# aous72/OpenJPH

Hardware: AMD Instinct MI355X
Metric: Msamples/s encode+decode, 8K 12-bit 4:4:4; achieved HBM GB/s vs roofline (higher is better)
Workload: dtype f32; 1 GPU; c3_8k_444_12b_irv97; width=7680, height=4320, components=3, bit_depth=12, wavelet=9/7 irreversible, decomps=5, hip_streams=1, sample_container_bits=16, roundtrip_max_abs_err=8

## Files before the change

### openjph_amd/csrc/ht_tables.h

```cpp
#ifndef OJPH_HT_TABLES_H
#define OJPH_HT_TABLES_H
#include <stdint.h>

namespace ojphgpu {

struct HtTables {
  uint16_t enc_vlc[2][2048];
  uint16_t dec_vlc[2][1024];
  uint32_t dec_vlc32[2][1024];
  uint16_t dec_uvlc0[320];
  uint16_t dec_uvlc1[256];
};

void build_ht_tables(HtTables& t);
int ensure_tables();
int upload_enc_tables(const HtTables& t);
int upload_dec_tables(const HtTables& t);

}

struct ojphgpu_cb_desc; struct ojphgpu_cb_result;
namespace ojphgpu {
int ht_encode_launch(void* stream, const ojphgpu_cb_desc* d_blocks, uint32_t n, const void* d_coef, uint8_t* d_scratch,
                     uint8_t* d_out, uint32_t out_cap, ojphgpu_cb_result* d_results, uint32_t* d_cursor, uint32_t* d_status,
                     int widths, const uint32_t* d_regions, uint32_t nreg);
bool dec_fuses();
uint64_t ht_decode_fused_state_words(uint32_t n);
uint32_t device_cus(int device);
bool ht_decode_fused_pays(uint32_t n, uint32_t max_h, uint32_t cus);
uint32_t ht_decode_fused_grid(uint32_t n, uint32_t cus);
int ht_decode_fused_launch(void* stream, const ojphgpu_cb_desc* d_blocks, uint32_t n, const uint8_t* d_data, uint32_t* d_quad_scratch,
                           void* d_coef, uint8_t* d_block_status, uint32_t* d_state, uint32_t epoch, uint32_t max_h, int kinds,
                           uint32_t cus, uint32_t* d_host_retry);
uint32_t ht_decode64_extra_aux_words(uint32_t len1);
int ht_decode64_launch(void* stream, const ojphgpu_cb_desc* d_blocks, uint32_t n, const uint8_t* d_data, uint32_t* d_aux,
                       uint32_t* d_quad_scratch, void* d_coef, uint8_t* d_block_status, int refine);
int ht_decode_step2_launch(void* stream, const ojphgpu_cb_desc* d_blocks, uint32_t n, const uint8_t* d_data,
                           const uint32_t* d_quad_scratch, void* d_coef, uint8_t* d_block_status, int kinds);
inline int ht_decode_block_kinds(uint32_t w, uint32_t reversible, uint32_t num_passes, uint32_t len2)
{
  const int refine = (num_passes > 1u && len2 > 0u) ? 16 : 0;
  if (reversible & 4u) return refine | 32;
  return refine | (w > 64u ? 2 : 1) | ((reversible & 1u) ? 4 : 8) | (w > 32u ? 64 : 0) | (w > 16u ? 128 : 0) | 256;
}

}
#endif
```

### openjph_amd/csrc/kernels_ht_enc.hip

```cpp
#include <hip/hip_runtime.h>
#include <stdint.h>
#include <cstdlib>
#include <type_traits>
#include "../../include/ojphgpu.h"
#include "ht_quant.h"
#include "ht_tables.h"

namespace ojphgpu {
__device__ __attribute__((aligned(16))) uint16_t g_enc_vlc[2][2048];
}

namespace {

using ojphgpu::to_sign_mag;

constexpr int MS_WORDS = 512;
constexpr int VLC_WORDS = 64;
constexpr int MEL_CAP = 192;
constexpr int VLC_CAP = 3072 - MEL_CAP;
constexpr int WAVES = 4;
constexpr uint32_t NARROW_MAX_W = 64;

constexpr int MS_WORDS64 = 1040;
constexpr int VLC_WORDS64 = 96;
template <int MSW, int VLW>
struct WaveLdsT {
  uint32_t ms[MSW];
  uint32_t vlc[VLW];
  uint32_t ev[8];
  uint8_t  mel[MEL_CAP];
};

__device__ __forceinline__ void wave_sync()
{
  __builtin_amdgcn_fence(__ATOMIC_SEQ_CST, "wavefront");
  __builtin_amdgcn_wave_barrier();
}

__device__ __forceinline__ uint32_t wave_incl_scan(uint32_t v, int)
{
  int x = (int)v;
  x += __builtin_amdgcn_update_dpp(0, x, 0x111, 0xF, 0xF, false);
  x += __builtin_amdgcn_update_dpp(0, x, 0x112, 0xF, 0xF, false);
  x += __builtin_amdgcn_update_dpp(0, x, 0x114, 0xF, 0xF, false);
  x += __builtin_amdgcn_update_dpp(0, x, 0x118, 0xF, 0xF, false);
  x += __builtin_amdgcn_update_dpp(0, x, 0x142, 0xA, 0xF, false);
  x += __builtin_amdgcn_update_dpp(0, x, 0x143, 0xC, 0xF, false);
  return (uint32_t)x;
}

__device__ __forceinline__ uint32_t get_bits(const uint32_t* buf, uint32_t pos, uint32_t n)
{
  const uint32_t w = pos >> 5, sh = pos & 31;
  const uint32_t lo = buf[w], hi = buf[w + 1];
  const uint32_t v = __funnelshift_r(lo, hi, sh);
  return v & ((1u << n) - 1u);
}

__device__ __forceinline__ void or_bits(uint32_t* buf, uint32_t pos, uint32_t v, uint32_t n)
{
  if (n == 0) return;
  const uint32_t w = pos >> 5, sh = pos & 31;
  atomicOr(&buf[w], v << sh);
  if (sh + n > 32) atomicOr(&buf[w + 1], v >> (32 - sh));
}

__device__ __forceinline__ uint32_t rdlane(uint32_t v, int l) { return (uint32_t)__builtin_amdgcn_readlane((int)v, l); }
__device__ __forceinline__ uint32_t rdfirst(uint32_t v) { return (uint32_t)__builtin_amdgcn_readfirstlane((int)v); }

__device__ __forceinline__ uint32_t expo(uint32_t val) { return val ? 32u - (uint32_t)__clz((int)(val - 1)) : 0u; }
__device__ __forceinline__ uint32_t expo(uint64_t val) { return val ? 64u - (uint32_t)__clzll((long long)(val - 1)) : 0u; }

__device__ __forceinline__ uint32_t mel_exp(uint32_t k)
{
  const uint64_t tbl = 0ull | (1ull << 9) | (1ull << 12) | (1ull << 15) | (2ull << 18) | (2ull << 21) | (2ull << 24) |
                       (3ull << 27) | (3ull << 30) | (4ull << 33) | (5ull << 36);
  return (uint32_t)(tbl >> (3 * k)) & 7u;
}

struct MelState {
  uint32_t k, run, acc, nb, pos, lastff, err;
};

__device__ __forceinline__ void mel_put(MelState& m, uint8_t* buf, uint32_t code, uint32_t n, int lane)
{
  m.acc = (m.acc << n) | code; m.nb += n;
  for (;;) {
    const uint32_t need = m.lastff ? 7u : 8u;
    if (m.nb < need) break;
    const uint32_t byte = (m.acc >> (m.nb - need)) & ((1u << need) - 1u);
    m.nb -= need; m.acc &= (1u << m.nb) - 1u;
    if (m.pos >= (uint32_t)MEL_CAP) { m.err = 1; break; }
    if (lane == 0) buf[m.pos] = (uint8_t)byte;
    m.pos++; m.lastff = (byte == 0xFF);
  }
}

__device__ __forceinline__ void mel_zero_run(MelState& m, uint8_t* buf, uint32_t n, int lane)
{
  while (n > 0) {
    const uint32_t thr = 1u << mel_exp(m.k);
    const uint32_t need = thr - m.run;
    if (n >= need) { mel_put(m, buf, 1, 1, lane); n -= need; m.run = 0; m.k = m.k < 12 ? m.k + 1 : 12; }
    else { m.run += n; n = 0; }
  }
}

__device__ __forceinline__ void mel_one(MelState& m, uint8_t* buf, int lane)
{
  const uint32_t e = mel_exp(m.k);
  mel_put(m, buf, m.run, e + 1, lane);
  m.run = 0; m.k = m.k > 0 ? m.k - 1 : 0;
}

struct Claim { uint32_t raw, base, cap; };
__device__ __forceinline__ Claim claim_request(uint32_t* cursor, const uint32_t* regions, uint32_t nreg, uint32_t bi,
                                               uint32_t bytes, uint32_t out_cap, int lane)
{
  Claim c = { 0, 0, out_cap };
  uint32_t* cur = cursor;
  if (nreg) {
    const uint32_t r = bi & (nreg - 1u);
    c.base = regions[2u * r]; c.cap = regions[2u * r + 1u];
    cur = cursor + 32u * r;
  }
  if (lane == 0) {
    uint32_t z = 0;
    asm volatile("" : "+v"(z));
    c.raw = atomicAdd(cur + z, bytes);
  }
  return c;
}
__device__ __forceinline__ uint32_t claim_offset(const Claim& c, uint32_t bytes)
{
  const uint32_t off = rdfirst(c.raw);
  return (off > c.cap || bytes > c.cap - off) ? 0xFFFFFFFFu : c.base + off;
}
__device__ __forceinline__ uint32_t claim_output(uint32_t* cursor, const uint32_t* regions, uint32_t nreg, uint32_t bi,
                                                 uint32_t bytes, uint32_t out_cap, int lane)
{
  return claim_offset(claim_request(cursor, regions, nreg, bi, bytes, out_cap, lane), bytes);
}

template <bool S64>
__global__ __launch_bounds__(64 * WAVES) void ht_encode_wide_kernel(
    const ojphgpu_cb_desc* __restrict__ blocks, uint32_t n, const uint32_t* __restrict__ coef,
    uint8_t* __restrict__ scratch, uint8_t* __restrict__ out, uint32_t out_cap,
    ojphgpu_cb_result* __restrict__ results, uint32_t* __restrict__ cursor, uint32_t* __restrict__ status,
    const uint32_t* __restrict__ regions, uint32_t nreg)
{
  using V = typename std::conditional<S64, uint64_t, uint32_t>::type;
  constexpr uint32_t VBITS = S64 ? 64u : 32u;
  constexpr int MSW = S64 ? MS_WORDS64 : MS_WORDS, VLW = S64 ? VLC_WORDS64 : VLC_WORDS;
  __shared__ __attribute__((aligned(16))) uint16_t s_vlc[2][2048];
  __shared__ WaveLdsT<MSW, VLW> s_wave[WAVES];
  const int lane = threadIdx.x & 63;
  const int wave = __builtin_amdgcn_readfirstlane((int)(threadIdx.x >> 6));
  const uint32_t bi = blockIdx.x * WAVES + wave;
  const bool mine = bi < n && (S64 ? (blocks[bi].reversible & 4u) != 0 : (blocks[bi].w > NARROW_MAX_W && (blocks[bi].reversible & 4u) == 0));
  if (!__syncthreads_or(mine ? 1 : 0)) return;
  for (int i = threadIdx.x; i < 2 * 2048 / 8; i += blockDim.x)
    reinterpret_cast<uint4*>(&s_vlc[0][0])[i] = reinterpret_cast<const uint4*>(&ojphgpu::g_enc_vlc[0][0])[i];
  __syncthreads();
  if (!mine) return;
  const ojphgpu_cb_desc d = blocks[bi];
  WaveLdsT<MSW, VLW>& L = s_wave[wave];
  const uint32_t W = d.w, H = d.h;
  if (W == 0 || H == 0) { if (lane == 0) { results[bi].offset = 0; results[bi].length = 0; } return; }
  const uint32_t K = d.K_max, p = VBITS - 1u - K;
  const bool rev = (d.reversible & 1u) != 0;
  const float delta_inv = rev ? 0.0f : __fdiv_rn(1.0f, d.delta);
  const uint32_t* src = coef + d.coef_off;
  const uint32_t pitch = d.pitch;
  uint8_t* ms_out = scratch + d.data_off;
  const uint32_t ms_cap = d.scratch_cap > (uint32_t)VLC_CAP ? d.scratch_cap - VLC_CAP : 0;
  uint8_t* vlc_last = scratch + d.data_off + d.scratch_cap - 1;

  const uint32_t QW = (W + 1) >> 1, QH = (H + 1) >> 1, PW = (QW + 1) >> 1, NP = PW * QH;

  for (int i = lane; i < MSW; i += 64) L.ms[i] = 0;
  for (int i = lane; i < VLW; i += 64) L.vlc[i] = 0;
  if (lane < 8) L.ev[lane] = 0;
  wave_sync();
  if (lane == 0) L.vlc[0] = 0xF;
  wave_sync();

  uint32_t ms_carry = 0, ms_k = 0, ms_ff = 0;
  uint32_t v_carry = 4, v_pos = 1, v_prev = 0xFF;
  MelState mel = { 0, 0, 0, 0, 0, 0, 0 };
  uint32_t err = 0, any_sig = 0;
  uint32_t carry_rho = 0;

  uint32_t over = 0;
  auto sample = [&](int x, int y) -> V {
    if (x < 0 || y < 0 || x >= (int)W || y >= (int)H) return (V)0;
    if constexpr (S64) {
      const long long v = reinterpret_cast<const long long*>(src)[(size_t)y * pitch + x];
      const uint64_t m = (v >= 0 ? (uint64_t)v : 0ull - (uint64_t)v) << p;
      over |= (uint32_t)(m >> 63);
      return (v >= 0 ? 0ull : 0x8000000000000000ull) | m;
    } else
      return to_sign_mag(src[(size_t)y * pitch + x], rev, p, delta_inv, over);
  };

  for (uint32_t base = 0; base < NP; base += 64) {
    const uint32_t P = base + lane;
    const bool active = P < NP;
    const uint32_t qy = active ? P / PW : 0, px = active ? P - qy * PW : 0;
    const int x0 = (int)(4 * px), y0 = (int)(2 * qy);
    const bool has_q1 = active && (x0 + 2 < (int)W);
    const bool first_row = qy == 0;

    V val[8]; uint32_t sgn[8];
#pragma unroll
    for (int i = 0; i < 8; ++i) {
      const int q = i >> 2, nn = i & 3;
      V t = active ? sample(x0 + 2 * q + (nn >> 1), y0 + (nn & 1)) : (V)0;
      val[i] = ((V)(t + t) >> p) & ~(V)1;
      sgn[i] = (uint32_t)(t >> (VBITS - 1u));
    }
    uint32_t Eab[6], Sab[6];
#pragma unroll
    for (int i = 0; i < 6; ++i) {
      V t = (active && !first_row) ? sample(x0 - 1 + i, y0 - 1) : (V)0;
      V v = ((V)(t + t) >> p) & ~(V)1;
      Eab[i] = expo(v); Sab[i] = v != 0;
    }

    uint32_t rho[2], cq[2], uq[2], Uq[2], tup[2];
    V msv[8]; uint32_t msl[8];
    uint32_t rho_q[2] = { 0, 0 }, emax[2] = { 0, 0 }, e[8];
#pragma unroll
    for (int i = 0; i < 8; ++i) {
      e[i] = expo(val[i]);
      if (val[i]) rho_q[i >> 2] |= 1u << (i & 3);
      emax[i >> 2] = max(emax[i >> 2], e[i]);
    }
    if (!has_q1) { rho_q[1] = 0; emax[1] = 0; }
    uint32_t rho_prev = __shfl_up(rho_q[1], 1);
    if (lane == 0) rho_prev = carry_rho;
    if (px == 0) rho_prev = 0;
    carry_rho = rdlane(rho_q[1], 63);
#pragma unroll
    for (int q = 0; q < 2; ++q) {
      const uint32_t rl = q == 0 ? rho_prev : rho_q[0];
      uint32_t kappa = 1, c;
      if (first_row) c = (rl >> 1) | (rl & 1);
      else {
        const uint32_t* E = Eab + 2 * q; const uint32_t* S = Sab + 2 * q;
        uint32_t me = max(max(E[0], E[1]), max(E[2], E[3]));
        int max_e = (int)me - 1;
        if (rho_q[q] & (rho_q[q] - 1)) kappa = (uint32_t)max(1, max_e);
        c = (S[0] | S[1]) | ((S[2] | S[3]) << 2) | ((rl & 4) >> 1) | ((rl & 8) >> 2);
      }
      const uint32_t U = max(emax[q], kappa), u = U - kappa;
      uint32_t eps = 0;
      if (u > 0) {
#pragma unroll
        for (int nn = 0; nn < 4; ++nn) eps |= (uint32_t)(e[q * 4 + nn] == emax[q]) << nn;
      }
      const uint32_t tuple = s_vlc[first_row ? 0 : 1][(c << 8) + (rho_q[q] << 4) + eps];
      rho[q] = rho_q[q]; cq[q] = c; uq[q] = u; Uq[q] = U; tup[q] = tuple;
#pragma unroll
      for (int nn = 0; nn < 4; ++nn) {
        const int i = q * 4 + nn;
        const uint32_t m = ((rho_q[q] >> nn) & 1u) ? U - ((tuple >> nn) & 1u) : 0u;
        const V s = val[i] ? val[i] - 2u + sgn[i] : (V)0;
        msl[i] = m;
        msv[i] = m ? (s & ((m >= VBITS ? (V)0 : ((V)1 << m)) - (V)1)) : (V)0;
      }
    }
    const bool q0on = active, q1on = has_q1;
    if (!q1on) { uq[1] = 0; for (int nn = 4; nn < 8; ++nn) { msl[nn] = 0; msv[nn] = 0; } }
    if (!q0on) { uq[0] = 0; for (int nn = 0; nn < 4; ++nn) { msl[nn] = 0; msv[nn] = 0; } }
    any_sig |= (__ballot(((rho[0] | rho[1]) != 0 && active) || over != 0u) != 0ull) ? 1u : 0u;

    uint64_t vb = 0; uint32_t vl = 0;
    auto vadd = [&](uint32_t c, uint32_t len) { vb |= (uint64_t)c << vl; vl += len; };
    uint32_t x0e = 0, xl0 = 0, x1e = 0, xl1 = 0;
    auto uvlc = [](uint32_t u, uint32_t& pre, uint32_t& pl, uint32_t& suf, uint32_t& sl, uint32_t& ext, uint32_t& el) {
      ext = 0; el = 0;
      if (u == 0) { pre = 0; pl = 0; suf = 0; sl = 0; }
      else if (u == 1) { pre = 1; pl = 1; suf = 0; sl = 0; }
      else if (u == 2) { pre = 2; pl = 2; suf = 0; sl = 0; }
      else if (u <= 4) { pre = 4; pl = 3; suf = u - 3; sl = 1; }
      else if (u <= 32 || !S64) { pre = 0; pl = 3; suf = u - 5; sl = 5; }
      else { pre = 0; pl = 3; suf = 28u + ((u - 33u) & 3u); sl = 5; ext = (u - 33u) >> 2; el = 4; }
    };
    bool ev2_valid = false; uint32_t ev2_bit = 0;
    if (q0on) {
      vadd(tup[0] >> 8, (tup[0] >> 4) & 7);
      if (q1on) vadd(tup[1] >> 8, (tup[1] >> 4) & 7);
      const uint32_t u0 = uq[0], u1 = uq[1];
      uint32_t p0, l0, s0, sl0, p1, l1, s1, sl1;
      if (first_row && u0 > 0 && u1 > 0) { ev2_valid = true; ev2_bit = min(u0, u1) > 2; }
      if (first_row && u0 > 2 && u1 > 2) {
        uvlc(u0 - 2, p0, l0, s0, sl0, x0e, xl0); uvlc(u1 - 2, p1, l1, s1, sl1, x1e, xl1);
        vadd(p0, l0); vadd(p1, l1); vadd(s0, sl0); vadd(s1, sl1); vadd(x0e, xl0); vadd(x1e, xl1);
      } else if (first_row && u0 > 2 && u1 > 0) {
        uvlc(u0, p0, l0, s0, sl0, x0e, xl0);
        vadd(p0, l0); vadd(u1 - 1, 1); vadd(s0, sl0); vadd(x0e, xl0);
      } else {
        uvlc(u0, p0, l0, s0, sl0, x0e, xl0); uvlc(u1, p1, l1, s1, sl1, x1e, xl1);
        vadd(p0, l0); vadd(p1, l1); vadd(s0, sl0); vadd(s1, sl1); vadd(x0e, xl0); vadd(x1e, xl1);
      }
    }

    const bool ev0_valid = q0on && cq[0] == 0, ev1_valid = q1on && cq[1] == 0;
    const uint32_t ev0_bit = rho[0] != 0, ev1_bit = rho[1] != 0;
    {
      const uint32_t cnt = (uint32_t)ev0_valid + (uint32_t)ev1_valid + (uint32_t)ev2_valid;
      const uint32_t incl = wave_incl_scan(cnt, lane);
      const uint32_t nev = rdlane(incl, 63);
      uint32_t at = incl - cnt;
      if (ev0_valid) { if (ev0_bit) atomicOr(&L.ev[at >> 5], 1u << (at & 31)); at++; }
      if (ev1_valid) { if (ev1_bit) atomicOr(&L.ev[at >> 5], 1u << (at & 31)); at++; }
      if (ev2_valid) { if (ev2_bit) atomicOr(&L.ev[at >> 5], 1u << (at & 31)); at++; }
      wave_sync();
      uint32_t done = 0;
      while (done < nev) {
        const uint32_t w = done >> 5, sh = done & 31;
        uint32_t word = rdfirst(L.ev[w]) >> sh;
        const uint32_t avail = min(32u - sh, nev - done);
        if (word == 0) { mel_zero_run(mel, L.mel, avail, lane); done += avail; continue; }
        const uint32_t z = (uint32_t)__builtin_ctz(word);
        if (z >= avail) { mel_zero_run(mel, L.mel, avail, lane); done += avail; continue; }
        mel_zero_run(mel, L.mel, z, lane);
        mel_one(mel, L.mel, lane);
        done += z + 1;
      }
      wave_sync();
      if (lane < 8) L.ev[lane] = 0;
    }

    {
      uint32_t tot = 0;
#pragma unroll
      for (int i = 0; i < 8; ++i) tot += msl[i];
      const uint32_t incl = wave_incl_scan(tot, lane);
      const uint32_t T = ms_carry + rdlane(incl, 63);
      uint32_t at = ms_carry + incl - tot;
#pragma unroll
      for (int i = 0; i < 8; ++i) {
        if constexpr (S64) {
          const uint32_t lo = msl[i] < 32u ? msl[i] : 32u;
          or_bits(L.ms, at, (uint32_t)msv[i], lo);
          if (msl[i] > 32u) or_bits(L.ms, at + 32u, (uint32_t)(msv[i] >> 32), msl[i] - 32u);
        } else or_bits(L.ms, at, (uint32_t)msv[i], msl[i]);
        at += msl[i];
      }
      wave_sync();
      uint32_t pos = 0;
      for (;;) {
        const uint32_t first_n = ms_ff ? 7u : 8u;
        const uint32_t start = pos + (lane == 0 ? 0u : first_n + 8u * (uint32_t)(lane - 1));
        const uint32_t nb = lane == 0 ? first_n : 8u;
        const bool ok = start + nb <= T;
        const uint32_t v = ok ? get_bits(L.ms, start, nb) : 0u;
        const uint64_t m_ok = __ballot(ok), m_ff = __ballot(ok && v == 0xFF);
        const uint32_t n_ok = m_ok == ~0ull ? 64u : (uint32_t)__builtin_ctzll(~m_ok);
        const uint32_t f_ff = m_ff ? (uint32_t)__builtin_ctzll(m_ff) : 64u;
        const uint32_t nc = min(n_ok, f_ff + 1u);
        if (nc == 0) break;
        if (ms_k + nc > ms_cap) { err = 1; break; }
        if ((uint32_t)lane < nc) ms_out[ms_k + lane] = (uint8_t)v;
        ms_k += nc;
        pos += first_n + 8u * (nc - 1u);
        ms_ff = f_ff < n_ok ? 1u : 0u;
      }
      const uint32_t rem = T - pos;
      const uint32_t cv = rem ? get_bits(L.ms, pos, rem) : 0u;
      wave_sync();
      const uint32_t used = (T >> 5) + 2;
      for (uint32_t i = lane; i < used && i < (uint32_t)MSW; i += 64) L.ms[i] = 0;
      wave_sync();
      if (lane == 0) L.ms[0] = cv;
      ms_carry = rem;
      wave_sync();
    }

    {
      const uint32_t incl = wave_incl_scan(vl, lane);
      const uint32_t T = v_carry + rdlane(incl, 63);
      {
        const uint32_t at = v_carry + incl - vl, lo = vl < 32u ? vl : 32u;
        or_bits(L.vlc, at, (uint32_t)vb, lo);
        if (vl > 32u) or_bits(L.vlc, at + 32u, (uint32_t)(vb >> 32), vl - 32u);
      }
      wave_sync();
      uint32_t pos = 0;
      for (;;) {
        const uint32_t start = pos + 8u * (uint32_t)lane;
        const bool have7 = start + 7 <= T, have8 = start + 8 <= T;
        const uint32_t v8 = have7 ? get_bits(L.vlc, start, 8) : 0u;
        uint32_t pv = __shfl_up(v8, 1);
        if (lane == 0) pv = v_prev;
        const bool special = have7 && pv > 0x8F && (v8 & 0x7F) == 0x7F;
        const bool stop = !have8 && !special;
        const uint64_t m_sp = __ballot(special), m_st = __ballot(stop);
        const uint32_t fs = m_sp ? (uint32_t)__builtin_ctzll(m_sp) : 64u;
        const uint32_t ft = m_st ? (uint32_t)__builtin_ctzll(m_st) : 64u;
        const uint32_t n8 = min(fs, ft);
        const bool sp = fs < ft;
        if (n8 == 0 && !sp) break;
        if (v_pos + n8 + 1 >= (uint32_t)VLC_CAP) { err = 1; break; }
        if ((uint32_t)lane < n8) *(vlc_last - (v_pos + lane)) = (uint8_t)v8;
        if (sp && (uint32_t)lane == fs) *(vlc_last - (v_pos + lane)) = 0x7F;
        const uint32_t last8 = n8 ? rdlane(v8, (int)(n8 - 1)) : v_prev;
        v_pos += n8 + (sp ? 1u : 0u);
        pos += 8u * n8 + (sp ? 7u : 0u);
        v_prev = sp ? 0x7Fu : last8;
      }
      const uint32_t rem = T - pos;
      const uint32_t cv = rem ? get_bits(L.vlc, pos, rem) : 0u;
      wave_sync();
      for (int i = lane; i < VLW; i += 64) L.vlc[i] = 0;
      wave_sync();
      if (lane == 0) L.vlc[0] = cv;
      v_carry = rem;
      wave_sync();
    }
    if (err) break;
  }

  err |= mel.err;
  uint32_t total = 0, ms_len = ms_k;
  if (!err && any_sig) {
    const uint32_t ms_tmp0 = rdfirst(L.ms[0]);
    if (ms_carry) {
      const uint32_t maxb = ms_ff ? 7u : 8u, t = maxb - ms_carry;
      const uint32_t tmp = ms_tmp0 | ((0xFFu & ((1u << t) - 1u)) << ms_carry);
      if (tmp != 0xFF) {
        if (ms_len >= ms_cap) err = 1;
        else { if (lane == 0) ms_out[ms_len] = (uint8_t)tmp; ms_len++; }
      }
    } else if (ms_ff) ms_len--;
    if (mel.run > 0) mel_put(mel, L.mel, 1, 1, lane);
    const uint32_t need = mel.lastff ? 7u : 8u, remaining = need - mel.nb;
    const uint32_t mel_tmp = (mel.acc << remaining) & 0xFFu;
    const uint32_t mel_mask = (0xFFu << remaining) & 0xFFu;
    const uint32_t vlc_tmp = rdfirst(L.vlc[0]) & 0xFFu;
    const uint32_t vlc_mask = v_carry ? (0xFFu >> (8 - v_carry)) : 0u;
    if ((mel_mask | vlc_mask) != 0) {
      if (mel.pos >= (uint32_t)MEL_CAP) err = 1;
      else {
        const uint32_t fuse = mel_tmp | vlc_tmp;
        if (((((fuse ^ mel_tmp) & mel_mask) | ((fuse ^ vlc_tmp) & vlc_mask)) == 0) && fuse != 0xFF && v_pos > 1) {
          if (lane == 0) L.mel[mel.pos] = (uint8_t)fuse;
          mel.pos++;
        } else {
          if (v_pos >= (uint32_t)VLC_CAP) err = 1;
          else {
            if (lane == 0) { L.mel[mel.pos] = (uint8_t)mel_tmp; *(vlc_last - v_pos) = (uint8_t)vlc_tmp; }
            mel.pos++; v_pos++;
          }
        }
      }
    }
    err |= mel.err;
    total = ms_len + mel.pos + v_pos;
  }
  wave_sync();
  __threadfence_block();

  uint32_t off = 0;
  if (err) total = 0;
  if (total) {
    off = claim_output(cursor, regions, nreg, bi, (total + 3u) & ~3u, out_cap, lane);
    if (off == 0xFFFFFFFFu) { err = 1; total = 0; off = 0; }
  }
  if (total) {
    const uint32_t scup = mel.pos + v_pos;
    uint8_t* dst = out + off;
    const uint8_t* vsrc = vlc_last - v_pos + 1;
    for (uint32_t i = lane; i < total; i += 64) {
      uint32_t b;
      if (i < ms_len) b = ms_out[i];
      else if (i < ms_len + mel.pos) b = L.mel[i - ms_len];
      else b = vsrc[i - ms_len - mel.pos];
      if (i == total - 1) b = scup >> 4;
      else if (i == total - 2) b = (b & 0xF0u) | (scup & 0xFu);
      dst[i] = (uint8_t)b;
    }
  }
  if (lane == 0) {
    results[bi].offset = off; results[bi].length = total;
    if (err) atomicOr(status, 1u);
  }
}

#ifndef ABL
#define ABL 0
#endif
#ifndef NWAVES
#define NWAVES 4
#endif
#ifndef NOUT_CAP
#define NOUT_CAP 5120
#endif
#ifndef NWAVES_PER_EU
#define NWAVES_PER_EU 4
#endif
constexpr uint32_t OUT_CAP = NOUT_CAP;
constexpr int PMS_WORDS = 576;
constexpr int PVLC_WORDS = 112;

struct NarrowLds {
  uint32_t out[OUT_CAP / 4];
  uint32_t ms[PMS_WORDS];
  uint32_t vlc[PVLC_WORDS];
  uint8_t  mel[MEL_CAP + 8];
};
static_assert(MEL_CAP + 8 >= 4 * (MEL_CAP / 4 + 2), "raw MEL words");
#ifndef NWG_PER_CU
#define NWG_PER_CU 4
#endif
static_assert(NWG_PER_CU * (2 * 2048 * 2 + 64 * 4 + NWAVES * sizeof(NarrowLds)) <= 160 * 1024, "the narrow kernel's workgroups do not fit the LDS as planned");

#ifndef ENC_ROWS_W4V
#define ENC_ROWS_W4V 1
#endif
#ifndef ENC_ROWS_AHEAD
#define ENC_ROWS_AHEAD 1
#endif
static_assert(ENC_ROWS_AHEAD == 1 || ENC_ROWS_AHEAD == 2, "one or two steps of rows in flight");

struct __attribute__((aligned(4))) U4 { uint32_t x, y, z, w; };
typedef uint32_t U4V __attribute__((ext_vector_type(4), aligned(4)));

template <int KIND> struct RawRows {
  uint32_t t[4], b[4];
  __device__ __forceinline__ void arrived() { asm volatile("" : "+v"(t[0]), "+v"(t[1]), "+v"(t[2]), "+v"(t[3]), "+v"(b[0]), "+v"(b[1]), "+v"(b[2]), "+v"(b[3])); }
  __device__ __forceinline__ uint32_t top(int k) const { return t[k]; }
  __device__ __forceinline__ uint32_t bot(int k) const { return b[k]; }
};
template <> struct RawRows<1> {
  U4V t, b;
  __device__ __forceinline__ void arrived() { asm volatile("" : "+v"(t), "+v"(b)); }
  __device__ __forceinline__ uint32_t top(int k) const { return t[k]; }
  __device__ __forceinline__ uint32_t bot(int k) const { return b[k]; }
};

__device__ __forceinline__ uint32_t dpp_prev(uint32_t v) { return (uint32_t)__builtin_amdgcn_update_dpp(0, (int)v, 0x138, 0xF, 0xF, false); }
__device__ __forceinline__ uint32_t dpp_next(uint32_t v) { return (uint32_t)__builtin_amdgcn_update_dpp(0, (int)v, 0x130, 0xF, 0xF, false); }

__device__ __forceinline__ uint32_t uvlc_word(uint32_t u)
{
  const uint32_t lo = u < 3u ? 1u : 0u, mid = (u >= 3u && u < 5u) ? 1u : 0u;
  const uint32_t pre = lo ? u : (mid ? 4u : 0u);
  const uint32_t pl = u < 3u ? u : 3u;
  const uint32_t suf = lo ? 0u : (mid ? u - 3u : u - 5u);
  const uint32_t sl = lo ? 0u : (mid ? 1u : 5u);
  return pre | (pl << 8) | (suf << 16) | (sl << 24);
}

constexpr uint64_t MEL_PM = (1ull << 0) | (1ull << 1) | (1ull << 2) | (1ull << 3) | (1ull << 5) | (1ull << 7) | (1ull << 9) | (1ull << 13) |
                            (1ull << 17) | (1ull << 21) | (1ull << 29) | (1ull << 37) | (1ull << 53);
constexpr uint32_t MEL_RAW_BITS = 8u * MEL_CAP;
constexpr uint32_t MEL_RAW_WORDS = MEL_CAP / 4 + 2;

__device__ __forceinline__ void mel_at(uint32_t k, uint32_t c, uint32_t& K, uint32_t& run, uint32_t& ones, uint32_t& pKm1)
{
  const uint32_t full = c >= 85u ? (c - 53u) >> 5 : 0u;
  const uint32_t cc = c - 32u * full;
  if (cc >= 53u) { K = 12u; run = cc - 53u; pKm1 = 37u; }
  else {
    const uint64_t m = MEL_PM << (63u - cc);
    const uint32_t lz = (uint32_t)__builtin_clzll(m);
    K = (uint32_t)__popcll(m) - 1u; run = lz;
    const uint64_t m2 = m & ~(0x8000000000000000ull >> lz);
    pKm1 = m2 ? cc - (uint32_t)__builtin_clzll(m2) : 0u;
  }
  ones = K - k + full;
}

__device__ __forceinline__ void mel_stuff(const uint32_t* raw, uint32_t total_bits, uint8_t* out, MelState& st, int lane)
{
  uint32_t pos = 0, bytes = 0, lastff = 0, err = 0;
  for (;;) {
    const uint32_t first = lastff ? 7u : 8u;
    const uint32_t start = pos + (lane == 0 ? 0u : first + 8u * ((uint32_t)lane - 1u));
    const uint32_t len = lane == 0 ? first : 8u;
    const bool have = start + len <= total_bits;
    const uint32_t w = start >> 5, sh = start & 31u;
    const uint32_t x = have ? __funnelshift_l(raw[w + 1], raw[w], sh) >> (32u - len) : 0u;
    const uint64_t m_have = __ballot(have), m_ff = __ballot(have && x == 0xFFu);
    const uint32_t n_ok = m_have == ~0ull ? 64u : (uint32_t)__builtin_ctzll(~m_have);
    const uint32_t f_ff = m_ff ? (uint32_t)__builtin_ctzll(m_ff) : 64u;
    const uint32_t nc = min(n_ok, f_ff + 1u);
    if (nc == 0) break;
    if (bytes + nc > (uint32_t)MEL_CAP) { err = 1; break; }
    if ((uint32_t)lane < nc) out[bytes + lane] = (uint8_t)x;
    bytes += nc;
    pos += first + 8u * (nc - 1u);
    lastff = f_ff < n_ok ? 1u : 0u;
  }
  const uint32_t left = total_bits - pos;
  const uint32_t w = pos >> 5, sh = pos & 31u;
  const uint32_t x = left ? rdfirst(__funnelshift_l(raw[w + 1], raw[w], sh)) >> (32u - left) : 0u;
  st.k = 0; st.run = 0; st.acc = x; st.nb = left; st.pos = bytes; st.lastff = lastff; st.err = err;
}

template <bool REV, int LOGP>
__global__ __launch_bounds__(64 * NWAVES) __attribute__((amdgpu_waves_per_eu(NWAVES_PER_EU, 8))) void ht_encode_kernel(
    const ojphgpu_cb_desc* __restrict__ blocks, uint32_t n, const uint32_t* __restrict__ coef,
    uint8_t* __restrict__ scratch, uint8_t* __restrict__ out, uint32_t out_cap,
    ojphgpu_cb_result* __restrict__ results, uint32_t* __restrict__ cursor, uint32_t* __restrict__ status,
    const uint32_t* __restrict__ regions, uint32_t nreg)
{
  __shared__ __attribute__((aligned(16))) uint16_t s_vlc[2][2048];
  __shared__ uint32_t s_uvlc[64];
  __shared__ NarrowLds s_wave[NWAVES];
  const int lane = threadIdx.x & 63;
  const int wave = __builtin_amdgcn_readfirstlane((int)(threadIdx.x >> 6));
  const uint32_t bi = blockIdx.x * NWAVES + wave;
  struct DescWords { uint32_t v[sizeof(ojphgpu_cb_desc) / 4]; } dw;
  __builtin_memcpy(&dw, blocks + min(bi, n - 1u), sizeof dw);
  ojphgpu_cb_desc d;
  __builtin_memcpy(&d, &dw, sizeof d);
  static_assert(offsetof(ojphgpu_cb_desc, K_max) == 16 && offsetof(ojphgpu_cb_desc, reversible) == 17, "K_max, reversible: bytes 0, 1 of dword 4");
  uint32_t kr = dw.v[4];
  asm volatile("" : "+s"(kr));
  const uint32_t d_K_max = kr & 0xFFu, d_reversible = (kr >> 8) & 0xFFu;
  const uint32_t W = d.w, H = d.h;
  constexpr uint32_t PPR = 1u << LOGP, RPS = 64u >> LOGP;
  const bool my_width = LOGP == 5 ? (W > NARROW_MAX_W && W <= 4u * PPR) : (W <= NARROW_MAX_W && W <= 4u * PPR);
  const bool my_kind = bi < n && my_width && ((d_reversible & 1u) != 0) == REV && (d_reversible & 4u) == 0;
  const bool mine = my_kind && W != 0 && H != 0;
  NarrowLds& L = s_wave[wave];
  uint8_t* outb = reinterpret_cast<uint8_t*>(L.out);
  const uint32_t K = d_K_max, p = 31u - K;
  constexpr bool rev = REV;
  const float delta_inv = rev ? 0.0f : __fdiv_rn(1.0f, d.delta);
  const uint32_t* src = coef + d.coef_off;
  const uint32_t pitch = d.pitch;
  uint8_t* ms_spill = scratch + d.data_off;
  const uint32_t ms_cap = d.scratch_cap > (uint32_t)VLC_CAP ? d.scratch_cap - VLC_CAP : 0;
  const uint32_t QW = (W + 1) >> 1, QH = (H + 1) >> 1, PW = (QW + 1) >> 1;
  const uint32_t nsteps = (QH + RPS - 1u) / RPS;

  const uint32_t r = (uint32_t)lane >> LOGP, px = (uint32_t)lane & (PPR - 1u);
  const bool pxok = px < PW;
  const uint32_t x0 = 4u * px;
  const bool has_q1 = pxok && x0 + 2 < W;

  auto prologue = [&](bool clear) __attribute__((always_inline)) {
    for (int i = threadIdx.x; i < 2 * 2048 / 8; i += blockDim.x)
      reinterpret_cast<uint4*>(&s_vlc[0][0])[i] = reinterpret_cast<const uint4*>(&ojphgpu::g_enc_vlc[0][0])[i];
    if (threadIdx.x < 64) s_uvlc[threadIdx.x] = uvlc_word(threadIdx.x);
    if (clear) {
      for (int i = lane; i < PMS_WORDS; i += 64) L.ms[i] = 0;
      for (int i = lane; i < PVLC_WORDS; i += 64) L.vlc[i] = 0;
      if (lane < (int)MEL_RAW_WORDS) reinterpret_cast<uint32_t*>(L.mel)[lane] = 0;
      wave_sync();
      if (lane == 0) { L.vlc[0] = 0xF; outb[OUT_CAP - 1] = 0xFF; }
      wave_sync();
    }
    __syncthreads();
  };
  if (!mine) {
    prologue(false);
    if (my_kind && lane == 0) { results[bi].offset = 0; results[bi].length = 0; }
    return;
  }
  const bool w4 = (W & 3u) == 0;

  uint32_t ms_pend = 0, ms_base = 0, ms_k = 0, ms_ff = 0;
  uint32_t v_pend = 4, v_base = 0, v_pos = 1, v_prev = 0xFF;
  uint32_t mel_k = 0, mel_c = 0, mel_bits = 0, mel_err = 0;
  uint32_t* const mel_raw = reinterpret_cast<uint32_t*>(L.mel);
  auto mel_or = [&](uint32_t code, uint32_t len, uint32_t pos) __attribute__((always_inline)) {
    if (len) {
      const uint32_t sh = pos & 31u, w = pos >> 5;
      const uint64_t v = (uint64_t)code << (64u - sh - len);
      atomicOr(&mel_raw[w], (uint32_t)(v >> 32));
      if (sh + len > 32u) atomicOr(&mel_raw[w + 1u], (uint32_t)v);
    }
  };
  auto mel_ones = [&](uint32_t n) __attribute__((always_inline)) {
    if (n == 0u) return;
    if (mel_bits + n > MEL_RAW_BITS) mel_err = 1;
    else if (lane == 0) mel_or((1u << n) - 1u, n, mel_bits);
    mel_bits += n;
  };
  auto mel_zeros = [&](uint32_t n) __attribute__((always_inline)) {
    mel_c += n;
    if (mel_c >= 85u) {
      const uint32_t full = (mel_c - 53u) >> 5;
      mel_ones(12u - mel_k + full);
      mel_k = 12u; mel_c -= 32u * full;
    }
  };
  uint32_t err = 0, any_sig = 0;
  bool prev_sig = false;

  uint32_t ms_out = 0;
  auto flush_stage = [&]() __attribute__((always_inline)) -> bool {
    const uint32_t have = ms_k - ms_out, nwd = have >> 2;
    if (ms_out + 4u * nwd > ms_cap) return false;
    uint32_t* g = reinterpret_cast<uint32_t*>(ms_spill + ms_out);
    for (uint32_t i = lane; i < nwd; i += 64) g[i] = L.out[i];
    const uint32_t keep = L.out[nwd];
    wave_sync();
    if (lane == 0) L.out[0] = keep;
    wave_sync();
    ms_out += 4u * nwd;
    return true;
  };

  uint32_t last_S = 0;

  auto ms_windows = [&](uint32_t base, uint32_t T, bool flush) __attribute__((always_inline)) -> uint32_t {
    uint32_t pos = base;
    for (;;) {
      const uint32_t first_n = ms_ff ? 7u : 8u;
      if (!flush && pos + first_n + 8u * 255u > T) break;
      const uint32_t start = pos + (lane == 0 ? 0u : first_n + 8u * (4u * (uint32_t)lane - 1u));
      const uint32_t lead = lane == 0 ? first_n : 8u;
      uint32_t v = 0, cnt = 0;
      if (start + lead <= T) {
        const uint32_t w = start >> 5, sh = start & 31u;
        v = __funnelshift_r(L.ms[w], L.ms[w + 1], sh);
        cnt = min(4u, 1u + ((T - start - lead) >> 3));
      }
      const uint32_t bytes = (lane == 0 && first_n == 7u) ? ((v & 0x7Fu) | ((v >> 7) << 8)) : v;
      const uint32_t have = cnt == 4u ? 0xFFFFFFFFu : (1u << (8u * cnt)) - 1u;
      const uint32_t ffm = (((bytes & 0x7F7F7F7Fu) + 0x01010101u) & bytes & 0x80808080u) & have;
      const uint64_t m_full = __ballot(cnt == 4u), m_ff = __ballot(ffm != 0u);
      const uint32_t nfull = m_full == ~0ull ? 64u : (uint32_t)__builtin_ctzll(~m_full);
      const uint32_t n_ok = nfull == 64u ? 256u : 4u * nfull + rdlane(cnt, (int)nfull);
      uint32_t f_ff = 256u;
      if (m_ff) { const uint32_t lf = (uint32_t)__builtin_ctzll(m_ff); f_ff = 4u * lf + ((uint32_t)__builtin_ctz(rdlane(ffm, (int)lf)) >> 3); }
      const uint32_t nc = min(n_ok, f_ff + 1u);
      if (nc == 0) break;
      if (ms_k - ms_out + nc + v_pos + 72u > OUT_CAP && !flush_stage()) { err = 1; break; }
      uint8_t* dstb = outb + (ms_k - ms_out) + 4u * (uint32_t)lane;
      const uint32_t mine = nc > 4u * (uint32_t)lane ? min(4u, nc - 4u * (uint32_t)lane) : 0u;
      if (mine > 0) dstb[0] = (uint8_t)bytes;
      if (mine > 1) dstb[1] = (uint8_t)(bytes >> 8);
      if (mine > 2) dstb[2] = (uint8_t)(bytes >> 16);
      if (mine > 3) dstb[3] = (uint8_t)(bytes >> 24);
      ms_k += nc;
      pos += first_n + 8u * (nc - 1u);
      ms_ff = f_ff < n_ok ? 1u : 0u;
    }
    return pos;
  };
  auto ms_windows_full = [&](uint32_t base, uint32_t T) __attribute__((always_inline)) -> uint32_t {
    uint32_t pos = base;
    for (;;) {
      const uint32_t first_n = ms_ff ? 7u : 8u;
      if (pos + first_n + 8u * 255u > T) break;
      const uint32_t start = lane == 0 ? pos : pos + first_n - 8u + 32u * (uint32_t)lane;
      const uint32_t w = start >> 5, sh = start & 31u;
      uint32_t bytes = __funnelshift_r(L.ms[w], L.ms[w + 1], sh);
      if (ms_ff) bytes = lane == 0 ? ((bytes & 0x7Fu) | ((bytes >> 7) << 8)) : bytes;
      const uint32_t ffm = ((bytes & 0x7F7F7F7Fu) + 0x01010101u) & bytes & 0x80808080u;
      const uint64_t m_ff = __ballot(ffm != 0u);
      uint32_t nc = 256u, ff = 0u;
      if (m_ff) { const uint32_t lf = (uint32_t)__builtin_ctzll(m_ff); nc = 4u * lf + ((uint32_t)__builtin_ctz(rdlane(ffm, (int)lf)) >> 3) + 1u; ff = 1u; }
      if (ms_k - ms_out + nc + v_pos + 72u > OUT_CAP && !flush_stage()) { err = 1; break; }
      if (4u * (uint32_t)lane < nc) __builtin_memcpy(outb + (ms_k - ms_out) + 4u * (uint32_t)lane, &bytes, 4);
      ms_k += nc;
      pos += first_n + 8u * (nc - 1u);
      ms_ff = ff;
    }
    return pos;
  };
  auto vlc_windows_full = [&](uint32_t base, uint32_t T) __attribute__((always_inline)) -> uint32_t {
    uint32_t pos = base;
    for (;;) {
      if (pos + 8u * 64u > T) break;
      const uint32_t v8 = get_bits(L.vlc, pos + 8u * (uint32_t)lane, 8);
      uint32_t pv = dpp_prev(v8);
      if (lane == 0) pv = v_prev;
      const uint64_t m_sp = __ballot(pv > 0x8Fu && (v8 & 0x7Fu) == 0x7Fu);
      uint32_t n8 = 64u, sp = 0u;
      if (m_sp) { n8 = (uint32_t)__builtin_ctzll(m_sp); sp = 1u; }
      if (v_pos + n8 + 1 >= (uint32_t)VLC_CAP) { err = 1; break; }
      if (ms_k - ms_out + v_pos + n8 + 72u > OUT_CAP && !flush_stage()) { err = 1; break; }
      if ((uint32_t)lane < n8 + sp) outb[OUT_CAP - 1 - (v_pos + lane)] = (uint8_t)((uint32_t)lane == n8 ? 0x7Fu : v8);
      const uint32_t last8 = n8 ? rdlane(v8, (int)(n8 - 1)) : v_prev;
      v_pos += n8 + sp;
      pos += 8u * n8 + 7u * sp;
      v_prev = sp ? 0x7Fu : last8;
    }
    return pos;
  };
  auto vlc_windows = [&](uint32_t base, uint32_t T, bool flush) __attribute__((always_inline)) -> uint32_t {
    uint32_t pos = base;
    for (;;) {
      if (!flush && pos + 8u * 64u > T) break;
      const uint32_t start = pos + 8u * (uint32_t)lane;
      const bool have7 = start + 7 <= T, have8 = start + 8 <= T;
      const uint32_t v8 = have7 ? get_bits(L.vlc, start, 8) : 0u;
      uint32_t pv = dpp_prev(v8);
      if (lane == 0) pv = v_prev;
      const bool special = have7 && pv > 0x8F && (v8 & 0x7F) == 0x7F;
      const bool stop = !have8 && !special;
      const uint64_t m_sp = __ballot(special), m_st = __ballot(stop);
      const uint32_t fs = m_sp ? (uint32_t)__builtin_ctzll(m_sp) : 64u;
      const uint32_t ft = m_st ? (uint32_t)__builtin_ctzll(m_st) : 64u;
      const uint32_t n8 = min(fs, ft);
      const bool sp = fs < ft;
      if (n8 == 0 && !sp) break;
      if (v_pos + n8 + 1 >= (uint32_t)VLC_CAP) { err = 1; break; }
      if (ms_k - ms_out + v_pos + n8 + 72u > OUT_CAP && !flush_stage()) { err = 1; break; }
      if ((uint32_t)lane < n8) outb[OUT_CAP - 1 - (v_pos + lane)] = (uint8_t)v8;
      if (sp && (uint32_t)lane == fs) outb[OUT_CAP - 1 - (v_pos + lane)] = 0x7F;
      const uint32_t last8 = n8 ? rdlane(v8, (int)(n8 - 1)) : v_prev;
      v_pos += n8 + (sp ? 1u : 0u);
      pos += 8u * n8 + (sp ? 7u : 0u);
      v_prev = sp ? 0x7Fu : last8;
    }
    return pos;
  };
  auto compact = [&](uint32_t* buf, uint32_t pos, uint32_t T, uint32_t nwords) __attribute__((always_inline)) -> uint32_t {
    const uint32_t rem = T - pos, nw = (rem + 31u) >> 5;
    const uint32_t w0 = pos >> 5, sh = pos & 31u;
    uint32_t keep = 0;
    if ((uint32_t)lane < nw) {
      keep = __funnelshift_r(buf[w0 + lane], buf[w0 + lane + 1], sh);
      if (lane == (int)nw - 1 && (rem & 31u)) keep &= (1u << (rem & 31u)) - 1u;
    }
    wave_sync();
    const uint32_t used = min((T >> 5) + 2u, nwords);
    for (uint32_t i = lane; i < used; i += 64) buf[i] = 0;
    wave_sync();
    if ((uint32_t)lane < nw) buf[lane] = keep;
    wave_sync();
    return rem;
  };

  auto or32 = [&](uint32_t* buf, uint32_t pos, uint32_t v) __attribute__((always_inline)) {
    const uint32_t sh = pos & 31u;
    uint32_t* wp = buf + (pos >> 5);
    atomicOr(wp, v << sh);
    atomicOr(wp + 1, (v >> 1) >> (sh ^ 31u));
  };
  auto nz_flags = [](uint32_t x) __attribute__((always_inline)) -> uint32_t { return (x + 0x7F7F7F7Fu) & 0x80808080u; };
  auto gather4 = [](uint32_t f) __attribute__((always_inline)) -> uint32_t { return ((f >> 7) * 0x10204080u) >> 28; };
  typedef unsigned short us2 __attribute__((ext_vector_type(2)));
  auto pk_max = [](uint32_t a, uint32_t b2) __attribute__((always_inline)) -> uint32_t {
    return __builtin_bit_cast(uint32_t, __builtin_elementwise_max(__builtin_bit_cast(us2, a), __builtin_bit_cast(us2, b2)));
  };
  auto left_of = [&](uint32_t v) __attribute__((always_inline)) -> uint32_t {
    if (LOGP == 4) return (uint32_t)__builtin_amdgcn_update_dpp(0, (int)v, 0x111, 0xF, 0xF, false);
    const uint32_t t = dpp_prev(v); return px == 0 ? 0u : t;
  };
  auto right_of = [&](uint32_t v) __attribute__((always_inline)) -> uint32_t {
    if (LOGP == 4) return (uint32_t)__builtin_amdgcn_update_dpp(0, (int)v, 0x101, 0xF, 0xF, false);
    const uint32_t t = dpp_next(v); return px == PPR - 1u ? 0u : t;
  };

  auto code_steps = [&](auto kind_c) __attribute__((always_inline)) {
    constexpr int KIND = decltype(kind_c)::value;
    using Rows = RawRows<KIND>;
    auto load_rows = [&](uint32_t qy, Rows& R) __attribute__((always_inline)) {
      const uint32_t qyc = min(qy, QH - 1u);
      const uint32_t y0 = 2u * qyc, y1 = min(y0 + 1u, H - 1u);
      const uint32_t* r0 = src + (size_t)y0 * pitch;
      const uint32_t* r1 = src + (size_t)y1 * pitch;
      if (ABL & 32) { r0 = coef + (size_t)bi * 4096u + y0 * 64u; r1 = coef + (size_t)bi * 4096u + y1 * 64u; }
      if constexpr (KIND == 1) {
        const uint32_t xc = min(x0, W - 4u);
        R.t = *reinterpret_cast<const U4V*>(r0 + xc);
        R.b = *reinterpret_cast<const U4V*>(r1 + xc);
      } else if (KIND == 0 && w4) {
        const uint32_t xc = min(x0, W - 4u);
        const U4 a = *reinterpret_cast<const U4*>(r0 + xc);
        const U4 c = *reinterpret_cast<const U4*>(r1 + xc);
        R.t[0] = a.x; R.t[1] = a.y; R.t[2] = a.z; R.t[3] = a.w;
        R.b[0] = c.x; R.b[1] = c.y; R.b[2] = c.z; R.b[3] = c.w;
      } else {
#pragma unroll
        for (int k = 0; k < 4; ++k) { const uint32_t xk = min(x0 + (uint32_t)k, W - 1u); R.t[k] = r0[xk]; R.b[k] = r1[xk]; }
      }
    };
    Rows A;
    [[maybe_unused]] Rows B;
    load_rows(r, A);
    if constexpr (ENC_ROWS_AHEAD == 2) load_rows(r + RPS, B);
    prologue(true);

    float colf[4]; uint32_t colm[4];
#pragma unroll
    for (int k = 0; k < 4; ++k) {
      const bool in = pxok && x0 + (uint32_t)k < W;
      colf[k] = in ? ldexpf(delta_inv, -(int)p) : 0.0f;
      colm[k] = in ? (1u << (31u - p)) - 1u : 0u;
    }
    const bool ragged = (QH & (RPS - 1u)) != 0 || (H & 1u) != 0;

    auto one_step = [&](const uint32_t step, Rows& R) __attribute__((always_inline)) {
      const uint32_t qy = RPS * step + r;
      const bool active = pxok && qy < QH;
      R.arrived();
      uint32_t rt[4], rb[4];
#pragma unroll
      for (int k = 0; k < 4; ++k) { rt[k] = R.top(k); rb[k] = R.bot(k); }
      if (ragged && step + 1 == nsteps) {
        const bool bot = active && 2u * qy + 1u < H;
#pragma unroll
        for (int k = 0; k < 4; ++k) { rt[k] = active ? rt[k] : 0u; rb[k] = bot ? rb[k] : 0u; }
      }
      uint32_t mu[8], sx[8];
      uint32_t nz = 0;
#pragma unroll
      for (int k = 0; k < 4; ++k) {
#pragma unroll
        for (int j = 0; j < 2; ++j) {
// ... 22 lines not shown
      if (rev) nz &= (1u << K) - 1u;
      if (ENC_ROWS_AHEAD == 2 || step + 1 < nsteps) load_rows(qy + ENC_ROWS_AHEAD * RPS, R);
      if (ENC_ROWS_AHEAD == 2 && err) return;
      if (ABL & 16) { any_sig |= (uint32_t)(__ballot((mu[0] ^ mu[1] ^ mu[2] ^ mu[3] ^ mu[4] ^ mu[5] ^ mu[6] ^ mu[7]) == 0x12345u) != 0ull); return; }
      {
        const bool step_sig = __ballot(nz != 0u) != 0ull;
        const bool skip = !step_sig && !prev_sig;
        prev_sig = step_sig;
        if (skip) {
          const uint32_t nq = (uint32_t)__popcll(__ballot(active)) + (uint32_t)__popcll(__ballot(has_q1 && active));
          mel_zeros(nq);
          last_S = 0;
          return;
        }
        any_sig |= step_sig ? 1u : 0u;
      }
      uint32_t e[8], sv[8];
#pragma unroll
      for (int i = 0; i < 8; ++i) {
        const uint32_t m1 = mu[i] - 1u, w = m1 + mu[i];
        e[i] = (0u - (uint32_t)__builtin_clz(w)) & 31u;
        sv[i] = __builtin_amdgcn_alignbit(m1, sx[i], 31);
      }
      const uint32_t ep0 = e[0] | (e[1] << 8) | (e[2] << 16) | (e[3] << 24);
      const uint32_t ep1 = e[4] | (e[5] << 8) | (e[6] << 16) | (e[7] << 24);
      const uint32_t sf0 = nz_flags(ep0), sf1 = nz_flags(ep1);
      const uint32_t rho0 = gather4(sf0), rho1 = gather4(sf1);
      const uint32_t emax0 = max(max(e[0], e[1]), max(e[2], e[3])), emax1 = max(max(e[4], e[5]), max(e[6], e[7]));

      uint32_t S;
      {
        const uint32_t b0 = e[1], b1 = e[3], b2 = e[5], b3 = e[7];
        const uint32_t m12 = max(b1, b2);
        const uint32_t own = max(b0, m12) | (max(m12, b3) << 16);
        const uint32_t X = b3 | (b0 << 16), Y = b0 | (b3 << 16);
        const uint32_t nb = (left_of(X) & 0xFFFFu) | (right_of(X) & 0xFFFF0000u);
        const uint32_t mx = pk_max(own, nb);
        const uint32_t F = (pk_max(nb, Y) + 0x007F001Fu) & 0x00800020u;
        const uint32_t f12 = ((m12 + 31u) & 32u) * 0x10004u;
        S = mx | F | f12;
      }
      const uint32_t give = (uint32_t)lane >= 64u - PPR ? last_S : S;
      const uint32_t above = (uint32_t)__builtin_amdgcn_ds_bpermute((int)(((lane - (int)PPR) & 63) << 2), (int)give);
      last_S = S;

      const uint32_t rho_left = left_of(rho1);
      uint32_t uq[2], tup[2], Uq[2], chi[2];
#pragma unroll
      for (int q = 0; q < 2; ++q) {
        const uint32_t rl = q == 0 ? rho_left : rho0, rho = q ? rho1 : rho0, emax = q ? emax1 : emax0, ep = q ? ep1 : ep0;
        const uint32_t aq = q ? above >> 16 : above;
        uint32_t c5 = (aq & 0xA0u) | ((4u * rl + 48u) & 64u);
        uint32_t tsel = 2048u;
        if (step == 0) {
          const bool fr = qy == 0;
          c5 = fr ? ((rl >> 1) | (rl & 1u)) << 5 : c5;
          tsel = fr ? 0u : 2048u;
        }
        const uint32_t multi = 0u - ((0xFEE8u >> rho) & 1u);
        const uint32_t me = aq & 31u;
        const uint32_t kappa = 1u + ((me > 2u ? me - 2u : 0u) & multi);
        const uint32_t U = max(emax, kappa), u = U - kappa;
        const uint32_t xe = ep ^ (emax * 0x01010101u);
        uint32_t eps = gather4((nz_flags(xe) ^ 0x80808080u));
        eps = u ? eps : 0u;
        tup[q] = (&s_vlc[0][0])[tsel + (c5 << 3) + (rho << 4) + eps];
        uq[q] = u; Uq[q] = U; chi[q] = c5;
      }

      uint32_t vb = 0, vl = 0;
      bool ev2_valid = false; uint32_t ev2_bit = 0;
      {
        const uint32_t u0 = uq[0], u1 = has_q1 ? uq[1] : 0u;
        vb = tup[0] >> 8; vl = (tup[0] >> 4) & 7u;
        if (has_q1) { vb |= (tup[1] >> 8) << vl; vl += (tup[1] >> 4) & 7u; }
        const bool first_row = qy == 0;
        const bool both_big = first_row && u0 > 2 && u1 > 2;
        const bool one_big = first_row && !both_big && u0 > 2 && u1 > 0;
        ev2_valid = first_row && u0 > 0 && u1 > 0; ev2_bit = min(u0, u1) > 2;
        const uint32_t w0 = s_uvlc[both_big ? u0 - 2u : u0];
        uint32_t w1 = s_uvlc[both_big ? u1 - 2u : u1];
        if (one_big) w1 = (u1 - 1u) | (1u << 8);
        vb |= (w0 & 0xFFu) << vl; vl += (w0 >> 8) & 0xFFu;
        vb |= (w1 & 0xFFu) << vl; vl += (w1 >> 8) & 0xFFu;
        vb |= ((w0 >> 16) & 0xFFu) << vl; vl += w0 >> 24;
        vb |= ((w1 >> 16) & 0xFFu) << vl; vl += w1 >> 24;
        if (!active) { vb = 0; vl = 0; ev2_valid = false; }
      }

      uint32_t mp[2];
#pragma unroll
      for (int q = 0; q < 2; ++q) {
        const uint32_t sf = q ? sf1 : sf0;
        const uint32_t sig = (sf - (sf >> 7)) | sf;
        const uint32_t ek = ((tup[q] & 15u) * 0x204081u) & 0x01010101u;
        mp[q] = (Uq[q] * 0x01010101u - ek) & sig;
      }
      const uint32_t tot0 = __builtin_amdgcn_sad_u8(mp[0], 0u, 0u), tot = __builtin_amdgcn_sad_u8(mp[1], 0u, tot0);

      const uint32_t incl = wave_incl_scan(tot | (vl << 16), lane);
      const uint32_t sums = rdlane(incl, 63);
      const uint32_t step_bits = sums & 0xFFFFu, step_vbits = sums >> 16;
      if (ms_base + ms_pend + step_bits + 64u > 32u * (uint32_t)PMS_WORDS) {
        ms_pend = compact(L.ms, ms_base, ms_base + ms_pend, PMS_WORDS);
        ms_base = 0;
      }
      if (v_base + v_pend + step_vbits + 64u > 32u * (uint32_t)PVLC_WORDS) {
        v_pend = compact(L.vlc, v_base, v_base + v_pend, PVLC_WORDS);
        v_base = 0;
      }

      if (ABL & 8) { any_sig |= (uint32_t)(__ballot((vb ^ mp[0] ^ mp[1] ^ sv[0] ^ sv[7] ^ chi[1] ^ incl) == 0x12345u) != 0ull); return; }
      if (!(ABL & 1)) {
        const uint32_t fl = ((active && chi[0] == 0u) ? (rho0 != 0u ? 0x11u : 0x01u) : 0u) |
                            ((active && has_q1 && chi[1] == 0u) ? (rho1 != 0u ? 0x22u : 0x02u) : 0u) |
                            ((step == 0 && ev2_valid) ? (ev2_bit != 0u ? 0x44u : 0x04u) : 0u);
        if (__ballot((fl & 7u) != 0u) != 0ull) {
          const uint32_t nwords = step == 0 ? 3u : 2u;
          for (uint32_t wd = 0; wd < nwords; ++wd) {
            const uint32_t e = 64u * wd + (uint32_t)lane;
            uint32_t from, slot;
            if (step == 0) {
              const uint32_t e2 = e - 3u * PPR;
              const bool fr = e < 3u * PPR;
              from = fr ? e / 3u : PPR + (e2 >> 1);
              slot = fr ? e - 3u * (e / 3u) : e2 & 1u;
            } else { from = e >> 1; slot = e & 1u; }
            const uint32_t g = (uint32_t)__builtin_amdgcn_ds_bpermute((int)((from & 63u) << 2), (int)fl) >> slot;
            const bool valid = from < 64u && (g & 1u) != 0u, one = valid && (g & 16u) != 0u;
            const uint64_t Vw = __ballot(valid), Bw = __ballot(one);
            if (Vw == 0ull) continue;
            const uint32_t nvalid = (uint32_t)__popcll(Vw);
            if (Bw == 0ull) { mel_c += nvalid; continue; }
            const uint32_t before = __builtin_amdgcn_mbcnt_hi((uint32_t)(Vw >> 32), __builtin_amdgcn_mbcnt_lo((uint32_t)Vw, 0u));
            uint32_t info = 0;
            uint32_t consumed = 0;
            {
              uint64_t ones = Bw;
              while (ones) {
                const uint32_t l = (uint32_t)__builtin_ctzll(ones);
                asm("s_bitset0_b64 %0, %1" : "+s"(ones) : "s"(l));
                const uint32_t bf = rdlane(before, (int)l);
                mel_c += bf - consumed; consumed = bf + 1u;
                info = (uint32_t)lane == l ? (mel_k | (mel_c << 4)) : info;
                uint32_t K, pKm1;
                if (mel_c >= 85u) mel_c -= (mel_c - 53u) & ~31u;
                if (mel_c >= 53u) { K = 12u; pKm1 = 37u; }
                else {
                  const uint64_t m = MEL_PM << (63u - mel_c);
                  K = (uint32_t)__popcll(m) - 1u;
                  const uint64_t m2 = m & ~(0x8000000000000000ull >> (uint32_t)__builtin_clzll(m));
                  pKm1 = m2 ? mel_c - (uint32_t)__builtin_clzll(m2) : 0u;
                }
                int km1 = (int)K - 1;
                asm("s_max_i32 %0, %1, 0" : "=s"(km1) : "s"(km1) : "scc");
                mel_k = (uint32_t)km1; mel_c = pKm1;
              }
            }
            uint32_t code = 0, len = 0;
            if (one) {
              uint32_t K, run, nones, pKm1;
              mel_at(info & 15u, info >> 4, K, run, nones, pKm1);
              const uint32_t eb = mel_exp(K);
              code = (((1u << nones) - 1u) << (eb + 1u)) | run;
              len = nones + eb + 1u;
            }
            const uint32_t at_incl = wave_incl_scan(len, lane);
            const uint32_t wbits = rdlane(at_incl, 63);
            if (mel_bits + wbits > MEL_RAW_BITS) mel_err = 1;
            else mel_or(code, len, mel_bits + at_incl - len);
            mel_bits += wbits;
            mel_c += nvalid - consumed;
          }
          mel_zeros(0u);
        }
      }

      if (ABL & 2) { any_sig |= (uint32_t)(__ballot((vb ^ mp[0] ^ mp[1] ^ sv[0] ^ sv[3] ^ sv[5] ^ sv[7] ^ incl) == 0x12345u) != 0ull); }
      else {
        const uint32_t at = ms_base + ms_pend + (incl & 0xFFFFu) - tot;
        const bool wide_bits = __ballot(max(Uq[0], Uq[1]) > 16u) != 0ull;
        if (!wide_bits) {
          uint32_t pr[4], ln[2];
#pragma unroll
          for (int q = 0; q < 2; ++q) {
            const uint32_t m = mp[q];
            const uint32_t m0 = m & 0xFFu, m2 = (m >> 16) & 0xFFu;
            const uint32_t v0 = __builtin_amdgcn_ubfe(sv[4 * q + 0], 0u, m0), v1 = __builtin_amdgcn_ubfe(sv[4 * q + 1], 0u, (m >> 8) & 0xFFu);
            const uint32_t v2 = __builtin_amdgcn_ubfe(sv[4 * q + 2], 0u, m2), v3 = __builtin_amdgcn_ubfe(sv[4 * q + 3], 0u, m >> 24);
            pr[2 * q] = v0 | (v1 << m0); pr[2 * q + 1] = v2 | (v3 << m2);
            ln[q] = (m + (m >> 8)) & 0xFFu;
          }
          if (tot != 0u) {
            or32(L.ms, at, pr[0]);
            or32(L.ms, at + ln[0], pr[1]);
            or32(L.ms, at + tot0, pr[2]);
            or32(L.ms, at + tot0 + ln[1], pr[3]);
          }
        } else {
          uint32_t pos = at;
#pragma unroll
          for (int i = 0; i < 8; ++i) {
            const uint32_t m = (mp[i >> 2] >> (8 * (i & 3))) & 0xFFu;
            or_bits(L.ms, pos, __builtin_amdgcn_ubfe(sv[i], 0u, m), m);
            pos += m;
          }
        }
        if (vl != 0u) or32(L.vlc, v_base + v_pend + (incl >> 16) - vl, vb);
      }
      wave_sync();
      if (ABL & 4) { ms_base = 0; ms_pend = step_bits & 7u; v_base = 0; v_pend = step_vbits & 7u; return; }
      {
        const uint32_t T = ms_base + ms_pend + step_bits;
        const uint32_t pos = ms_windows_full(ms_base, T);
        ms_base = pos; ms_pend = T - pos;
      }
      {
        const uint32_t T = v_base + v_pend + step_vbits;
        const uint32_t pos = vlc_windows_full(v_base, T);
        v_base = pos; v_pend = T - pos;
      }
    };
    if constexpr (ENC_ROWS_AHEAD == 2) {
      uint32_t step = 0;
      for (; step + 1u < nsteps && !err; step += 2) {
        one_step(step, A);
        one_step(step + 1u, B);
      }
      if (step < nsteps && !err) one_step(step, A);
    } else {
      for (uint32_t step = 0; step < nsteps && !err; ++step) one_step(step, A);
    }
  };
  if (!ENC_ROWS_W4V) code_steps(std::integral_constant<int, 0>());
  else if (w4) code_steps(std::integral_constant<int, 1>());
  else code_steps(std::integral_constant<int, 2>());

  uint32_t ms_carry = 0, v_carry = 0;
  if (!err) {
    uint32_t pos = ms_windows(ms_base, ms_base + ms_pend, true);
    ms_carry = compact(L.ms, pos, ms_base + ms_pend, PMS_WORDS);
    pos = vlc_windows(v_base, v_base + v_pend, true);
    v_carry = compact(L.vlc, pos, v_base + v_pend, PVLC_WORDS);
  }

  err |= mel_err;
  uint32_t total = 0, ms_len = ms_k;
  MelState mel = { 0, 0, 0, 0, 0, 0, 0 };
  if (!err && any_sig) {
    const uint32_t ms_tmp0 = rdfirst(L.ms[0]);
    if (ms_carry) {
      const uint32_t maxb = ms_ff ? 7u : 8u, tt = maxb - ms_carry;
      const uint32_t tmp = ms_tmp0 | ((0xFFu & ((1u << tt) - 1u)) << ms_carry);
      if (tmp != 0xFF) {
        if (lane == 0) outb[ms_len - ms_out] = (uint8_t)tmp;
        ms_len++;
      }
    } else if (ms_ff) ms_len--;
    {
      uint32_t K, run, nones, pKm1;
      mel_at(mel_k, mel_c, K, run, nones, pKm1);
      mel_ones(nones + (run > 0u ? 1u : 0u));
    }
    err |= mel_err;
    {
      uint32_t* rawc = L.ms + 128;
      const uint32_t total_bits = mel_bits;
      wave_sync();
      if ((uint32_t)lane < MEL_RAW_WORDS) rawc[lane] = (uint32_t)lane < MEL_RAW_WORDS - 1u ? mel_raw[lane] : 0u;
      wave_sync();
      mel_stuff(rawc, err ? 0u : total_bits, L.mel, mel, lane);
      wave_sync();
    }
    const uint32_t need = mel.lastff ? 7u : 8u, remaining = need - mel.nb;
    const uint32_t mel_tmp = (mel.acc << remaining) & 0xFFu;
    const uint32_t mel_mask = (0xFFu << remaining) & 0xFFu;
    const uint32_t vlc_tmp = rdfirst(L.vlc[0]) & 0xFFu;
    const uint32_t vlc_mask = v_carry ? (0xFFu >> (8 - v_carry)) : 0u;
    if ((mel_mask | vlc_mask) != 0) {
      if (mel.pos >= (uint32_t)MEL_CAP) err = 1;
      else {
        const uint32_t fuse = mel_tmp | vlc_tmp;
        if (((((fuse ^ mel_tmp) & mel_mask) | ((fuse ^ vlc_tmp) & vlc_mask)) == 0) && fuse != 0xFF && v_pos > 1) {
          if (lane == 0) L.mel[mel.pos] = (uint8_t)fuse;
          mel.pos++;
        } else {
          if (v_pos >= (uint32_t)VLC_CAP) err = 1;
          else {
            if (lane == 0) { L.mel[mel.pos] = (uint8_t)mel_tmp; outb[OUT_CAP - 1 - v_pos] = (uint8_t)vlc_tmp; }
            mel.pos++; v_pos++;
          }
        }
      }
    }
    err |= mel.err;
    total = ms_len + mel.pos + v_pos;
  }
  wave_sync();
  __threadfence_block();

  if (err) total = 0;
  const uint32_t slot = (total + 3u) & ~3u;
  Claim claim = { 0, 0, 0 };
  if (total) claim = claim_request(cursor, regions, nreg, bi, slot, out_cap, lane);
  const uint32_t scup = mel.pos + v_pos;
  const uint32_t tail = mel.pos + v_pos;
  const uint32_t gpart = min(ms_out, ms_len), local = ms_len - gpart;
  const bool packed = (gpart & 3u) == 0 && local + tail <= OUT_CAP;
  if (total && packed) {
    for (uint32_t base = 0; base < tail; base += 64) {
      const uint32_t i = base + lane;
      uint32_t b = 0;
      if (i < mel.pos) b = L.mel[i];
      else if (i < tail) b = outb[OUT_CAP - v_pos + (i - mel.pos)];
      wave_sync();
      if (i < tail) {
        if (i == tail - 1) b = scup >> 4;
        else if (i == tail - 2) b = (b & 0xF0u) | (scup & 0xFu);
        outb[local + i] = (uint8_t)b;
      }
      wave_sync();
    }
  }
  uint32_t off = 0;
  if (total) {
    off = claim_offset(claim, slot);
    if (off == 0xFFFFFFFFu) { err = 1; total = 0; off = 0; }
  }
  if (total) {
    uint8_t* dst = out + off;
    if (gpart) {
      const uint32_t nwd = gpart >> 2;
      const uint32_t* s32 = reinterpret_cast<const uint32_t*>(ms_spill);
      uint32_t* d32 = reinterpret_cast<uint32_t*>(dst);
      for (uint32_t i = lane; i < nwd; i += 64) d32[i] = s32[i];
      if ((uint32_t)lane < (gpart & 3u)) dst[4u * nwd + lane] = ms_spill[4u * nwd + lane];
    }
    if (packed) {
      uint32_t* d32 = reinterpret_cast<uint32_t*>(dst + gpart);
      const uint32_t nw = (local + tail + 3u) >> 2;
      for (uint32_t i = lane; i < nw; i += 64) d32[i] = L.out[i];
    } else {
      for (uint32_t i = gpart + lane; i < total; i += 64) {
        uint32_t b;
        if (i < ms_len) b = outb[i - ms_out];
        else if (i < ms_len + mel.pos) b = L.mel[i - ms_len];
        else b = outb[OUT_CAP - v_pos + (i - ms_len - mel.pos)];
        if (i == total - 1) b = scup >> 4;
        else if (i == total - 2) b = (b & 0xF0u) | (scup & 0xFu);
        dst[i] = (uint8_t)b;
      }
    }
  }
  if (lane == 0) {
    results[bi].offset = off; results[bi].length = total;
    if (err) atomicOr(status, 1u);
  }
}

}

namespace ojphgpu {
int ht_encode_launch(void* stream, const ojphgpu_cb_desc* d_blocks, uint32_t n, const void* d_coef, uint8_t* d_scratch,
                     uint8_t* d_out, uint32_t out_cap, ojphgpu_cb_result* d_results, uint32_t* d_cursor, uint32_t* d_status,
                     int widths, const uint32_t* d_regions, uint32_t nreg)
{
  if (n == 0) return OJPHGPU_OK;
  if (ensure_tables() != 0) return OJPHGPU_E_HIP;
  if (!d_blocks || !d_coef || !d_scratch || !d_out || !d_results || !d_cursor || !d_status) return OJPHGPU_E_INVALID;
  if (nreg && (!d_regions || (nreg & (nreg - 1u)))) return OJPHGPU_E_INVALID;
  dim3 grid((n + WAVES - 1) / WAVES);
  if ((widths & 12) == 0) widths |= 12;
  static const unsigned ballast = [] { const char* e = getenv("OJPHGPU_ENC_LDS_BALLAST"); const long v = e ? atol(e) : 0; return v > 0 && v < 100000 ? (unsigned)v : 0u; }();
  const dim3 ngrid((n + NWAVES - 1) / NWAVES);
  if ((widths & 1) && (widths & 4) && (widths & 16))
    hipLaunchKernelGGL((ht_encode_kernel<true, 3>), ngrid, dim3(64 * NWAVES), ballast, (hipStream_t)stream, d_blocks, n,
                       (const uint32_t*)d_coef, d_scratch, d_out, out_cap, d_results, d_cursor, d_status, d_regions, nreg);
  else if ((widths & 1) && (widths & 4))
    hipLaunchKernelGGL((ht_encode_kernel<true, 4>), ngrid, dim3(64 * NWAVES), ballast, (hipStream_t)stream, d_blocks, n,
                       (const uint32_t*)d_coef, d_scratch, d_out, out_cap, d_results, d_cursor, d_status, d_regions, nreg);
  if ((widths & 1) && (widths & 8) && (widths & 16))
    hipLaunchKernelGGL((ht_encode_kernel<false, 3>), ngrid, dim3(64 * NWAVES), ballast, (hipStream_t)stream, d_blocks, n,
                       (const uint32_t*)d_coef, d_scratch, d_out, out_cap, d_results, d_cursor, d_status, d_regions, nreg);
  else if ((widths & 1) && (widths & 8))
    hipLaunchKernelGGL((ht_encode_kernel<false, 4>), ngrid, dim3(64 * NWAVES), ballast, (hipStream_t)stream, d_blocks, n,
                       (const uint32_t*)d_coef, d_scratch, d_out, out_cap, d_results, d_cursor, d_status, d_regions, nreg);
  if ((widths & 2) && (widths & 64)) {
    if (widths & 4)
      hipLaunchKernelGGL((ht_encode_kernel<true, 5>), ngrid, dim3(64 * NWAVES), ballast, (hipStream_t)stream, d_blocks, n,
                         (const uint32_t*)d_coef, d_scratch, d_out, out_cap, d_results, d_cursor, d_status, d_regions, nreg);
    if (widths & 8)
      hipLaunchKernelGGL((ht_encode_kernel<false, 5>), ngrid, dim3(64 * NWAVES), ballast, (hipStream_t)stream, d_blocks, n,
                         (const uint32_t*)d_coef, d_scratch, d_out, out_cap, d_results, d_cursor, d_status, d_regions, nreg);
  } else if (widths & 2)
    hipLaunchKernelGGL(ht_encode_wide_kernel<false>, grid, dim3(64 * WAVES), 0, (hipStream_t)stream, d_blocks, n,
                       (const uint32_t*)d_coef, d_scratch, d_out, out_cap, d_results, d_cursor, d_status, d_regions, nreg);
  if (widths & 32)
    hipLaunchKernelGGL(ht_encode_wide_kernel<true>, grid, dim3(64 * WAVES), 0, (hipStream_t)stream, d_blocks, n,
                       (const uint32_t*)d_coef, d_scratch, d_out, out_cap, d_results, d_cursor, d_status, d_regions, nreg);
  return hipGetLastError() == hipSuccess ? OJPHGPU_OK : OJPHGPU_E_HIP;
}
}

extern "C" int ojphgpu_ht_encode(void* stream, const ojphgpu_cb_desc* d_blocks, uint32_t n,
                                  const void* d_coef, uint8_t* d_scratch, uint8_t* d_out, uint32_t out_cap,
                                  ojphgpu_cb_result* d_results, uint32_t* d_cursor, uint32_t* d_status)
{
  return ojphgpu::ht_encode_launch(stream, d_blocks, n, d_coef, d_scratch, d_out, out_cap, d_results, d_cursor, d_status, 3 | 32, nullptr, 0);
}

namespace ojphgpu {
int upload_enc_tables(const HtTables& t)
{
  return hipMemcpyToSymbol(HIP_SYMBOL(g_enc_vlc), t.enc_vlc, sizeof(t.enc_vlc)) == hipSuccess ? 0 : -1;
}
}
```

### openjph_amd/csrc/ojphgpu_codec.cpp

```cpp
#include <hip/hip_runtime.h>

#include <algorithm>
#include <chrono>
#include <cstdio>
#include <cstdlib>
#include <cstring>
#include <memory>
#include <mutex>
#include <new>
#include <vector>

#include "ht_tables.h"
#include "ojph_plan.h"
#include "ojph_pool.h"

using namespace ojphgpu;

namespace ojphgpu {

int ensure_tables()
{
  static std::mutex mu;
  static bool done[64] = { false };
  int dev = 0;
  if (hipGetDevice(&dev) != hipSuccess || dev < 0 || dev >= 64) return -1;
  std::lock_guard<std::mutex> lock(mu);
  if (done[dev]) return 0;
  static HtTables tables;
  static bool built = false;
  if (!built) { build_ht_tables(tables); built = true; }
  if (upload_enc_tables(tables) != 0 || upload_dec_tables(tables) != 0) return -1;
  done[dev] = true;
  return 0;
}

}

#include "ojphgpu_objects.h"

extern "C" void ojphgpu_encoder_destroy(ojphgpu_encoder* e)
{
  if (!e) return;
  (void)hipSetDevice(e->device);
  if (e->side) (void)hipStreamSynchronize(e->side);
  if (e->low) (void)hipStreamSynchronize(e->low);
  e->pending = false;
  for (DeviceBuf* b : { &e->arena, &e->image, &e->dwt_descs, &e->img_descs, &e->cb_descs, &e->conv_descs, &e->scratch, &e->out,
                        &e->results, &e->counters, &e->regions }) b->release();
  e->h_out.release(); e->h_res.release();
  if (e->side) (void)hipStreamDestroy(e->side);
  if (e->low) (void)hipStreamDestroy(e->low);
  if (e->ev_fork) (void)hipEventDestroy(e->ev_fork);
  if (e->ev_join) (void)hipEventDestroy(e->ev_join);
  if (e->ev_low) (void)hipEventDestroy(e->ev_low);
  e->timer.destroy();
  delete e->quality;
  delete e->rate;
  delete e;
}

extern "C" int ojphgpu_encoder_create(const ojphgpu_plan* plan, int device, void* stream, ojphgpu_encoder** out)
{
  if (!plan) return OJPHGPU_E_INVALID;
  return ojphgpu_encoder_create_tiles(plan, device, stream, 0, (uint32_t)plan->plan.tiles.size(), out);
}

static int encoder_create(const ojphgpu_plan* plan, int device, void* stream, uint32_t tile_first, uint32_t tile_count,
                          uint32_t nframes, ojphgpu_encoder** out, bool blocks_only = false, bool joined_only = false);

extern "C" int ojphgpu_encoder_create_tiles(const ojphgpu_plan* plan, int device, void* stream, uint32_t tile_first,
                                             uint32_t tile_count, ojphgpu_encoder** out)
{
  return no_throw([&] { return encoder_create(plan, device, stream, tile_first, tile_count, 1, out); });
}

int ojphgpu_encoder_create_joined(const ojphgpu_plan* plan, int device, void* stream, ojphgpu_encoder** out)
{
  if (!plan) return OJPHGPU_E_INVALID;
  return no_throw([&] { return encoder_create(plan, device, stream, 0, (uint32_t)plan->plan.tiles.size(), 1, out, false, true); });
}

extern "C" int ojphgpu_encoder_create_batch(const ojphgpu_plan* plan, int device, void* stream, uint32_t num_frames,
                                             ojphgpu_encoder** out)
{
  if (!plan) return OJPHGPU_E_INVALID;
  return no_throw([&] { return encoder_create(plan, device, stream, 0, (uint32_t)plan->plan.tiles.size(), num_frames, out); });
}

static void encoder_block_layout(ojphgpu_encoder* e, const uint32_t* band_kmax, std::vector<ojphgpu_cb_desc>& bd, uint64_t& scratch_total,
                                 bool* clamped = nullptr)
{
  if (clamped) *clamped = false;
  const Plan& P = *e->P;
  const uint32_t nframes = e->nframes;
  bd.assign(e->block_ids.size(), ojphgpu_cb_desc());
  uint64_t scratch_bytes = 0, samples = 0;
  bool over32_top = false, over32_rest = false, over128_top = false, over128_rest = false;
  for (size_t i = 0; i < bd.size(); ++i) {
    const Block& k = P.blocks[e->block_ids[i]]; const Band& B = P.bands[k.band];
    samples += (uint64_t)k.r.w * k.r.h;
    ojphgpu_cb_desc& d = bd[i]; memset(&d, 0, sizeof(d));
    const bool wide = is_wide(P, B.comp);
    d.coef_off = B.plane_off + ((uint64_t)k.r.y0 * B.pitch + k.r.x0) * (wide ? 2u : 1u); d.pitch = B.pitch;
    d.w = (uint16_t)k.r.w; d.h = (uint16_t)k.r.h; d.K_max = (uint8_t)B.K_max; d.reversible = (uint8_t)((P.style(B.comp).rev ? 1 : 0) | (wide ? 4 : 0));
    d.missing_msbs = (uint8_t)(B.K_max - 1); d.num_passes = 1; d.delta = B.delta;
    d.data_off = scratch_bytes; d.scratch_cap = block_scratch_bytes(k.r.w, k.r.h, band_kmax ? std::max(B.K_max, band_kmax[k.band]) : B.K_max);
    scratch_bytes += d.scratch_cap;
    (i < e->n_top ? e->widths_top : e->widths_rest) |= wide ? 32 : ((k.r.w > 64 ? 2 : 1) | ((d.reversible & 1) ? 4 : 8));
    if (!wide && k.r.w > 32 && k.r.w <= 64) (i < e->n_top ? over32_top : over32_rest) = true;
    if (!wide && k.r.w > 128) (i < e->n_top ? over128_top : over128_rest) = true;
  }
  if (!over32_top) e->widths_top |= 16;
  if (!over32_rest) e->widths_rest |= 16;
  if (!over128_top) e->widths_top |= 64;
  if (!over128_rest) e->widths_rest |= 64;
  if (nframes > 1) {
    const size_t nb = bd.size();
    bd.resize(nb * nframes);
    for (uint32_t f = 1; f < nframes; ++f)
      for (size_t i = 0; i < nb; ++i) {
        ojphgpu_cb_desc d = bd[i];
        d.coef_off += (uint64_t)f * P.arena_elems; d.data_off += (uint64_t)f * scratch_bytes;
        bd[f * nb + i] = d;
      }
    scratch_bytes *= nframes; samples *= nframes;
  }
  uint32_t kmax_all = 0;
  for (size_t b = 0; b < P.bands.size(); ++b) kmax_all = std::max(kmax_all, band_kmax ? std::max(P.bands[b].K_max, band_kmax[b]) : P.bands[b].K_max);
  uint64_t cap = kmax_all > 20 ? scratch_bytes : std::min<uint64_t>(scratch_bytes, samples * 3 + (1u << 20));
  if (clamped && cap > 0xFFFFFF00ull) *clamped = true;
  cap = std::min<uint64_t>(cap, 0xFFFFFF00ull);
  {
    const char* ev = getenv("OJPHGPU_ENC_REGIONS"); const long v = ev ? atol(ev) : 16;
    uint32_t R = (v >= 0 && v <= 64 && (v & (v - 1)) == 0) ? (uint32_t)v : 16u;
    if (bd.size() < 4 * (size_t)R) R = 0;
    std::vector<uint64_t> rc(R ? R : 1, 0);
    if (R) for (size_t i = 0; i < bd.size(); ++i) {
      const uint64_t own = kmax_all > 20 ? bd[i].scratch_cap : std::min<uint64_t>(bd[i].scratch_cap, (uint64_t)bd[i].w * bd[i].h * 3 + 64);
      rc[(i < e->n_top ? i : i - e->n_top) & (R - 1)] += own;
    }
    uint64_t total = 0;
    e->h_regions.assign(2 * (size_t)R, 0);
    for (uint32_t r = 0; r < R; ++r) {
      const uint64_t c = (rc[r] + (1u << 16) + 255) & ~(uint64_t)255;
      if (total + c > 0xFFFFFF00ull) {
        if (clamped) *clamped = true;
        R = 0; break;
      }
      e->h_regions[2 * r] = (uint32_t)total; e->h_regions[2 * r + 1] = (uint32_t)c;
      total += c;
    }
    e->nreg = R;
    if (R) cap = total; else e->h_regions.clear();
    e->counters_bytes = R ? (size_t)R * 128 : 16;
  }
  e->out_cap = (uint32_t)cap;
  scratch_total = scratch_bytes;
}

static int encoder_create(const ojphgpu_plan* plan, int device, void* stream, uint32_t tile_first, uint32_t tile_count,
                          uint32_t nframes, ojphgpu_encoder** out, bool blocks_only, bool joined_only)
{
  if (!plan || !out || nframes == 0) return OJPHGPU_E_INVALID;
  *out = nullptr;
  if ((uint64_t)tile_first + tile_count > plan->plan.tiles.size()) return OJPHGPU_E_INVALID;
  if (plan->plan.skip_read || plan->plan.skip_recon) return OJPHGPU_E_INVALID;
  HIPCHK(hipSetDevice(device));
  if (ensure_tables() != 0) return OJPHGPU_E_HIP;
  ojphgpu_encoder* e = new (std::nothrow) ojphgpu_encoder();
  if (!e) return OJPHGPU_E_NOMEM;
  struct Owner { ojphgpu_encoder* p; ~Owner() { if (p) ojphgpu_encoder_destroy(p); } } owner{ e };
  const Plan& P = plan->plan;
  e->handle = plan; e->P = &P; e->device = device; e->stream = (hipStream_t)stream;
  auto bail = [&](int rc) { return rc; };

  e->tiles = TileRange{ tile_first, tile_count };
  e->nframes = nframes;
  const TileRange tr = e->tiles;
  const uint64_t frame_elems = P.frame_elems;
  std::vector<ojphgpu_dwt_desc> dd, idd;
  std::vector<ojphgpu_convert_desc> cd;
  if (!blocks_only) {
    build_level_batches(P, tr, dd, e->batches);
    build_image_level_descs(P, tr, dd, e->batches, idd);
    replicate_levels(dd, idd, e->batches, nframes, P.arena_elems, frame_elems);
    e->need_convert = build_convert_descs(P, tr, cd, e->conv_max_w, e->conv_max_h);
    replicate_converts(cd, nframes, P.arena_elems, P.frame_elems);
  }
  e->block_ids = blocks_of_tiles(P, tr);
  if (nframes == 1 && max_recon_decomps(P) >= 2 && getenv("OJPHGPU_NO_OVERLAP") == nullptr) {
    auto top = [&](uint32_t id) { const Band& B = P.bands[P.blocks[id].band]; return B.res == P.style(B.comp).L; };
    auto mid = std::stable_partition(e->block_ids.begin(), e->block_ids.end(), top);
    e->n_top = (uint32_t)(mid - e->block_ids.begin());
    {
      static const int share_env = [] { const char* v = getenv("OJPHGPU_ENC_TOP_SHARE"); const int x = v ? atoi(v) : 0; return x < 10 ? 0 : x > 100 ? 100 : x; }();
      double s_top = 0, s_low = 0;
      for (size_t i = 0; i < e->block_ids.size(); ++i) {
        const Block& k = P.blocks[e->block_ids[i]];
        (i < e->n_top ? s_top : s_low) += (double)k.r.w * k.r.h * 1e-6;
      }
      double dwt_us = 0, level_bytes = 8.0 * (s_top + s_low) * 1e6 / 4.0;
      for (uint32_t l = 2; l <= max_recon_decomps(P); ++l, level_bytes /= 4.0) dwt_us += std::max(12.0, level_bytes / 3.0e6);
      const double us_per_ms = 3.8, margin_us = 30.0;
      const double move = (s_top + margin_us / us_per_ms - 1.6 * s_low - dwt_us / us_per_ms) / 2.0;
      int share = share_env;
      if (!share) { share = s_top > 0 && move > 0 ? (int)(100.0 * (1.0 - move / s_top)) : 100; share = share < 50 ? 50 : share > 100 ? 100 : share; }
      e->n_top = (uint32_t)((uint64_t)e->n_top * (uint32_t)share / 100u);
    }
    if (e->n_top == 0 || e->n_top == e->block_ids.size()) e->n_top = 0;
    else {
      int prio_lo = 0, prio_hi = 0;
      (void)hipDeviceGetStreamPriorityRange(&prio_lo, &prio_hi);
      const char* pe = getenv("OJPHGPU_ENC_SIDE_PRIO");
      const int prio = pe && pe[0] == 'l' ? prio_lo : pe && pe[0] == 'h' ? prio_hi : (prio_lo + prio_hi) / 2;
      const char* rel = getenv("OJPHGPU_ENC_RELEASE");
      e->can_release = !blocks_only && !joined_only && !(rel && rel[0] == '0');
      const int own_prio = pe ? prio : e->can_release ? prio_lo : 0;
      if (hipStreamCreateWithPriority(&e->side, hipStreamNonBlocking, own_prio) != hipSuccess ||
          hipEventCreateWithFlags(&e->ev_fork, hipEventDisableTiming) != hipSuccess ||
          hipEventCreateWithFlags(&e->ev_join, hipEventDisableTiming) != hipSuccess) return bail(OJPHGPU_E_HIP);
      if (e->can_release &&
          (hipStreamCreateWithPriority(&e->low, hipStreamNonBlocking, own_prio) != hipSuccess ||
           hipEventCreateWithFlags(&e->ev_low, hipEventDisableTiming) != hipSuccess)) return bail(OJPHGPU_E_HIP);
    }
  }
  std::vector<ojphgpu_cb_desc> bd;
  uint64_t scratch_bytes = 0;
  encoder_block_layout(e, nullptr, bd, scratch_bytes);
  const uint64_t cap = e->out_cap;

  if ((!blocks_only && (e->arena.alloc(P.arena_elems * 4 * nframes) || e->dwt_descs.alloc(dd.size() * sizeof(dd[0])) ||
                        e->img_descs.alloc(idd.size() * sizeof(dd[0])) || e->conv_descs.alloc(cd.size() * sizeof(cd[0])))) ||
      e->cb_descs.alloc(bd.size() * sizeof(bd[0])) ||
      e->scratch.alloc(scratch_bytes) || e->out.alloc(cap) ||
      e->results.alloc(bd.size() * sizeof(ojphgpu_cb_result)) || e->counters.alloc(e->counters_bytes) ||
      (e->nreg && e->regions.alloc(e->h_regions.size() * 4)))
    return bail(OJPHGPU_E_NOMEM);
  if (e->nreg && hipMemcpy(e->regions.p, e->h_regions.data(), e->h_regions.size() * 4, hipMemcpyHostToDevice) != hipSuccess) return bail(OJPHGPU_E_HIP);
  if (!blocks_only && hipMemset(e->arena.p, 0, P.arena_elems * 4 * nframes) != hipSuccess) return bail(OJPHGPU_E_HIP);
  if (!dd.empty() && hipMemcpy(e->dwt_descs.p, dd.data(), dd.size() * sizeof(dd[0]), hipMemcpyHostToDevice) != hipSuccess) return bail(OJPHGPU_E_HIP);
  if (!idd.empty() && hipMemcpy(e->img_descs.p, idd.data(), idd.size() * sizeof(idd[0]), hipMemcpyHostToDevice) != hipSuccess) return bail(OJPHGPU_E_HIP);
  if (!bd.empty() && hipMemcpy(e->cb_descs.p, bd.data(), bd.size() * sizeof(bd[0]), hipMemcpyHostToDevice) != hipSuccess) return bail(OJPHGPU_E_HIP);
  if (!cd.empty() && hipMemcpy(e->conv_descs.p, cd.data(), cd.size() * sizeof(cd[0]), hipMemcpyHostToDevice) != hipSuccess) return bail(OJPHGPU_E_HIP);
  e->h_results.resize(bd.size());
  if (e->timer.init() != 0) return bail(OJPHGPU_E_HIP);
  owner.p = nullptr;
  *out = e;
  return OJPHGPU_OK;
}

int ojphgpu_encoder_run_container(ojphgpu_encoder* e, const void* d_image, int container);

extern "C" int ojphgpu_encoder_run_device(ojphgpu_encoder* e, const int32_t* d_image) { return ojphgpu_encoder_run_container(e, d_image, 32); }
extern "C" int ojphgpu_encoder_run_device16(ojphgpu_encoder* e, const uint16_t* d_image) { return ojphgpu_encoder_run_container(e, d_image, 16); }
extern "C" int ojphgpu_encoder_run_device8(ojphgpu_encoder* e, const uint8_t* d_image) { return ojphgpu_encoder_run_container(e, d_image, 8); }

namespace {
struct BlockCoderRun {
  ojphgpu_encoder* e; uint8_t* out; ojphgpu_cb_result* res; uint32_t* cnt; uint32_t nblocks; Spans* T;
  bool forked = false;
  int launch(hipStream_t st, uint32_t first, uint32_t n, int widths) {
    const int sh = T ? T->begin(SP_HT_ENC, st) : -1;
    int rc = ojphgpu::ht_encode_launch(st, (const ojphgpu_cb_desc*)e->cb_descs.p + first, n, e->arena.p, (uint8_t*)e->scratch.p, out,
                                       e->out_cap, res + first, cnt, cnt + 1, widths, (const uint32_t*)e->regions.p, e->nreg);
    if (rc) return rc;
    if (T) T->end(sh, st);
    return OJPHGPU_OK;
  }
  int clear() { int rc = encoder_settle(e); if (rc) return rc; HIPCHK(hipMemsetAsync(cnt, 0, e->counters_bytes, e->stream)); return OJPHGPU_OK; }
  int fork_top(bool release = false) {
    forked = true;
    HIPCHK(hipEventRecord(e->ev_fork, e->stream));
    HIPCHK(hipStreamWaitEvent(e->side, e->ev_fork, 0));
    int rc = launch(e->side, 0, e->n_top, e->widths_top);
    if (rc) return rc;
    HIPCHK(hipEventRecord(e->ev_join, e->side));
    if (release) { e->pending = true; HIPCHK(hipStreamWaitEvent(e->low, e->ev_fork, 0)); }
    return OJPHGPU_OK;
  }
  int rest_released() { return launch(e->low, e->n_top, nblocks - e->n_top, e->widths_rest); }
  int rest_and_join() {
    int rc = e->n_top && !forked ? fork_top() : OJPHGPU_OK;
    if (rc) return rc;
    rc = launch(e->stream, e->n_top, nblocks - e->n_top, e->widths_rest);
    if (rc) return rc;
    if (e->n_top) HIPCHK(hipStreamWaitEvent(e->stream, e->ev_join, 0));
    return OJPHGPU_OK;
  }
};
struct ReleasedBranch {
  ojphgpu_encoder* e; bool armed = false;
  ~ReleasedBranch() { if (armed) (void)hipEventRecord(e->ev_low, e->low); }
};
}

int ojphgpu_encoder_run_container(ojphgpu_encoder* e, const void* d_image, int container)
{
  if (!e || !d_image) return OJPHGPU_E_INVALID;
  const Plan& P = *e->P;
  if (container != 32 && container != 16 && container != 8) return OJPHGPU_E_INVALID;
  if (container != 32) for (const CompGeo& g : P.comps) if (g.bit_depth > (uint32_t)container) return OJPHGPU_E_INVALID;
  hipStream_t s = e->stream;
  Spans& T = e->timer;
  BlockCoderRun coder{ e, (uint8_t*)(e->o_out ? e->o_out : e->out.p),
                       (ojphgpu_cb_result*)(e->o_results ? e->o_results : e->results.p),
                       (uint32_t*)(e->o_counters ? e->o_counters : e->counters.p), (uint32_t)e->block_ids.size() * e->nframes, &T };
  int rc = coder.clear();
  if (rc) return rc;
  const bool release = encoder_releases(e);
  ReleasedBranch branch{ e };
  T.start(s);
  if (e->need_convert) {
    const int sp = T.begin(SP_CONVERT, s);
    rc = ojphgpu_convert_forward_ex(s, &P.p, (const ojphgpu_convert_desc*)e->conv_descs.p, e->tiles.count * e->nframes,
                                    e->conv_max_w, e->conv_max_h, d_image, e->arena.p, container);
    T.end(sp, s);
  }
  if (rc) return rc;
  const bool budget = e->searches();
  for (size_t i = 0; i < e->batches.size(); ++i) {
    const LevelBatch& b = e->batches[i];
    const int sp = T.begin(SP_DWT, s);
    if (b.img_first >= 0) {
      ojphgpu_params pp = P.p; pp.reversible = b.rev ? 1 : 0; pp.bit_depth = b.img_depth; pp.is_signed = b.img_signed;
      const ojphgpu_dwt_desc* idesc = (const ojphgpu_dwt_desc*)e->img_descs.p + b.img_first;
      rc = b.general ? ojphgpu_dwt_forward_general_image(s, &b.k, &pp, idesc, b.count, b.max_w, b.max_h, d_image, e->arena.p, container)
                     : ojphgpu_dwt_forward_image_ex(s, &pp, idesc, b.count, b.max_w, b.max_h, d_image, e->arena.p, container, b.nc == 3);
    } else if (b.general)
      rc = ojphgpu_dwt_forward_general(s, &b.k, (const ojphgpu_dwt_desc*)e->dwt_descs.p + b.first, b.count, b.max_w, b.max_h, e->arena.p);
    else
      rc = ojphgpu_dwt_forward(s, b.rev ? 1 : 0, (const ojphgpu_dwt_desc*)e->dwt_descs.p + b.first, b.count,
                               b.max_w, b.max_h, e->arena.p);
    if (rc) return rc;
    T.end(sp, s);
    const bool top_done = b.depth == 0 && (i + 1 == e->batches.size() || e->batches[i + 1].depth != 0);
    if (!budget && e->n_top && top_done) {
      if ((rc = coder.fork_top(release)) != 0) return rc;
      if (release) { s = e->low; branch.armed = true; }
    }
  }
  if (e->quality_on) {
    T.finish(s);
    e->quality->frame = d_image; e->quality->container = container;
    e->rate->searched = false;
    e->ran = true; e->fetched = false;
    return OJPHGPU_OK;
  }
  if (budget) {
    EncoderRate& R = *e->rate;
    HIPCHK(hipMemsetAsync(R.hist.p, 0, R.hist.n, s));
    const int sp = T.begin(SP_STATS, s);
    rc = ojphgpu_band_stats(s, (const ojphgpu_stats_desc*)R.stats_descs.p, R.n_stats, R.stats_max_w, R.stats_max_h, e->arena.p, (uint32_t*)R.hist.p);
    if (rc) return rc;
    T.end(sp, s);
    T.finish(s);
    R.searched = false;
    e->ran = true; e->fetched = false;
    return OJPHGPU_OK;
  }
  if (release && coder.forked) {
    if ((rc = coder.rest_released()) != 0) return rc;
    T.finish_two(s, e->side);
  } else {
    if ((rc = coder.rest_and_join()) != 0) return rc;
    T.finish(s);
  }
  e->ran = true; e->fetched = false;
  return OJPHGPU_OK;
}

extern "C" int ojphgpu_encoder_set_timing(ojphgpu_encoder* e, int per_launch)
{
  if (!e) return OJPHGPU_E_INVALID;
  e->timer.detail = per_launch != 0;
  return OJPHGPU_OK;
}

extern "C" int ojphgpu_encoder_is_pending(const ojphgpu_encoder* e, int* pending)
{
  if (!e || !pending) return OJPHGPU_E_INVALID;
  *pending = e->pending ? 1 : 0;
  return OJPHGPU_OK;
}

extern "C" int ojphgpu_encoder_coded_bytes(ojphgpu_encoder* e, uint64_t* bytes)
{
  if (!e || !bytes || !e->ran) return OJPHGPU_E_INVALID;
  int rc = encoder_settle(e);
  if (rc) return rc;
  e->h_cursors.assign(e->counters_bytes / 4, 0);
  HIPCHK(hipMemcpyAsync(e->h_cursors.data(), e->counters.p, e->counters_bytes, hipMemcpyDeviceToHost, e->stream));
  HIPCHK(hipStreamSynchronize(e->stream));
  uint64_t total = e->h_cursors[0];
  for (uint32_t r = 1; r < e->nreg; ++r) total += e->h_cursors[32 * (size_t)r];
  *bytes = total;
  return e->h_cursors[1] ? OJPHGPU_E_OVERFLOW : OJPHGPU_OK;
}

static int encoder_fetch(ojphgpu_encoder* e, uint32_t frame, std::vector<ojphgpu_coded_block>& cb)
{
  if (frame >= e->nframes) return OJPHGPU_E_INVALID;
  const Plan& P = e->searches() ? e->rate->frame_plan[frame]->plan : *e->P;
  if (!e->fetched) {
    int rc = ojphgpu_encoder_coded_bytes(e, &e->nbytes);
    if (rc) return rc;
    const size_t rbytes = e->h_results.size() * sizeof(ojphgpu_cb_result);
    if (e->h_out.reserve(std::max<size_t>((size_t)e->nbytes + 16, (size_t)e->out_cap / 4)) || e->h_res.reserve(rbytes + 16))
      return OJPHGPU_E_NOMEM;
    if (rbytes) HIPCHK(hipMemcpyAsync(e->h_res.p, e->results.p, rbytes, hipMemcpyDeviceToHost, e->stream));
    std::vector<uint64_t> hpos(e->nreg ? e->nreg : 1, 0);
    if (e->nreg) {
      uint64_t at = 0;
      for (uint32_t r = 0; r < e->nreg; ++r) {
        const uint32_t used = e->h_cursors[32 * (size_t)r];
        hpos[r] = at;
        if (used) HIPCHK(hipMemcpyAsync(e->h_out.p + at, (const uint8_t*)e->out.p + e->h_regions[2 * r], used, hipMemcpyDeviceToHost, e->stream));
        at += used;
      }
    } else if (e->nbytes) HIPCHK(hipMemcpyAsync(e->h_out.p, e->out.p, (size_t)e->nbytes, hipMemcpyDeviceToHost, e->stream));
    HIPCHK(hipStreamSynchronize(e->stream));
    if (rbytes) memcpy(e->h_results.data(), e->h_res.p, rbytes);
    if (e->nreg)
      for (size_t i = 0; i < e->h_results.size(); ++i) {
        const uint32_t r = (uint32_t)(i < e->n_top ? i : i - e->n_top) & (e->nreg - 1);
        if (e->h_results[i].length) e->h_results[i].offset = (uint32_t)(e->h_results[i].offset - e->h_regions[2 * r] + hpos[r]);
      }
    e->fetched = true;
  }
  ojphgpu_coded_blocks(P, e->block_ids, e->h_results.data() + (size_t)frame * e->block_ids.size(), cb);
  return OJPHGPU_OK;
}

static int encoder_rate_search(ojphgpu_encoder* e);
static int encoder_quality_search(ojphgpu_encoder* e);
static int encoder_capped_search(ojphgpu_encoder* e);

extern "C" int ojphgpu_encoder_finish(ojphgpu_encoder* e, uint8_t* h_out, size_t cap, size_t* out_len)
{
  if (!e || !out_len || !e->ran) return OJPHGPU_E_INVALID;
  return ojphgpu_encoder_finish_frame(e, 0, h_out, cap, out_len);
}

extern "C" int ojphgpu_encoder_finish_frame(ojphgpu_encoder* e, uint32_t frame, uint8_t* h_out, size_t cap, size_t* out_len)
{
  if (!e || !out_len || !e->ran) return OJPHGPU_E_INVALID;
  if (e->tiles.first != 0 || e->tiles.count != e->P->tiles.size()) return OJPHGPU_E_INVALID;
  if (frame >= e->nframes) return OJPHGPU_E_INVALID;
  return no_throw([&]() -> int {
  std::vector<ojphgpu_coded_block> cb;
  const bool tm = getenv("OJPHGPU_TIMING") != nullptr;
  auto now = [] { return std::chrono::steady_clock::now(); };
  auto t0 = now();
  const bool budgets = !e->budgets.empty();
  int rc = e->quality_on ? (e->cap_bytes ? encoder_capped_search(e) : encoder_quality_search(e)) : budgets ? encoder_rate_search(e) : OJPHGPU_OK;
  if (rc) return rc;
  ojphgpu_rate_info info;
  if (budgets && (rc = ojphgpu_rate_rounds_frame(e->rate->rounds, frame, &info)) != 0) return rc;
  if (e->searches()) t0 = now();
  rc = encoder_fetch(e, frame, cb);
  if (rc) return rc;
  auto t1 = now();
  rc = ojphgpu_t2_write(e->searches() ? e->rate->frame_plan[frame] : e->handle, e->h_out.p, cb.data(), h_out, cap, out_len);
  if (budgets) e->rate->final_ms = std::chrono::duration<double, std::milli>(now() - t0).count();
  if (e->quality_on) e->quality->final_ms += std::chrono::duration<double, std::milli>(now() - t0).count();
  if (tm) fprintf(stderr, "ojphgpu: finish frame %u: D2H %.2f ms, Tier-2 %.2f ms\n", frame,
                  std::chrono::duration<double, std::milli>(t1 - t0).count(),
                  std::chrono::duration<double, std::milli>(now() - t1).count());
  return rc;
  });
}

extern "C" int ojphgpu_encoder_finish_tiles(ojphgpu_encoder* e, uint8_t* h_out, size_t cap, size_t* out_len,
                                             uint32_t* tile_part_len)
{
  if (!e || !out_len || !e->ran || e->searches()) return OJPHGPU_E_INVALID;
  return no_throw([&]() -> int {
    std::vector<ojphgpu_coded_block> cb;
    int rc = encoder_fetch(e, 0, cb);
    if (rc) return rc;
    return ojphgpu_t2_write_tiles(e->handle, e->h_out.p, cb.data(), e->tiles.first, e->tiles.count, h_out, cap,
                                  out_len, tile_part_len);
  });
}

namespace ojphgpu {
int assemble_launch(void* stream, const T2Job* d_jobs, uint32_t njobs, const uint8_t* d_blob, const uint8_t* d_data, uint8_t* d_out);
int publish_words_launch(void* stream, uint32_t* d_dst, const uint32_t* src, uint32_t n);
int copy_to_host_launch(void* stream, void* d_dst, const void* src, size_t bytes);
}

extern "C" int ojphgpu_encoder_finish_tiles_device(ojphgpu_encoder* e, uint8_t* d_out, size_t cap, size_t* out_len,
                                                    uint32_t* tile_part_len)
{
  if (!e || !out_len || !e->ran || e->searches()) return OJPHGPU_E_INVALID;
  return no_throw([&]() -> int {
    const Plan& P = *e->P;
    uint64_t nbytes = 0;
    int rc = ojphgpu_encoder_coded_bytes(e, &nbytes);
    if (rc) return rc;
    const size_t rbytes = e->h_results.size() * sizeof(ojphgpu_cb_result);
    if (rbytes) HIPCHK(hipMemcpyAsync(e->h_results.data(), e->results.p, rbytes, hipMemcpyDeviceToHost, e->stream));
    HIPCHK(hipStreamSynchronize(e->stream));
    e->fetched = false;
    std::vector<ojphgpu_coded_block> cb;
    ojphgpu_coded_blocks(P, e->block_ids, e->h_results.data(), cb);
    T2Layout L;
    rc = t2_layout_tiles(P, cb.data(), e->tiles.first, (size_t)e->tiles.first + e->tiles.count, L, tile_part_len);
    if (rc) return rc;
    *out_len = (size_t)L.total;
    if (!d_out || cap < L.total) return OJPHGPU_E_OVERFLOW;
    const size_t jbytes = L.jobs.size() * sizeof(T2Job), boff = (jbytes + 63) & ~(size_t)63;
    DeviceBuf lay;
    if (lay.alloc(boff + L.blob.size() + 64)) return OJPHGPU_E_NOMEM;
    struct Free { DeviceBuf& b; ~Free() { b.release(); } } fr{ lay };
    if (jbytes) HIPCHK(hipMemcpyAsync(lay.p, L.jobs.data(), jbytes, hipMemcpyHostToDevice, e->stream));
    if (!L.blob.empty()) HIPCHK(hipMemcpyAsync((uint8_t*)lay.p + boff, L.blob.data(), L.blob.size(), hipMemcpyHostToDevice, e->stream));
    rc = assemble_launch(e->stream, (const T2Job*)lay.p, (uint32_t)L.jobs.size(), (const uint8_t*)lay.p + boff,
                         (const uint8_t*)(e->o_out ? e->o_out : e->out.p), d_out);
    if (rc) return rc;
    HIPCHK(hipStreamSynchronize(e->stream));
    return OJPHGPU_OK;
  });
}

static int encoder_restore_descs(ojphgpu_encoder* e)
{
  HIPCHK(hipSetDevice(e->device));
  int rc = encoder_settle(e);
  if (rc) return rc;
  HIPCHK(hipStreamSynchronize(e->stream));
  const std::vector<ojphgpu_cb_desc>& bd = e->rate->bd;
  if (!bd.empty()) HIPCHK(hipMemcpy(e->cb_descs.p, bd.data(), bd.size() * sizeof(bd[0]), hipMemcpyHostToDevice));
  e->ran = false;
  return OJPHGPU_OK;
}

static bool encoder_may_search(const ojphgpu_encoder* e)
{
  const Plan& P = *e->P;
  return e->tiles.first == 0 && e->tiles.count == P.tiles.size() && !e->o_out && rate_plan_ok(P);
}

static int encoder_rate_setup(ojphgpu_encoder* e);

extern "C" int ojphgpu_encoder_set_budget(ojphgpu_encoder* e, uint64_t max_bytes)
{
  if (!e) return OJPHGPU_E_INVALID;
  if (max_bytes == 0) {
    if (!e->budgets.empty() && e->rate) { const int rc = encoder_restore_descs(e); if (rc) return rc; }
    e->budgets.clear();
    return OJPHGPU_OK;
  }
  if (e->nframes > 1) return OJPHGPU_E_INVALID;
  return ojphgpu_encoder_set_budgets(e, &max_bytes, 1);
}

extern "C" int ojphgpu_encoder_set_budgets(ojphgpu_encoder* e, const uint64_t* max_bytes, uint32_t n)
{
  if (!e || !max_bytes || n != e->nframes) return OJPHGPU_E_INVALID;
  uint32_t zeros = 0;
  for (uint32_t f = 0; f < n; ++f) zeros += max_bytes[f] == 0;
  if (zeros == n) return ojphgpu_encoder_set_budget(e, 0);
  if (zeros) return OJPHGPU_E_INVALID;
  if (!encoder_may_search(e) || e->quality_on) return OJPHGPU_E_INVALID;
  return no_throw([&]() -> int {
    if (!e->rate) { const int rc = encoder_rate_setup(e); if (rc) return rc; }
    e->budgets.assign(max_bytes, max_bytes + n);
    e->ran = false;
    return OJPHGPU_OK;
  });
}

static int encoder_rate_setup(ojphgpu_encoder* e)
{
  const Plan& P = *e->P;
  return no_throw([&]() -> int {
    HIPCHK(hipSetDevice(e->device));
    EncoderRate* R = new EncoderRate();
    struct Owner { EncoderRate* p; ~Owner() { delete p; } } owner{ R };
    for (const Band& B : P.bands) if ((uint64_t)B.r.w * B.r.h > 0xFFFFFFFFull) return OJPHGPU_E_INVALID;
    int rc = rate_table_build(P, R->table);
    if (rc) return rc;
    const uint32_t nframes = e->nframes;
    if ((uint64_t)P.bands.size() * nframes > 0xFFFFFFFFull) return OJPHGPU_E_INVALID;
    std::vector<ojphgpu_stats_desc> sd;
    for (uint32_t f = 0; f < nframes; ++f)
      for (size_t i = 0; i < P.bands.size(); ++i) {
        const Band& B = P.bands[i];
        if (B.empty) continue;
        sd.push_back(ojphgpu_stats_desc{ B.plane_off + (uint64_t)f * P.arena_elems, B.pitch, B.r.w, B.r.h, (uint32_t)(f * P.bands.size() + i) });
        R->stats_max_w = std::max(R->stats_max_w, B.r.w); R->stats_max_h = std::max(R->stats_max_h, B.r.h);
      }
    R->n_stats = (uint32_t)sd.size();
    std::vector<uint32_t> cls(e->block_ids.size());
    for (size_t i = 0; i < cls.size(); ++i) cls[i] = R->table.band_class[P.blocks[e->block_ids[i]].band];
    const uint32_t nc = R->table.nclasses;
    std::vector<uint32_t> kfine(P.bands.size());
    for (size_t i = 0; i < kfine.size(); ++i) kfine[i] = R->table.quant[(size_t)(OJPHGPU_RATE_GRID - 1) * nc + R->table.band_class[i]].K_max;
    std::vector<ojphgpu_cb_desc>& bd = R->bd;
    uint64_t scratch_bytes = 0;
    {
      const uint32_t out_cap = e->out_cap, nreg = e->nreg; const size_t counters_bytes = e->counters_bytes;
      const std::vector<uint32_t> regions = e->h_regions;
      bool clamped = false;
      encoder_block_layout(e, kfine.data(), bd, scratch_bytes, &clamped);
      if (clamped && nframes > 1) {
        e->out_cap = out_cap; e->nreg = nreg; e->counters_bytes = counters_bytes; e->h_regions = regions;
        return OJPHGPU_E_INVALID;
      }
    }
    { const int rc = encoder_settle(e); if (rc) return rc; }
    HIPCHK(hipStreamSynchronize(e->stream));
    if (e->side) HIPCHK(hipStreamSynchronize(e->side));
    e->scratch.release(); e->out.release(); e->regions.release(); e->counters.release();
    if (e->scratch.alloc(scratch_bytes) || e->out.alloc(e->out_cap) || e->counters.alloc(e->counters_bytes) ||
        (e->nreg && e->regions.alloc(e->h_regions.size() * 4)) ||
        R->stats_descs.alloc(sd.size() * sizeof(sd[0])) || R->hist.alloc(P.bands.size() * OJPHGPU_STATS_BINS * 4 * nframes) ||
        R->block_class.alloc(cls.size() * 4) || R->quant.alloc((size_t)nc * sizeof(BandQuant) * nframes))
      return OJPHGPU_E_NOMEM;
    if (e->nreg) HIPCHK(hipMemcpy(e->regions.p, e->h_regions.data(), e->h_regions.size() * 4, hipMemcpyHostToDevice));
    if (!bd.empty()) HIPCHK(hipMemcpy(e->cb_descs.p, bd.data(), bd.size() * sizeof(bd[0]), hipMemcpyHostToDevice));
    if (!sd.empty()) HIPCHK(hipMemcpy(R->stats_descs.p, sd.data(), sd.size() * sizeof(sd[0]), hipMemcpyHostToDevice));
    if (!cls.empty()) HIPCHK(hipMemcpy(R->block_class.p, cls.data(), cls.size() * 4, hipMemcpyHostToDevice));
    R->h_hist.assign(P.bands.size() * OJPHGPU_STATS_BINS * nframes, 0);
    R->h_quant.assign((size_t)nc * nframes, BandQuant{ 0.0f, 0 });
    e->rate = R; owner.p = nullptr;
    e->ran = false;
    return OJPHGPU_OK;
  });
}

static int encoder_code_round(ojphgpu_encoder* e, const RateTrialOut& o, const uint32_t* idx, const ojphgpu_cb_result** lengths)
{
  EncoderRate& R = *e->rate;
  hipStream_t s = e->stream;
  const uint32_t F = e->nframes, nc = R.table.nclasses, nb = (uint32_t)e->block_ids.size();
  for (uint32_t f = 0; f < F; ++f) std::copy_n(&R.table.quant[(size_t)idx[f] * nc], nc, &R.h_quant[(size_t)f * nc]);
  HIPCHK(hipMemcpyAsync(R.quant.p, R.h_quant.data(), R.h_quant.size() * sizeof(BandQuant), hipMemcpyHostToDevice, s));
  int rc = requant_frames_launch(s, (ojphgpu_cb_desc*)e->cb_descs.p, nb, F, (const uint32_t*)R.block_class.p, (const BandQuant*)R.quant.p, nc);
  if (rc) return rc;
  BlockCoderRun coder{ e, (uint8_t*)o.out, o.d_results, o.d_counters, nb * F, nullptr };
  if ((rc = coder.clear()) != 0 || (rc = coder.rest_and_join()) != 0) return rc;
  uint32_t status = 0;
  const auto w0 = std::chrono::steady_clock::now();
  if (o.h_results) {
    if ((rc = publish_words_launch(s, o.d_publish, o.d_counters, 2)) != 0) return rc;
    HIPCHK(hipEventRecord(o.done, s));
    HIPCHK(hipEventSynchronize(o.done));
    status = o.h_publish[1];
    *lengths = o.h_results;
  } else {
    const size_t rbytes = e->h_results.size() * sizeof(ojphgpu_cb_result);
    if (rbytes) HIPCHK(hipMemcpyAsync(e->h_results.data(), o.d_results, rbytes, hipMemcpyDeviceToHost, s));
    HIPCHK(hipMemcpyAsync(&status, o.d_counters + 1, 4, hipMemcpyDeviceToHost, s));
    HIPCHK(hipStreamSynchronize(s));
    *lengths = e->h_results.data();
  }
  R.wait_ms += std::chrono::duration<double, std::milli>(std::chrono::steady_clock::now() - w0).count();
  e->fetched = false;
  return status ? OJPHGPU_E_OVERFLOW : OJPHGPU_OK;
}

static int64_t rate_layout_bytes(const Plan& Q, const std::vector<uint32_t>& block_ids, const ojphgpu_cb_result* lengths)
{
  std::vector<ojphgpu_coded_block> cb;
  ojphgpu_coded_blocks(Q, block_ids, lengths, cb);
  T2Layout L;
  const int rc = t2_layout_codestream(Q, cb.data(), L);
  return rc ? (int64_t)rc : (int64_t)L.total;
}

int64_t ojphgpu_encoder_rate_trial(ojphgpu_encoder* e, Plan& Q, const RateTrialOut& o, uint32_t j)
{
  if (!rate_apply_step(Q, rate_grid_qstep(j))) return OJPHGPU_E_INVALID;
  const ojphgpu_cb_result* lengths = nullptr;
  const int rc = encoder_code_round(e, o, &j, &lengths);
  return rc ? (int64_t)rc : rate_layout_bytes(Q, e->block_ids, lengths);
}

static int encoder_plans_at(ojphgpu_encoder* e, const std::vector<uint32_t>& idx)
{
  EncoderRate& R = *e->rate;
  if (R.plans.size() > 32)
    for (auto it = R.plans.begin(); it != R.plans.end();) {
      if (std::find(idx.begin(), idx.end(), it->first) == idx.end()) { delete it->second; it = R.plans.erase(it); } else ++it;
    }
  R.frame_plan.assign(idx.size(), nullptr);
  for (size_t f = 0; f < idx.size(); ++f) {
    auto it = R.plans.find(idx[f]);
    if (it == R.plans.end()) {
      std::unique_ptr<ojphgpu_plan> q(new ojphgpu_plan{ *e->P });
      if (!rate_apply_step(q->plan, rate_grid_qstep(idx[f]))) return OJPHGPU_E_INVALID;
      it = R.plans.emplace(idx[f], q.release()).first;
    }
    R.frame_plan[f] = it->second;
  }
  return OJPHGPU_OK;
}

static int encoder_rate_search(ojphgpu_encoder* e)
{
  EncoderRate& R = *e->rate;
  if (R.searched) return R.search_rc;
  const auto t0 = std::chrono::steady_clock::now();
  R.wait_ms = 0;
  auto run = [&]() -> int {
    const uint32_t F = e->nframes, nb = (uint32_t)e->block_ids.size();
    if (e->budgets.size() != F) return OJPHGPU_E_INVALID;
    HIPCHK(hipMemcpyAsync(R.h_hist.data(), R.hist.p, R.h_hist.size() * 4, hipMemcpyDeviceToHost, e->stream));
    HIPCHK(hipStreamSynchronize(e->stream));
    R.wait_ms += std::chrono::duration<double, std::milli>(std::chrono::steady_clock::now() - t0).count();
    ojphgpu_rate_rounds_destroy(R.rounds); R.rounds = nullptr;
    int rc = rate_rounds_create(R.table, R.h_hist.data(), e->P->bands.size() * OJPHGPU_STATS_BINS, e->budgets.data(), F, -1, &R.rounds);
    if (rc) return rc;
    const RateTrialOut own{ e->out.p, (ojphgpu_cb_result*)e->results.p, (uint32_t*)e->counters.p, nullptr, nullptr, nullptr, nullptr };
    std::vector<uint32_t> idx(F, 0), list; std::vector<uint8_t> measures(F, 0); std::vector<int64_t> sizes(F, 0);
    while ((rc = ojphgpu_rate_rounds_next(R.rounds, idx.data(), measures.data())) == 1) {
      const ojphgpu_cb_result* lengths = nullptr;
      if ((rc = encoder_plans_at(e, idx)) != 0 || (rc = encoder_code_round(e, own, idx.data(), &lengths)) != 0) return rc;
      list.clear();
      for (uint32_t f = 0; f < F; ++f) if (measures[f]) list.push_back(f);
      parallel_for(list.size(), [&](size_t k) {
        const uint32_t f = list[k];
        sizes[f] = rate_layout_bytes(R.frame_plan[f]->plan, e->block_ids, lengths + (size_t)f * nb);
      });
      if ((rc = ojphgpu_rate_rounds_feed(R.rounds, sizes.data())) != 0) return rc;
    }
    return rc;
  };
  R.search_rc = no_throw(run);
  R.searched = true;
  R.search_ms = std::chrono::duration<double, std::milli>(std::chrono::steady_clock::now() - t0).count();
  return R.search_rc;
}

extern "C" int ojphgpu_encoder_rate_info_frame(ojphgpu_encoder* e, uint32_t frame, ojphgpu_rate_info* info)
{
  if (!e || !info || !e->rate || frame >= e->nframes) return OJPHGPU_E_INVALID;
  const EncoderRate& R = *e->rate;
  if (e->budgets.empty() || !R.searched || R.search_rc) return OJPHGPU_E_INVALID;
  return ojphgpu_rate_rounds_frame(R.rounds, frame, info);
}

extern "C" int ojphgpu_encoder_rate_info(ojphgpu_encoder* e, ojphgpu_rate_info* info)
{
  const int rc = ojphgpu_encoder_rate_info_frame(e, 0, info);
  return rc == OJPHGPU_E_BUDGET ? OJPHGPU_OK : rc;
}

extern "C" int ojphgpu_encoder_rate_rounds(ojphgpu_encoder* e, uint32_t* rounds)
{
  if (!e || !rounds || !e->rate || !e->rate->searched || e->budgets.empty()) return OJPHGPU_E_INVALID;
  return ojphgpu_rate_rounds_count(e->rate->rounds, rounds);
}

extern "C" int ojphgpu_encoder_rate_timing(ojphgpu_encoder* e, float out[4])
{
  if (!e || !out || !e->rate || !e->rate->searched || !e->ran) return OJPHGPU_E_INVALID;
  out[0] = (float)e->rate->search_ms; out[1] = (float)e->rate->wait_ms; out[2] = (float)e->rate->final_ms;
  if (e->timer.read(SP_STATS, &out[3])) return OJPHGPU_E_HIP;
  return OJPHGPU_OK;
}

static int decoder_create_synthesis(const ojphgpu_plan* plan, int device, void* stream, ojphgpu_decoder** out);
static int decoder_synthesis_only(ojphgpu_decoder* d, void* d_image, int container);

extern "C" int ojphgpu_encoder_clear_quality(ojphgpu_encoder* e)
{
  if (!e) return OJPHGPU_E_INVALID;
  if (e->quality_on && e->rate) { const int rc = encoder_restore_descs(e); if (rc) return rc; }
  e->quality_on = false; e->cap_bytes = 0;
  return OJPHGPU_OK;
}

extern "C" int ojphgpu_encoder_set_quality(ojphgpu_encoder* e, uint64_t max_sse)
{
  if (!e) return OJPHGPU_E_INVALID;
  if (e->nframes > 1 || !encoder_may_search(e) || !e->budgets.empty()) return OJPHGPU_E_INVALID;
  const Plan& P = *e->P;
  for (const CompGeo& g : P.comps) if (g.bit_depth > 16) return OJPHGPU_E_INVALID;
  if (e->quality) { e->max_sse = max_sse; e->cap_bytes = 0; e->quality_on = true; e->ran = false; return OJPHGPU_OK; }
  return no_throw([&]() -> int {
    HIPCHK(hipSetDevice(e->device));
    {
      RateTable T;
      const int rc = e->rate ? OJPHGPU_OK : rate_table_build(P, T);
      if (rc) return rc;
      const RateTable& U = e->rate ? e->rate->table : T;
      for (uint32_t c = 0; c < U.nclasses; ++c) if (U.quant[(size_t)(OJPHGPU_RATE_GRID - 1) * U.nclasses + c].K_max > 30) return OJPHGPU_E_INVALID;
    }
    if (!e->rate) { const int rc = encoder_rate_setup(e); if (rc) return rc; }
    EncoderQuality* Q = new EncoderQuality();
    struct Owner { EncoderQuality* p; ~Owner() { delete p; } } owner{ Q };
    int rc = decoder_create_synthesis(e->handle, e->device, e->stream, &Q->syn);
    if (rc) return rc;
    for (size_t i = 0; i < P.bands.size(); ++i) {
      const Band& B = P.bands[i];
      if (B.empty) continue;
      ojphgpu_requant_desc d; memset(&d, 0, sizeof(d));
      d.plane_off = B.plane_off; d.pitch = B.pitch; d.w = B.r.w; d.h = B.r.h;
      Q->h_descs.push_back(d); Q->desc_band.push_back((uint32_t)i);
      Q->max_w = std::max(Q->max_w, B.r.w); Q->max_h = std::max(Q->max_h, B.r.h);
    }
    std::vector<ojphgpu_error_comp> ec;
    for (const CompGeo& g : P.comps) ec.push_back(ojphgpu_error_comp{ g.frame_off, (uint64_t)g.w * g.h, g.is_signed ? 1u : 0u, 0u });
    Q->h_err.assign(ec.size(), ojphgpu_frame_err{ 0, 0, 0 }); Q->best = Q->h_err;
    if (Q->recon.alloc((size_t)P.frame_elems * 4) || Q->descs.alloc(Q->h_descs.size() * sizeof(ojphgpu_requant_desc)) ||
        Q->comps.alloc(ec.size() * sizeof(ec[0])) || Q->err.alloc(ec.size() * sizeof(ojphgpu_frame_err)))
      return OJPHGPU_E_NOMEM;
    if (!ec.empty()) HIPCHK(hipMemcpy(Q->comps.p, ec.data(), ec.size() * sizeof(ec[0]), hipMemcpyHostToDevice));
    e->quality = Q; owner.p = nullptr;
    e->max_sse = max_sse; e->cap_bytes = 0; e->quality_on = true; e->ran = false;
    return OJPHGPU_OK;
  });
}

extern "C" int ojphgpu_encoder_set_quality_capped(ojphgpu_encoder* e, uint64_t max_sse, uint64_t cap_bytes)
{
  const int rc = ojphgpu_encoder_set_quality(e, max_sse);
  if (rc == OJPHGPU_OK) e->cap_bytes = cap_bytes;
  return rc;
}

int ojphgpu_encoder_quality_trial(ojphgpu_encoder* e, const QualityTrialIo& io, uint32_t j, ojphgpu_frame_err* comps)
{
  EncoderRate& R = *e->rate; EncoderQuality& Q = *e->quality;
  hipStream_t s = e->stream;
  auto hip = [](hipError_t x) { return x == hipSuccess; };
  const uint32_t nc = R.table.nclasses;
  for (size_t i = 0; i < Q.h_descs.size(); ++i) {
    const BandQuant& q = R.table.quant[(size_t)j * nc + R.table.band_class[Q.desc_band[i]]];
    Q.h_descs[i].delta = q.delta; Q.h_descs[i].delta_inv = 1.0f / q.delta; Q.h_descs[i].K_max = q.K_max;
  }
  const size_t dbytes = Q.h_descs.size() * sizeof(ojphgpu_requant_desc), ebytes = Q.h_err.size() * sizeof(ojphgpu_frame_err);
  int rc;
  if (io.h_descs) {
    memcpy(io.h_descs, Q.h_descs.data(), dbytes);
    if ((rc = copy_to_host_launch(s, Q.descs.p, io.d_descs, dbytes)) != 0) return rc;
  } else if (dbytes && !hip(hipMemcpyAsync(Q.descs.p, Q.h_descs.data(), dbytes, hipMemcpyHostToDevice, s))) return OJPHGPU_E_HIP;
  rc = ojphgpu_band_requantise(s, (const ojphgpu_requant_desc*)Q.descs.p, (uint32_t)Q.h_descs.size(), Q.max_w, Q.max_h, e->arena.p, Q.syn->arena.p);
  if (rc) return rc;
  if ((rc = decoder_synthesis_only(Q.syn, Q.recon.p, 32)) != 0) return rc;
  if (!hip(hipMemsetAsync(Q.err.p, 0, ebytes, s))) return OJPHGPU_E_HIP;
  rc = ojphgpu_frame_error_ex(s, io.frame, io.container, Q.recon.p, 32, (const ojphgpu_error_comp*)Q.comps.p, (uint32_t)Q.h_err.size(), (ojphgpu_frame_err*)Q.err.p);
  if (rc) return rc;
  const auto w0 = std::chrono::steady_clock::now();
  if (io.h_err) {
    if ((rc = copy_to_host_launch(s, io.d_err, Q.err.p, ebytes)) != 0) return rc;
    if (!hip(hipEventRecord(io.done, s)) || !hip(hipEventSynchronize(io.done))) return OJPHGPU_E_HIP;
    memcpy(comps, io.h_err, ebytes);
  } else if (!hip(hipMemcpyAsync(comps, Q.err.p, ebytes, hipMemcpyDeviceToHost, s)) || !hip(hipStreamSynchronize(s))) return OJPHGPU_E_HIP;
  Q.wait_ms += std::chrono::duration<double, std::milli>(std::chrono::steady_clock::now() - w0).count();
  return OJPHGPU_OK;
}

static int64_t encoder_quality_trial(void* user, uint32_t j, uint64_t* sse)
{
  ojphgpu_encoder* e = (ojphgpu_encoder*)user;
  EncoderQuality& Q = *e->quality;
  const QualityTrialIo own{ Q.frame, Q.container, nullptr, nullptr, nullptr, nullptr, nullptr };
  const int rc = ojphgpu_encoder_quality_trial(e, own, j, Q.h_err.data());
  if (rc) return rc;
  uint64_t total = 0;
  for (const ojphgpu_frame_err& c : Q.h_err) total += c.sse;
  Q.by_index[j] = Q.h_err;
  *sse = total;
  return 0;
}

static int encoder_quality_search(ojphgpu_encoder* e)
{
  EncoderRate& R = *e->rate; EncoderQuality& Q = *e->quality;
  if (R.searched) return R.search_rc;
  const auto t0 = std::chrono::steady_clock::now();
  Q.wait_ms = 0; Q.final_ms = 0;
  auto run = [&]() -> int {
    if (!Q.frame) return OJPHGPU_E_INVALID;
    Q.by_index.assign(OJPHGPU_RATE_GRID, {});
    int rc = ojphgpu_quality_search(e->max_sse, encoder_quality_trial, e, &Q.info);
    Q.have_info = rc == OJPHGPU_OK || rc == OJPHGPU_E_QUALITY; Q.have_capped = false;
    Q.search_ms = std::chrono::duration<double, std::milli>(std::chrono::steady_clock::now() - t0).count();
    if (rc) return rc;
    Q.best = Q.by_index[Q.info.grid_index];
    for (const ojphgpu_frame_err& c : Q.best) Q.info.pae = std::max(Q.info.pae, c.pae);
    const auto t1 = std::chrono::steady_clock::now();
    const RateTrialOut own{ e->out.p, (ojphgpu_cb_result*)e->results.p, (uint32_t*)e->counters.p, nullptr, nullptr, nullptr, nullptr };
    const ojphgpu_cb_result* lengths = nullptr;
    if ((rc = encoder_plans_at(e, { Q.info.grid_index })) != 0 || (rc = encoder_code_round(e, own, &Q.info.grid_index, &lengths)) != 0) return rc;
    const int64_t size = rate_layout_bytes(R.frame_plan[0]->plan, e->block_ids, lengths);
    Q.final_ms = std::chrono::duration<double, std::milli>(std::chrono::steady_clock::now() - t1).count();
    if (size < 0) return size < INT32_MIN ? OJPHGPU_E_INVALID : (int)size;
    Q.info.bytes = (uint64_t)size;
    return OJPHGPU_OK;
  };
  R.search_rc = no_throw(run);
  R.searched = true;
  return R.search_rc;
}

static int64_t encoder_size_trial(void* user, uint32_t j)
{
  ojphgpu_encoder* e = (ojphgpu_encoder*)user;
  EncoderRate& R = *e->rate;
  const RateTrialOut own{ e->out.p, (ojphgpu_cb_result*)e->results.p, (uint32_t*)e->counters.p, nullptr, nullptr, nullptr, nullptr };
  const ojphgpu_cb_result* lengths = nullptr;
  int rc;
  if ((rc = encoder_plans_at(e, { j })) != 0 || (rc = encoder_code_round(e, own, &j, &lengths)) != 0) return rc;
  e->quality->coded_at = (int)j;
  return rate_layout_bytes(R.frame_plan[0]->plan, e->block_ids, lengths);
}

static const uint32_t* encoder_capped_hist(void* user)
{
  ojphgpu_encoder* e = (ojphgpu_encoder*)user;
  EncoderRate& R = *e->rate;
  int& verdict = e->quality->hist_rc;
  hipStream_t s = e->stream;
  auto hip = [](hipError_t x) { return x == hipSuccess; };
  verdict = OJPHGPU_E_HIP;
  if (!hip(hipMemsetAsync(R.hist.p, 0, R.hist.n, s))) return nullptr;
  if ((verdict = ojphgpu_band_stats(s, (const ojphgpu_stats_desc*)R.stats_descs.p, R.n_stats, R.stats_max_w, R.stats_max_h, e->arena.p, (uint32_t*)R.hist.p)) != 0) return nullptr;
  verdict = OJPHGPU_E_HIP;
  if (!hip(hipMemcpyAsync(R.h_hist.data(), R.hist.p, R.h_hist.size() * 4, hipMemcpyDeviceToHost, s)) || !hip(hipStreamSynchronize(s))) return nullptr;
  verdict = OJPHGPU_OK;
  return R.h_hist.data();
}

static int encoder_capped_search(ojphgpu_encoder* e)
{
  EncoderRate& R = *e->rate; EncoderQuality& Q = *e->quality;
  if (R.searched) return R.search_rc;
  const auto t0 = std::chrono::steady_clock::now();
  Q.wait_ms = 0; Q.final_ms = 0; R.wait_ms = 0;
  auto run = [&]() -> int {
    if (!Q.frame) return OJPHGPU_E_INVALID;
    Q.by_index.assign(OJPHGPU_RATE_GRID, {});
    Q.coded_at = -1; Q.have_info = false; Q.hist_rc = OJPHGPU_OK;
    int rc = capped_search(R.table, e->max_sse, e->cap_bytes, -1, -1, encoder_quality_trial, encoder_size_trial, encoder_capped_hist, e, &Q.capped);
    Q.have_capped = !Q.hist_rc && (rc == OJPHGPU_OK || rc == OJPHGPU_E_BUDGET);
    if (Q.hist_rc) return Q.hist_rc;
    if (rc) return rc;
    ojphgpu_capped_info& I = Q.capped;
    if (Q.coded_at != (int)I.grid_index) {
      const int64_t size = encoder_size_trial(e, I.grid_index);
      I.rate_passes++;
      if (size < 0) return size < INT32_MIN ? OJPHGPU_E_INVALID : (int)size;
      if ((uint64_t)size != I.bytes) return OJPHGPU_E_HIP;
    }
    Q.best = Q.by_index[I.grid_index];
    if (Q.best.size() != Q.h_err.size()) return OJPHGPU_E_INVALID;
    for (const ojphgpu_frame_err& c : Q.best) I.pae = std::max(I.pae, c.pae);
    return OJPHGPU_OK;
  };
  R.search_rc = no_throw(run);
  R.searched = true;
  Q.search_ms = std::chrono::duration<double, std::milli>(std::chrono::steady_clock::now() - t0).count();
  Q.wait_ms += R.wait_ms;
  return R.search_rc;
}

extern "C" int ojphgpu_encoder_capped_info(ojphgpu_encoder* e, ojphgpu_capped_info* info)
{
  if (!e || !info || !e->quality || !e->quality_on || !e->cap_bytes || !e->quality->have_capped || !e->rate->searched) return OJPHGPU_E_INVALID;
  *info = e->quality->capped;
  return OJPHGPU_OK;
}

extern "C" int ojphgpu_encoder_quality_info(ojphgpu_encoder* e, ojphgpu_quality_info* info)
{
  if (!e || !info || !e->quality || e->cap_bytes || !e->quality->have_info) return OJPHGPU_E_INVALID;
  *info = e->quality->info;
  return OJPHGPU_OK;
}

extern "C" int ojphgpu_encoder_quality_comp(ojphgpu_encoder* e, uint32_t comp, uint64_t* sse, uint32_t* pae)
{
  if (!e || !sse || !pae || !e->quality || !(e->quality->have_info || e->quality->have_capped) || !e->rate->searched || e->rate->search_rc || comp >= e->quality->best.size())
    return OJPHGPU_E_INVALID;
  *sse = e->quality->best[comp].sse; *pae = e->quality->best[comp].pae;
  return OJPHGPU_OK;
}

extern "C" int ojphgpu_encoder_quality_timing(ojphgpu_encoder* e, float out[3])
{
  if (!e || !out || !e->quality || !e->rate->searched) return OJPHGPU_E_INVALID;
  out[0] = (float)e->quality->search_ms; out[1] = (float)e->quality->wait_ms; out[2] = (float)e->quality->final_ms;
  return OJPHGPU_OK;
}

static int encode_host(ojphgpu_encoder* e, const void* h_image, int container, uint8_t* h_out, size_t cap, size_t* out_len)
{
  if (!e || !h_image) return OJPHGPU_E_INVALID;
  const Plan& P = *e->P;
  const size_t bytes = (size_t)P.frame_elems * 4 * e->nframes;
  if (!e->image.p && e->image.alloc(bytes)) return OJPHGPU_E_NOMEM;
  HIPCHK(hipMemcpyAsync(e->image.p, h_image, bytes / (32 / container), hipMemcpyHostToDevice, e->stream));
  int rc = ojphgpu_encoder_run_container(e, e->image.p, container);
  if (rc) return rc;
  return ojphgpu_encoder_finish(e, h_out, cap, out_len);
}

extern "C" int ojphgpu_encode(ojphgpu_encoder* e, const int32_t* h_image, uint8_t* h_out, size_t cap, size_t* out_len)
{
  return encode_host(e, h_image, 32, h_out, cap, out_len);
}

extern "C" int ojphgpu_encode16(ojphgpu_encoder* e, const uint16_t* h_image, uint8_t* h_out, size_t cap, size_t* out_len)
{
  return encode_host(e, h_image, 16, h_out, cap, out_len);
}

extern "C" int ojphgpu_encoder_timing(ojphgpu_encoder* e, float out[4])
{
  if (!e || !out || !e->ran) return OJPHGPU_E_INVALID;
  if (encoder_settle(e)) return OJPHGPU_E_HIP;
  if (e->timer.read(SP_CONVERT, &out[0]) || e->timer.read(SP_DWT, &out[1]) || e->timer.read(SP_HT_ENC, &out[2]) ||
      e->timer.read(-1, &out[3])) return OJPHGPU_E_HIP;
  return OJPHGPU_OK;
}

extern "C" int ojphgpu_encoder_ht_timing(ojphgpu_encoder* e, float* out, uint32_t cap, uint32_t* n, uint32_t* n_top)
{
  if (!e || !out || !n || !e->ran) return OJPHGPU_E_INVALID;
  if (encoder_settle(e)) return OJPHGPU_E_HIP;
  int k = e->timer.read_each(SP_HT_ENC, out, cap);
  if (k < 0) return OJPHGPU_E_HIP;
  *n = (uint32_t)k;
  if (n_top) *n_top = e->n_top;
  return OJPHGPU_OK;
}

extern "C" int ojphgpu_encoder_level_timing(ojphgpu_encoder* e, float* out, uint32_t cap, uint32_t* n)
{
  if (!e || !out || !n || !e->ran) return OJPHGPU_E_INVALID;
  if (encoder_settle(e)) return OJPHGPU_E_HIP;
  int k = e->timer.read_each(SP_DWT, out, cap);
  if (k < 0) return OJPHGPU_E_HIP;
  *n = (uint32_t)k;
  return OJPHGPU_OK;
}

extern "C" void ojphgpu_decoder_destroy(ojphgpu_decoder* d)
{
  if (!d) return;
  (void)hipSetDevice(d->device);
  for (DeviceBuf* b : { &d->arena, &d->image, &d->dwt_descs, &d->img_descs, &d->cb_descs, &d->conv_descs, &d->data, &d->status, &d->quads, &d->aux,
                       &d->fstate, &d->dwt_regs, &d->img_regs })
    b->release();
  if (d->h_retry) (void)hipHostFree(d->h_retry);
  if (d->h_stage) (void)hipHostFree(d->h_stage);
  if (d->ev_stage) (void)hipEventDestroy(d->ev_stage);
  if (d->side) (void)hipStreamDestroy(d->side);
  if (d->ev_fork) (void)hipEventDestroy(d->ev_fork);
  if (d->ev_join) (void)hipEventDestroy(d->ev_join);
  d->timer.destroy();
  delete d;
}

extern "C" int ojphgpu_decoder_create(const ojphgpu_plan* plan, int device, void* stream, ojphgpu_decoder** out)
{
  if (!plan) return OJPHGPU_E_INVALID;
  return ojphgpu_decoder_create_tiles(plan, device, stream, 0, (uint32_t)plan->plan.tiles.size(), out);
}

static int decoder_create(const ojphgpu_plan* const* plans, uint32_t nframes, int device, void* stream, uint32_t tile_first,
                          uint32_t tile_count, ojphgpu_decoder** out, bool blocks_only = false);

extern "C" int ojphgpu_decoder_create_tiles(const ojphgpu_plan* plan, int device, void* stream, uint32_t tile_first,
                                             uint32_t tile_count, ojphgpu_decoder** out)
{
  return no_throw([&] { return decoder_create(&plan, 1, device, stream, tile_first, tile_count, out); });
}

extern "C" int ojphgpu_decoder_create_batch(const ojphgpu_plan* const* plans, uint32_t num_frames, int device, void* stream,
                                             ojphgpu_decoder** out)
{
  if (!plans || num_frames == 0 || !plans[0]) return OJPHGPU_E_INVALID;
  return no_throw([&] { return decoder_create(plans, num_frames, device, stream, 0, (uint32_t)plans[0]->plan.tiles.size(), out); });
}

int ojphgpu_same_frame_geometry(const Plan& P, const Plan& Q, bool compare_blocks)
{
  if (Q.coded.size() != Q.blocks.size()) return OJPHGPU_E_INVALID;
  if (Q.skip_read != P.skip_read || Q.skip_recon != P.skip_recon) return OJPHGPU_E_INVALID;
// ... 1043 lines not shown
```

### openjph_amd/csrc/ojphgpu_objects.h

```cpp
#ifndef OJPHGPU_OBJECTS_H
#define OJPHGPU_OBJECTS_H
#include <hip/hip_runtime.h>

#include <algorithm>
#include <cstdint>
#include <cstdlib>
#include <cstring>
#include <map>
#include <vector>

#include "dwt_region.h"
#include "ht_tables.h"
#include "ojph_plan.h"

using namespace ojphgpu;

namespace {

#define HIPCHK(x) do { if ((x) != hipSuccess) return OJPHGPU_E_HIP; } while (0)

struct DeviceBuf {
  void* p = nullptr; size_t n = 0;
  int alloc(size_t bytes) { n = bytes; return hipMalloc(&p, bytes ? bytes : 16) == hipSuccess ? 0 : -1; }
  void release() { if (p) (void)hipFree(p); p = nullptr; }
};

struct HostBuf {
  uint8_t* p = nullptr; size_t cap = 0; bool pinned = false; unsigned uses = 0;
  int reserve(size_t bytes) {
    const bool want_pin = ++uses >= 2;
    if (bytes <= cap && (pinned || !want_pin)) return 0;
    release();
    void* q = nullptr;
    if (want_pin && hipHostMalloc(&q, bytes, hipHostMallocDefault) == hipSuccess) { p = (uint8_t*)q; pinned = true; }
    else { (void)hipGetLastError(); p = (uint8_t*)malloc(bytes); pinned = false; }
    cap = p ? bytes : 0;
    return p ? 0 : -1;
  }
  void release() { if (p) { if (pinned) (void)hipHostFree(p); else free(p); } p = nullptr; cap = 0; }
};

struct LevelBatch { uint32_t first, count, max_w, max_h, depth; bool rev; int img_first; int nc; int group; bool general; ojphgpu_lift k;
                    std::vector<uint32_t> comps;
                    ojphgpu::DwtRegionGrid rgrid;
                    uint32_t img_depth = 0, img_signed = 0; };

struct TileRange { uint32_t first, count; bool has(uint32_t t) const { return t >= first && t - first < count; } };

inline bool in_group(uint32_t comp, int group) { return group == 0 || (group == 1) == (comp < 3); }

inline bool is_wide(const Plan& P, uint32_t comp) { return comp < P.wide.size() && P.wide[comp] != 0; }
inline bool deep(const Plan& P, uint32_t comp) { return P.comps[comp].bit_depth > 26 || P.general(comp); }

inline bool general_image_fusable(const Plan& P, uint32_t c)
{
  if (!P.general(c) || is_wide(P, c) || P.comps[c].bit_depth > 26 || P.recon_decomps(c) == 0) return false;
  if (P.p.color_transform && c < 3) return false;
  const ojphgpu_lift k = P.lift_of(c, P.skip_recon + 1);
  return k.horz && k.vert && k.num_steps >= 1 && k.num_steps <= 4 && k.elem != 1;
}
inline bool general_fused(const Plan& P);

inline bool colour_fused(const Plan& P)
{
  if (!P.p.color_transform || P.any_nlt3 || P.p.num_comps < 3) return false;
  for (uint32_t c = 0; c < 3; ++c) if (P.recon_decomps(c) == 0 || deep(P, c)) return false;
  const char* off = getenv("OJPHGPU_NO_COLOUR_FUSION");
  return !(off && off[0] && off[0] != '0');
}

inline bool general_fused(const Plan& P)
{
  const char* off = getenv("OJPHGPU_NO_GENERAL_FUSION");
  if ((off && off[0] && off[0] != '0') || P.any_nlt3 || (P.p.color_transform && !colour_fused(P))) return false;
  bool any = false;
  for (uint32_t c = 0; c < P.p.num_comps; ++c) {
    if (!P.general(c) || P.recon_decomps(c) == 0) continue;
    if (!general_image_fusable(P, c)) return false;
    any = true;
  }
  return any;
}

template <typename F>
void for_levels_of(const Plan& P, TileRange tr, uint32_t depth, bool rev, int group, int gen_comp, F f)
{
  for (const ojphgpu_level_info& lv : P.levels) {
    if (!tr.has(lv.tile) || P.style(lv.comp).rev != rev || !in_group(lv.comp, group)) continue;
    if (gen_comp < 0 ? P.general(lv.comp) : (int)lv.comp != gen_comp) continue;
    const uint32_t L = P.recon_decomps(lv.comp);
    if (L > depth && lv.res == L - depth) f(lv);
  }
}

uint32_t max_recon_decomps(const Plan& P)
{
  uint32_t m = 0;
  for (uint32_t c = 0; c < P.p.num_comps; ++c) m = std::max(m, P.recon_decomps(c));
  return m;
}

inline void push_level_desc(const ojphgpu_level_info& lv, std::vector<ojphgpu_dwt_desc>& descs, LevelBatch& b)
{
  ojphgpu_dwt_desc d; memset(&d, 0, sizeof(d));
  d.src_off = lv.src_off; d.ll_off = lv.ll_off; d.hl_off = lv.hl_off; d.lh_off = lv.lh_off; d.hh_off = lv.hh_off;
  d.src_pitch = lv.src_pitch; d.ll_pitch = lv.ll_pitch; d.hl_pitch = lv.hl_pitch; d.lh_pitch = lv.lh_pitch;
  d.hh_pitch = lv.hh_pitch; d.w = lv.w; d.h = lv.h; d.x_even = lv.x_even; d.y_even = lv.y_even;
  descs.push_back(d);
  b.count++; b.max_w = std::max(b.max_w, lv.w); b.max_h = std::max(b.max_h, lv.h);
}

void build_level_batches(const Plan& P, TileRange tr, std::vector<ojphgpu_dwt_desc>& descs, std::vector<LevelBatch>& batches)
{
  descs.clear(); batches.clear();
  const uint32_t depths = max_recon_decomps(P);
  const bool fused = colour_fused(P);
  ojphgpu_lift none; memset(&none, 0, sizeof(none));
  for (uint32_t depth = 0; depth < depths; ++depth) {
    for (int rev = 0; rev < 2; ++rev)
    for (int group = (fused && depth == 0) ? 1 : 0; group <= ((fused && depth == 0) ? 2 : 0); ++group) {
      LevelBatch b{ (uint32_t)descs.size(), 0, 0, 0, depth, rev != 0, -1, group == 1 ? 3 : 1, group, false, none };
      for_levels_of(P, tr, depth, rev != 0, group, -1, [&](const ojphgpu_level_info& lv) { push_level_desc(lv, descs, b); });
      if (b.count) batches.push_back(b);
    }
    for (uint32_t c = 0; c < P.p.num_comps; ++c) {
      if (!P.general(c)) continue;
      const uint32_t L = P.recon_decomps(c);
      if (L <= depth) continue;
      LevelBatch b{ (uint32_t)descs.size(), 0, 0, 0, depth, P.style(c).rev, -1, 1, 0, true, P.lift_of(c, P.skip_recon + depth + 1) };
      for_levels_of(P, tr, depth, P.style(c).rev, 0, (int)c, [&](const ojphgpu_level_info& lv) { push_level_desc(lv, descs, b); });
      if (!b.count) continue;
      b.comps.push_back(c);
      LevelBatch* prev = batches.empty() ? nullptr : &batches.back();
      if (prev && prev->general && prev->depth == depth && prev->first + prev->count == b.first && memcmp(&prev->k, &b.k, sizeof(b.k)) == 0) {
        prev->count += b.count; prev->max_w = std::max(prev->max_w, b.max_w); prev->max_h = std::max(prev->max_h, b.max_h);
        prev->comps.push_back(c);
      } else batches.push_back(b);
    }
  }
}

void build_image_level_descs(const Plan& P, TileRange tr, const std::vector<ojphgpu_dwt_desc>& descs, std::vector<LevelBatch>& batches,
                             std::vector<ojphgpu_dwt_desc>& out)
{
  out.clear();
  if (P.any_nlt3 || (P.p.color_transform && !colour_fused(P))) return;
  const bool gfused = general_fused(P);
  auto note_format = [&](LevelBatch& b, const CompGeo& g) {
    if (g.bit_depth > b.img_depth) { b.img_depth = g.bit_depth; b.img_signed = g.is_signed ? 1 : 0; }
  };
  auto image_desc = [&](const ojphgpu_level_info& lv, ojphgpu_dwt_desc d) {
    const TileComp& tc = P.tcomps[P.tiles[lv.tile].comps[lv.comp]];
    const CompGeo& g = P.comps[lv.comp];
    const Rect& rr = P.ress[tc.res[lv.res]].r;
    d.src_off = g.frame_off + (uint64_t)(rr.y0 - g.y0) * g.w + (rr.x0 - g.x0);
    d.src_pitch = g.w;
    d.reserved = g.bit_depth | (g.is_signed ? 0x100u : 0u);
    return d;
  };
  for (LevelBatch& b : batches) {
    if (b.depth == 0 && b.count && b.general && gfused) {
      b.img_first = (int)out.size();
      size_t k = 0;
      for (uint32_t c : b.comps)
        for_levels_of(P, tr, 0, P.style(c).rev, 0, (int)c, [&](const ojphgpu_level_info& lv) {
          note_format(b, P.comps[lv.comp]);
          out.push_back(image_desc(lv, descs[b.first + k++]));
        });
      continue;
    }
    if (b.depth != 0 || b.count == 0 || b.general) continue;
    bool all_shallow = true;
    for_levels_of(P, tr, 0, b.rev, b.group, -1, [&](const ojphgpu_level_info& lv) { all_shallow = all_shallow && !deep(P, lv.comp); });
    if (!all_shallow) continue;
    b.img_first = (int)out.size();
    size_t k = 0;
    for_levels_of(P, tr, 0, b.rev, b.group, -1, [&](const ojphgpu_level_info& lv) {
      ojphgpu_dwt_desc d = descs[b.first + k++];
      const TileComp& tc = P.tcomps[P.tiles[lv.tile].comps[lv.comp]];
      const CompGeo& g = P.comps[lv.comp];
      const Rect& rr = P.ress[tc.res[lv.res]].r;
      d.src_off = g.frame_off + (uint64_t)(rr.y0 - g.y0) * g.w + (rr.x0 - g.x0);
      d.src_pitch = g.w;
      d.reserved = g.bit_depth | (g.is_signed ? 0x100u : 0u);
      note_format(b, g);
      out.push_back(d);
    });
  }
}

bool build_convert_descs(const Plan& P, TileRange tr, std::vector<ojphgpu_convert_desc>& descs, uint32_t& max_w, uint32_t& max_h)
{
  descs.clear(); max_w = max_h = 0;
  bool any = false;
  for (const Tile& t : P.tiles) {
    if (!tr.has(t.idx)) continue;
    for (uint32_t c = 0; c < P.p.num_comps; ++c) {
      const uint32_t L = P.recon_decomps(c);
      const TileComp& tc = P.tcomps[t.comps[c]];
      const Resolution& R = P.ress[tc.res[L]];
      ojphgpu_convert_desc d; memset(&d, 0, sizeof(d));
      if (L == 0) { const Band& B = P.bands[(size_t)R.band[0]]; d.plane_off = B.plane_off; d.pitch = B.pitch; }
      else { d.plane_off = R.plane_off; d.pitch = R.pitch; }
      const CompGeo& g = P.comps[c];
      d.src_x0 = R.r.x0 - g.x0; d.src_y0 = R.r.y0 - g.y0;
      d.img_pitch = g.w; d.img_off = g.frame_off;
      d.fmt = g.bit_depth | (g.is_signed ? 0x100u : 0u) | 0x200u | (P.style(c).rev ? 0x400u : 0u) | (P.nlt3[c] ? 0x800u : 0u) |
              (is_wide(P, c) ? 0x1000u : 0u);
      bool batch_deep = false;
      const int grp = colour_fused(P) ? (c < 3 ? 1 : 2) : 0;
      for (uint32_t o = 0; o < P.p.num_comps; ++o)
        batch_deep = batch_deep || (P.style(o).rev == P.style(c).rev && in_group(o, grp) && !P.general(o) && deep(P, o) && P.recon_decomps(o) > 0);
      if ((P.p.color_transform && !colour_fused(P)) || P.any_nlt3 || L == 0 || (P.general(c) && !general_fused(P)) || batch_deep) { d.w = R.r.w; d.h = R.r.h; any |= d.w && d.h; }
      descs.push_back(d);
      max_w = std::max(max_w, d.w); max_h = std::max(max_h, d.h);
    }
  }
  return any;
}

inline ojphgpu_dwt_region region_of_level(const Plan& P, const ojphgpu_level_info& lv, bool top)
{
  const TileComp& tc = P.tcomps[P.tiles[lv.tile].comps[lv.comp]];
  const uint32_t rid = tc.res[lv.res];
  const Rect& E = P.reg_exact[rid]; const Rect& R = P.ress[rid].r;
  ojphgpu_dwt_region r; memset(&r, 0, sizeof(r));
  if (E.w == 0 || E.h == 0) return r;
  r.rx0 = E.x0 - R.x0; r.ry0 = E.y0 - R.y0; r.rx1 = r.rx0 + E.w; r.ry1 = r.ry0 + E.h;
  if (top) {
    const CompGeo& g = P.comps[lv.comp];
    r.out_off = g.frame_off + (uint64_t)(E.y0 - g.y0) * g.w + (E.x0 - g.x0); r.out_pitch = g.w;
  }
  return r;
}

void restrict_levels_to_region(const Plan& P, TileRange tr, std::vector<ojphgpu_dwt_desc>& descs, std::vector<ojphgpu_dwt_desc>& img_descs,
                               std::vector<LevelBatch>& batches, std::vector<ojphgpu_dwt_region>& regs, std::vector<ojphgpu_dwt_region>& img_regs)
{
  std::vector<ojphgpu_dwt_desc> od, oi; std::vector<LevelBatch> ob;
  regs.clear(); img_regs.clear();
  for (const LevelBatch& b : batches) {
    LevelBatch n = b;
    n.first = (uint32_t)od.size(); n.count = 0; n.img_first = b.img_first >= 0 ? (int)oi.size() : -1;
    n.rgrid = ojphgpu::DwtRegionGrid();
    size_t k = 0;
    for_levels_of(P, tr, b.depth, b.rev, b.group, -1, [&](const ojphgpu_level_info& lv) {
      const size_t i = k++;
      const ojphgpu_dwt_region r = region_of_level(P, lv, b.img_first >= 0);
      if (r.rx1 <= r.rx0) return;
      od.push_back(descs[b.first + i]); regs.push_back(r);
      if (b.img_first >= 0) { oi.push_back(img_descs[(size_t)b.img_first + i]); img_regs.push_back(r); }
      ojphgpu::dwt_region_grid_add(n.rgrid, descs[b.first + i], r);
      n.count++;
    });
    if (n.count) ob.push_back(n);
  }
  descs.swap(od); img_descs.swap(oi); batches.swap(ob);
}

void replicate_regions(std::vector<ojphgpu_dwt_region>& regs, std::vector<ojphgpu_dwt_region>& img_regs, const std::vector<LevelBatch>& batches,
                       uint32_t nframes, uint64_t frame_elems)
{
  if (nframes <= 1) return;
  std::vector<ojphgpu_dwt_region> out, iout;
  for (const LevelBatch& b : batches)
    for (uint32_t f = 0; f < nframes; ++f)
      for (uint32_t i = 0; i < b.count; ++i) {
        out.push_back(regs[b.first + i]);
        if (b.img_first >= 0) { ojphgpu_dwt_region r = img_regs[(size_t)b.img_first + i]; r.out_off += (uint64_t)f * frame_elems; iout.push_back(r); }
      }
  regs.swap(out); img_regs.swap(iout);
}

uint32_t restrict_converts_to_region(const Plan& P, TileRange tr, std::vector<ojphgpu_convert_desc>& descs, uint32_t& max_w, uint32_t& max_h)
{
  std::vector<ojphgpu_convert_desc> out;
  max_w = max_h = 0;
  uint32_t kept = 0, ti = 0;
  for (const Tile& t : P.tiles) {
    if (!tr.has(t.idx)) continue;
    const size_t base = (size_t)(ti++) * P.p.num_comps;
    if (!P.reg_tiles[t.idx]) continue;
    ++kept;
    for (uint32_t c = 0; c < P.p.num_comps; ++c) {
      ojphgpu_convert_desc d = descs[base + c];
      const TileComp& tc = P.tcomps[t.comps[c]];
      const uint32_t rid = tc.res[P.recon_decomps(c)];
      const Rect& E = P.reg_exact[rid]; const Rect& R = P.ress[rid].r;
      const CompGeo& g = P.comps[c];
      if (d.w && d.h && E.w && E.h) {
        d.plane_off += (uint64_t)(E.y0 - R.y0) * d.pitch + (E.x0 - R.x0);
        d.w = E.w; d.h = E.h;
        d.src_x0 = E.x0 - g.x0; d.src_y0 = E.y0 - g.y0;
        d.img_pitch = g.w; d.img_off = g.frame_off;
      } else d.w = d.h = 0;
      max_w = std::max(max_w, d.w); max_h = std::max(max_h, d.h);
      out.push_back(d);
    }
  }
  descs.swap(out);
  return kept;
}

void replicate_levels(std::vector<ojphgpu_dwt_desc>& descs, std::vector<ojphgpu_dwt_desc>& img_descs, std::vector<LevelBatch>& batches,
                      uint32_t nframes, uint64_t arena_elems, uint64_t frame_elems)
{
  if (nframes <= 1) return;
  std::vector<ojphgpu_dwt_desc> out, iout; std::vector<LevelBatch> nb;
  for (const LevelBatch& b : batches) {
    LevelBatch n = b;
    n.first = (uint32_t)out.size(); n.count = b.count * nframes;
    if (b.img_first >= 0) n.img_first = (int)iout.size();
    for (uint32_t f = 0; f < nframes; ++f)
      for (uint32_t i = 0; i < b.count; ++i) {
        const uint64_t o = (uint64_t)f * arena_elems;
        ojphgpu_dwt_desc d = descs[b.first + i];
        d.src_off += o; d.ll_off += o; d.hl_off += o; d.lh_off += o; d.hh_off += o;
        out.push_back(d);
        if (b.img_first >= 0) {
          d = img_descs[(size_t)b.img_first + i];
          d.src_off += (uint64_t)f * frame_elems; d.ll_off += o; d.hl_off += o; d.lh_off += o; d.hh_off += o;
          iout.push_back(d);
        }
      }
    nb.push_back(n);
  }
  descs.swap(out); img_descs.swap(iout); batches.swap(nb);
}

void replicate_converts(std::vector<ojphgpu_convert_desc>& descs, uint32_t nframes, uint64_t arena_elems, uint64_t frame_elems)
{
  if (nframes <= 1 || descs.empty()) return;
  const size_t n = descs.size();
  for (uint32_t f = 1; f < nframes; ++f)
    for (size_t i = 0; i < n; ++i) {
      ojphgpu_convert_desc d = descs[i];
      d.plane_off += (uint64_t)f * arena_elems; d.img_off += (uint64_t)f * frame_elems;
      descs.push_back(d);
    }
}

std::vector<uint32_t> blocks_of_tiles(const Plan& P, TileRange tr)
{
  std::vector<uint32_t> ids;
  for (size_t i = 0; i < P.blocks.size(); ++i) {
    const Band& B = P.bands[P.blocks[i].band];
    if (P.has_region && !P.reg_blocks[i]) continue;
    if (tr.has(B.tile) && B.res <= P.top_read_res(B.comp)) ids.push_back((uint32_t)i);
  }
  return ids;
}

struct Spans {
  struct Span { hipEvent_t a, b; int kind; };
  std::vector<Span> pool;
  size_t used = 0;
  hipEvent_t t0 = nullptr, t1 = nullptr, t2 = nullptr;
  bool ok = false;
  bool detail = true;
  bool two = false;
  int init() { ok = hipEventCreate(&t0) == hipSuccess && hipEventCreate(&t1) == hipSuccess && hipEventCreate(&t2) == hipSuccess; return ok ? 0 : -1; }
  void destroy() {
    for (Span& x : pool) { (void)hipEventDestroy(x.a); (void)hipEventDestroy(x.b); }
    if (t0) (void)hipEventDestroy(t0);
    if (t1) (void)hipEventDestroy(t1);
    if (t2) (void)hipEventDestroy(t2);
    pool.clear();
  }
  void start(hipStream_t s) { used = 0; two = false; if (ok) (void)hipEventRecord(t0, s); }
  void finish(hipStream_t s) { if (ok) (void)hipEventRecord(t1, s); }
  void finish_two(hipStream_t s, hipStream_t other) { finish(s); two = ok; if (ok) (void)hipEventRecord(t2, other); }
  int begin(int kind, hipStream_t s) {
    if (!ok || !detail) return -1;
    if (used == pool.size()) {
      Span x{ nullptr, nullptr, kind };
      if (hipEventCreate(&x.a) != hipSuccess || hipEventCreate(&x.b) != hipSuccess) { ok = false; return -1; }
      pool.push_back(x);
    }
    pool[used].kind = kind;
    (void)hipEventRecord(pool[used].a, s);
    return (int)used++;
  }
  void end(int id, hipStream_t s) { if (ok && id >= 0) (void)hipEventRecord(pool[(size_t)id].b, s); }
  int read(int kind, float* out) {
    if (!ok || hipEventSynchronize(t1) != hipSuccess) return -1;
    if (kind < 0) {
      if (hipEventElapsedTime(out, t0, t1) != hipSuccess) return -1;
      float other = 0;
      if (two && (hipEventSynchronize(t2) != hipSuccess || hipEventElapsedTime(&other, t0, t2) != hipSuccess)) return -1;
      *out = std::max(*out, other);
      return 0;
    }
    float sum = 0;
    for (size_t i = 0; i < used; ++i)
      if (pool[i].kind == kind) { float ms = 0; if (hipEventElapsedTime(&ms, pool[i].a, pool[i].b) != hipSuccess) return -1; sum += ms; }
    *out = sum;
    return 0;
  }
  int read_each(int kind, float* out, uint32_t cap) {
    if (!ok || hipEventSynchronize(t1) != hipSuccess) return -1;
    int n = 0;
    for (size_t i = 0; i < used; ++i)
      if (pool[i].kind == kind && (uint32_t)n < cap) { if (hipEventElapsedTime(&out[n], pool[i].a, pool[i].b) != hipSuccess) return -1; ++n; }
    return n;
  }
};
enum { SP_CONVERT = 0, SP_DWT = 1, SP_HT_ENC = 2, SP_PREP = 3, SP_STEP1 = 4, SP_STEP2 = 5, SP_REFINE = 6, SP_STATS = 7 };

}

struct EncoderRate {
  RateTable table;
  DeviceBuf stats_descs, hist, block_class, quant;
  uint32_t n_stats = 0, stats_max_w = 0, stats_max_h = 0;
  std::vector<uint32_t> h_hist;
  std::vector<BandQuant> h_quant;
  std::vector<ojphgpu_cb_desc> bd;
  bool searched = false; int search_rc = 0;
  double search_ms = 0, wait_ms = 0, final_ms = 0;
  ojphgpu_rate_rounds* rounds = nullptr;
  std::vector<ojphgpu_plan*> frame_plan;
  std::map<uint32_t, ojphgpu_plan*> plans;
  ~EncoderRate() {
    for (DeviceBuf* b : { &stats_descs, &hist, &block_class, &quant }) b->release();
    for (auto& kv : plans) delete kv.second;
    ojphgpu_rate_rounds_destroy(rounds);
  }
};

struct ojphgpu_decoder;
struct EncoderQuality {
  ojphgpu_decoder* syn = nullptr;
  DeviceBuf recon, descs, comps, err;
  std::vector<uint32_t> desc_band;
  std::vector<ojphgpu_requant_desc> h_descs;
  uint32_t max_w = 0, max_h = 0;
  const void* frame = nullptr; int container = 0;
  std::vector<ojphgpu_frame_err> h_err, best;
  std::vector<std::vector<ojphgpu_frame_err>> by_index;
  bool have_info = false;
  ojphgpu_quality_info info;
  bool have_capped = false;
  ojphgpu_capped_info capped;
  int coded_at = -1;
  int hist_rc = 0;
  double search_ms = 0, wait_ms = 0, final_ms = 0;
  ~EncoderQuality();
};

struct ojphgpu_encoder {
  const ojphgpu_plan* handle = nullptr;
  const Plan* P = nullptr;
  int device = 0; hipStream_t stream = nullptr;
  DeviceBuf arena, image, dwt_descs, img_descs, cb_descs, conv_descs, scratch, out, results, counters;
  bool need_convert = false;
  std::vector<LevelBatch> batches;
  uint32_t conv_max_w = 0, conv_max_h = 0, out_cap = 0;
  TileRange tiles{ 0, 0 };
  uint32_t nframes = 1;
  bool fetched = false;
  uint64_t nbytes = 0;
  std::vector<uint32_t> block_ids;
  std::vector<ojphgpu_cb_result> h_results;
  HostBuf h_out, h_res;
  Spans timer;
  bool ran = false;
  uint32_t n_top = 0;
  int widths_top = 0, widths_rest = 0;
  hipStream_t side = nullptr;
  hipEvent_t ev_fork = nullptr, ev_join = nullptr;
  hipStream_t low = nullptr;
  hipEvent_t ev_low = nullptr;
  bool pending = false, can_release = false;
  void* o_out = nullptr; void* o_results = nullptr; void* o_counters = nullptr;
  uint32_t nreg = 0;
  std::vector<uint32_t> h_regions, h_cursors;
  DeviceBuf regions;
  size_t counters_bytes = 16;
  std::vector<uint64_t> budgets;
  EncoderRate* rate = nullptr;
  bool quality_on = false; uint64_t max_sse = 0;
  uint64_t cap_bytes = 0;
  EncoderQuality* quality = nullptr;
  bool searches() const { return !budgets.empty() || quality_on; }
};
inline bool encoder_releases(const ojphgpu_encoder* e)
{
  return e->can_release && e->n_top && !e->o_out && !e->o_results && !e->o_counters && !e->searches() && !e->timer.detail;
}
inline int encoder_settle(ojphgpu_encoder* e)
{
  if (!e->pending) return OJPHGPU_OK;
  HIPCHK(hipStreamWaitEvent(e->stream, e->ev_join, 0));
  HIPCHK(hipStreamWaitEvent(e->stream, e->ev_low, 0));
  e->pending = false;
  return OJPHGPU_OK;
}
struct RateTrialOut {
  void* out; ojphgpu_cb_result* d_results; uint32_t* d_counters;
  const ojphgpu_cb_result* h_results; uint32_t* d_publish; const uint32_t* h_publish; hipEvent_t done;
};
int64_t ojphgpu_encoder_rate_trial(ojphgpu_encoder* e, Plan& Q, const RateTrialOut& o, uint32_t j);
struct QualityTrialIo {
  const void* frame; int container;
  ojphgpu_requant_desc* h_descs; const void* d_descs;
  const ojphgpu_frame_err* h_err; void* d_err; hipEvent_t done;
};
int ojphgpu_encoder_quality_trial(ojphgpu_encoder* e, const QualityTrialIo& io, uint32_t j, ojphgpu_frame_err* comps);
int ojphgpu_encoder_run_container(ojphgpu_encoder* e, const void* d_image, int container);
int ojphgpu_encoder_create_joined(const ojphgpu_plan* plan, int device, void* stream, ojphgpu_encoder** out);

inline void ojphgpu_coded_blocks(const Plan& P, const std::vector<uint32_t>& block_ids, const ojphgpu_cb_result* res,
                                 std::vector<ojphgpu_coded_block>& cb)
{
  cb.assign(P.blocks.size(), ojphgpu_coded_block{ 0, 0, 0, 0, 0 });
  for (size_t i = 0; i < block_ids.size(); ++i) {
    const ojphgpu_cb_result& r = res[i];
    ojphgpu_coded_block& c = cb[block_ids[i]];
    c.offset = r.offset; c.len1 = r.length; c.len2 = 0;
    c.missing_msbs = r.length ? P.bands[P.blocks[block_ids[i]].band].K_max - 1 : 0;
    c.num_passes = r.length ? 1 : 0;
  }
}

struct PadCopy { uint64_t src, dst; uint32_t got, total; };
struct DecRun { uint64_t src, dst, n; };
struct ojphgpu_decoder {
  const Plan* P = nullptr;
  int device = 0; hipStream_t stream = nullptr;
  DeviceBuf arena, image, dwt_descs, img_descs, cb_descs, conv_descs, data, status, quads, aux;
  DeviceBuf fstate; uint32_t fused_epoch = 0, max_block_h = 0;
  uint32_t cus = 256;
  bool last_fused = false, force_separate = false;
  void* last_image = nullptr; int last_container = 0;
  uint32_t fused_retries = 0;
  uint32_t* h_retry = nullptr; uint32_t* d_h_retry = nullptr; bool uncollected = false;
  uint32_t retry_acked = 0;
  uint32_t fused_strikes = 0; bool fused_off = false;
  void fused_outcome(bool repeated) { if (!repeated) fused_strikes = 0; else if (++fused_strikes >= 8u) fused_off = true; }
  uint32_t n_low = 0;
  hipStream_t side = nullptr;
  hipEvent_t ev_fork = nullptr, ev_join = nullptr;
  bool need_convert = false;
  TileRange tiles{ 0, 0 };
  uint32_t nframes = 1;
  bool any_refine = false;
  int kinds = 0;
  std::vector<size_t> f_first, f_len, f_base;
  std::vector<std::vector<PadCopy>> f_pads;
  bool region = false;
  std::vector<std::vector<DecRun>> f_runs;
  uint8_t* h_stage = nullptr; size_t stage_cap = 0;
  hipEvent_t ev_stage = nullptr;
  DeviceBuf dwt_regs, img_regs;
  uint32_t conv_tiles = 0, tiles_touched = 0;
  uint32_t nblocks = 0;
  std::vector<LevelBatch> batches;
  uint32_t conv_max_w = 0, conv_max_h = 0, max_len1 = 0;
  size_t data_first = 0, data_len = 0;
  Spans timer;
  bool ran = false;
  std::vector<uint32_t> block_ids;
  const void* o_cb_descs = nullptr; const void* o_data = nullptr; void* o_status = nullptr;
  bool blocks_only = false;
};
struct ojphgpu_transcoder {
  ojphgpu_decoder* dec = nullptr; ojphgpu_encoder* enc = nullptr;
  const Plan* S = nullptr; const Plan* O = nullptr;
  int device = 0; hipStream_t stream = nullptr;
  std::vector<ojphgpu_cb_desc> h_descs;
  int stage = 0;
  bool resilient = false;
  uint32_t failed = 0;
  double code_ms = 0, final_ms = 0;
};
struct ojphgpu_recoder {
  ojphgpu_decoder* dec = nullptr; ojphgpu_encoder* enc = nullptr;
  const Plan* S = nullptr; const Plan* O = nullptr;
  int device = 0; hipStream_t stream = nullptr;
  DeviceBuf frame, fitted, comps;
  int container = 32; uint32_t ncomps = 0;
  std::vector<ojphgpu_cb_desc> h_descs;
  std::vector<uint8_t> h_stage;
  hipEvent_t ev_fit0 = nullptr, ev_fit1 = nullptr;
  int stage = 0;
  bool resilient = false;
  uint32_t failed = 0;
  double final_ms = 0;
  void* g() const { return container == 32 ? frame.p : fitted.p; }
};
struct DecFrameInfo;
typedef int (*ojphgpu_status_fetch)(void* user, const uint8_t** h_status);
int ojphgpu_decoder_collect(ojphgpu_decoder* d, ojphgpu_status_fetch fetch, void* user, uint32_t* count);
int ojphgpu_transcoder_check_source(const ojphgpu_transcoder* t, const Plan& Q);
int ojphgpu_transcoder_fill_descs(const ojphgpu_transcoder* t, const Plan& Q, size_t cs_len, ojphgpu_cb_desc* bd, DecFrameInfo& fi);
int ojphgpu_transcoder_decode(ojphgpu_transcoder* t, bool any_refine, int kinds, uint32_t max_len1);
int ojphgpu_transcoder_stats(ojphgpu_transcoder* t);
int ojphgpu_transcoder_verdicts(ojphgpu_transcoder* t, ojphgpu_status_fetch fetch, void* user, bool resilient, uint32_t* failed);
int ojphgpu_transcoder_code(ojphgpu_transcoder* t, void* out, ojphgpu_cb_result* d_results, uint32_t* d_counters);
struct DecFrameInfo {
  std::vector<DecRun> runs;
  uint64_t first = 0, len = 0; bool any_refine = false; uint32_t max_len1 = 0; int kinds = 0;
  std::vector<PadCopy> pads; uint64_t pad_len = 0;
  uint64_t data_bytes() const { return ((len + 63) & ~(uint64_t)63) + pad_len; }
};
int ojphgpu_decoder_upload_pads(hipStream_t s, uint8_t* d_frame_data, const uint8_t* h_codestream, size_t cs_len, const std::vector<PadCopy>& pads);
int  ojphgpu_same_frame_geometry(const Plan& P, const Plan& Q, bool compare_blocks);
void ojphgpu_decoder_fill_descs(const Plan& P, const Plan& Q, const std::vector<uint32_t>& ids, uint64_t arena_off,
                                uint64_t data_base, ojphgpu_cb_desc* bd, DecFrameInfo& fi, bool want_runs = false);
int  ojphgpu_decoder_run_container(ojphgpu_decoder* d, void* d_image, int container);
inline EncoderQuality::~EncoderQuality()
{
  for (DeviceBuf* b : { &recon, &descs, &comps, &err }) b->release();
  if (syn) ojphgpu_decoder_destroy(syn);
}
inline bool ojphgpu_fused_retry_wanted(const uint8_t* h_status, uint32_t nblocks, uint32_t epoch)
{
  uint32_t w; memcpy(&w, h_status + ((nblocks + 3u) & ~3u), 4);
  return w == epoch;
}


#endif
```

Measured before the change: 108,300 Msamples/s.

## Double-buffer encoder output sets and split released top blocks separately

Adds a second set of arena, output, results and counter buffers that alternate between consecutive released encodes, so a new frame can start before the previous frame's low-priority block-coding tail has drained. The counter clear moves onto the side stream when possible, and the released path gets its own top/rest block split (default 50% of top-resolution blocks). Output regions are now indexed by absolute block index instead of being rebased per split. In exchange it doubles buffer memory and makes the event and stream ordering more complex.

```diff
diff --git a/openjph_amd/csrc/ht_tables.h b/openjph_amd/csrc/ht_tables.h
--- a/openjph_amd/csrc/ht_tables.h
+++ b/openjph_amd/csrc/ht_tables.h
@@ -23,7 +23,7 @@
 namespace ojphgpu {
 int ht_encode_launch(void* stream, const ojphgpu_cb_desc* d_blocks, uint32_t n, const void* d_coef, uint8_t* d_scratch,
                      uint8_t* d_out, uint32_t out_cap, ojphgpu_cb_result* d_results, uint32_t* d_cursor, uint32_t* d_status,
-                     int widths, const uint32_t* d_regions, uint32_t nreg);
+                     int widths, const uint32_t* d_regions, uint32_t nreg, uint32_t first);
 bool dec_fuses();
 uint64_t ht_decode_fused_state_words(uint32_t n);
 uint32_t device_cus(int device);
diff --git a/openjph_amd/csrc/kernels_ht_enc.hip b/openjph_amd/csrc/kernels_ht_enc.hip
--- a/openjph_amd/csrc/kernels_ht_enc.hip
+++ b/openjph_amd/csrc/kernels_ht_enc.hip
@@ -147,7 +147,7 @@
     const ojphgpu_cb_desc* __restrict__ blocks, uint32_t n, const uint32_t* __restrict__ coef,
     uint8_t* __restrict__ scratch, uint8_t* __restrict__ out, uint32_t out_cap,
     ojphgpu_cb_result* __restrict__ results, uint32_t* __restrict__ cursor, uint32_t* __restrict__ status,
-    const uint32_t* __restrict__ regions, uint32_t nreg)
+    const uint32_t* __restrict__ regions, uint32_t nreg, uint32_t first)
 {
   using V = typename std::conditional<S64, uint64_t, uint32_t>::type;
   constexpr uint32_t VBITS = S64 ? 64u : 32u;
@@ -466,7 +466,7 @@
   uint32_t off = 0;
   if (err) total = 0;
   if (total) {
-    off = claim_output(cursor, regions, nreg, bi, (total + 3u) & ~3u, out_cap, lane);
+    off = claim_output(cursor, regions, nreg, first + bi, (total + 3u) & ~3u, out_cap, lane);
     if (off == 0xFFFFFFFFu) { err = 1; total = 0; off = 0; }
   }
   if (total) {
@@ -606,7 +606,7 @@
     const ojphgpu_cb_desc* __restrict__ blocks, uint32_t n, const uint32_t* __restrict__ coef,
     uint8_t* __restrict__ scratch, uint8_t* __restrict__ out, uint32_t out_cap,
     ojphgpu_cb_result* __restrict__ results, uint32_t* __restrict__ cursor, uint32_t* __restrict__ status,
-    const uint32_t* __restrict__ regions, uint32_t nreg)
+    const uint32_t* __restrict__ regions, uint32_t nreg, uint32_t first)
 {
   __shared__ __attribute__((aligned(16))) uint16_t s_vlc[2][2048];
   __shared__ uint32_t s_uvlc[64];
@@ -1235,7 +1235,7 @@
   if (err) total = 0;
   const uint32_t slot = (total + 3u) & ~3u;
   Claim claim = { 0, 0, 0 };
-  if (total) claim = claim_request(cursor, regions, nreg, bi, slot, out_cap, lane);
+  if (total) claim = claim_request(cursor, regions, nreg, first + bi, slot, out_cap, lane);
   const uint32_t scup = mel.pos + v_pos;
   const uint32_t tail = mel.pos + v_pos;
   const uint32_t gpart = min(ms_out, ms_len), local = ms_len - gpart;
@@ -1296,7 +1296,7 @@
 namespace ojphgpu {
 int ht_encode_launch(void* stream, const ojphgpu_cb_desc* d_blocks, uint32_t n, const void* d_coef, uint8_t* d_scratch,
                      uint8_t* d_out, uint32_t out_cap, ojphgpu_cb_result* d_results, uint32_t* d_cursor, uint32_t* d_status,
-                     int widths, const uint32_t* d_regions, uint32_t nreg)
+                     int widths, const uint32_t* d_regions, uint32_t nreg, uint32_t first)
 {
   if (n == 0) return OJPHGPU_OK;
   if (ensure_tables() != 0) return OJPHGPU_E_HIP;
@@ -1308,29 +1308,29 @@
   const dim3 ngrid((n + NWAVES - 1) / NWAVES);
   if ((widths & 1) && (widths & 4) && (widths & 16))
     hipLaunchKernelGGL((ht_encode_kernel<true, 3>), ngrid, dim3(64 * NWAVES), ballast, (hipStream_t)stream, d_blocks, n,
-                       (const uint32_t*)d_coef, d_scratch, d_out, out_cap, d_results, d_cursor, d_status, d_regions, nreg);
+                       (const uint32_t*)d_coef, d_scratch, d_out, out_cap, d_results, d_cursor, d_status, d_regions, nreg, first);
   else if ((widths & 1) && (widths & 4))
     hipLaunchKernelGGL((ht_encode_kernel<true, 4>), ngrid, dim3(64 * NWAVES), ballast, (hipStream_t)stream, d_blocks, n,
-                       (const uint32_t*)d_coef, d_scratch, d_out, out_cap, d_results, d_cursor, d_status, d_regions, nreg);
+                       (const uint32_t*)d_coef, d_scratch, d_out, out_cap, d_results, d_cursor, d_status, d_regions, nreg, first);
   if ((widths & 1) && (widths & 8) && (widths & 16))
     hipLaunchKernelGGL((ht_encode_kernel<false, 3>), ngrid, dim3(64 * NWAVES), ballast, (hipStream_t)stream, d_blocks, n,
-                       (const uint32_t*)d_coef, d_scratch, d_out, out_cap, d_results, d_cursor, d_status, d_regions, nreg);
+                       (const uint32_t*)d_coef, d_scratch, d_out, out_cap, d_results, d_cursor, d_status, d_regions, nreg, first);
   else if ((widths & 1) && (widths & 8))
     hipLaunchKernelGGL((ht_encode_kernel<false, 4>), ngrid, dim3(64 * NWAVES), ballast, (hipStream_t)stream, d_blocks, n,
-                       (const uint32_t*)d_coef, d_scratch, d_out, out_cap, d_results, d_cursor, d_status, d_regions, nreg);
+                       (const uint32_t*)d_coef, d_scratch, d_out, out_cap, d_results, d_cursor, d_status, d_regions, nreg, first);
   if ((widths & 2) && (widths & 64)) {
     if (widths & 4)
       hipLaunchKernelGGL((ht_encode_kernel<true, 5>), ngrid, dim3(64 * NWAVES), ballast, (hipStream_t)stream, d_blocks, n,
-                         (const uint32_t*)d_coef, d_scratch, d_out, out_cap, d_results, d_cursor, d_status, d_regions, nreg);
+                         (const uint32_t*)d_coef, d_scratch, d_out, out_cap, d_results, d_cursor, d_status, d_regions, nreg, first);
     if (widths & 8)
       hipLaunchKernelGGL((ht_encode_kernel<false, 5>), ngrid, dim3(64 * NWAVES), ballast, (hipStream_t)stream, d_blocks, n,
-                         (const uint32_t*)d_coef, d_scratch, d_out, out_cap, d_results, d_cursor, d_status, d_regions, nreg);
+                         (const uint32_t*)d_coef, d_scratch, d_out, out_cap, d_results, d_cursor, d_status, d_regions, nreg, first);
   } else if (widths & 2)
     hipLaunchKernelGGL(ht_encode_wide_kernel<false>, grid, dim3(64 * WAVES), 0, (hipStream_t)stream, d_blocks, n,
-                       (const uint32_t*)d_coef, d_scratch, d_out, out_cap, d_results, d_cursor, d_status, d_regions, nreg);
+                       (const uint32_t*)d_coef, d_scratch, d_out, out_cap, d_results, d_cursor, d_status, d_regions, nreg, first);
   if (widths & 32)
     hipLaunchKernelGGL(ht_encode_wide_kernel<true>, grid, dim3(64 * WAVES), 0, (hipStream_t)stream, d_blocks, n,
-                       (const uint32_t*)d_coef, d_scratch, d_out, out_cap, d_results, d_cursor, d_status, d_regions, nreg);
+                       (const uint32_t*)d_coef, d_scratch, d_out, out_cap, d_results, d_cursor, d_status, d_regions, nreg, first);
   return hipGetLastError() == hipSuccess ? OJPHGPU_OK : OJPHGPU_E_HIP;
 }
 }
@@ -1339,7 +1339,7 @@
                                   const void* d_coef, uint8_t* d_scratch, uint8_t* d_out, uint32_t out_cap,
                                   ojphgpu_cb_result* d_results, uint32_t* d_cursor, uint32_t* d_status)
 {
-  return ojphgpu::ht_encode_launch(stream, d_blocks, n, d_coef, d_scratch, d_out, out_cap, d_results, d_cursor, d_status, 3 | 32, nullptr, 0);
+  return ojphgpu::ht_encode_launch(stream, d_blocks, n, d_coef, d_scratch, d_out, out_cap, d_results, d_cursor, d_status, 3 | 32, nullptr, 0, 0);
 }
 
 namespace ojphgpu {
diff --git a/openjph_amd/csrc/ojphgpu_codec.cpp b/openjph_amd/csrc/ojphgpu_codec.cpp
--- a/openjph_amd/csrc/ojphgpu_codec.cpp
+++ b/openjph_amd/csrc/ojphgpu_codec.cpp
@@ -44,15 +44,19 @@
   (void)hipSetDevice(e->device);
   if (e->side) (void)hipStreamSynchronize(e->side);
   if (e->low) (void)hipStreamSynchronize(e->low);
-  e->pending = false;
+  e->pending = e->other.pending = false;
   for (DeviceBuf* b : { &e->arena, &e->image, &e->dwt_descs, &e->img_descs, &e->cb_descs, &e->conv_descs, &e->scratch, &e->out,
-                        &e->results, &e->counters, &e->regions }) b->release();
+                        &e->results, &e->counters, &e->regions, &e->other.arena, &e->other.out, &e->other.results,
+                        &e->other.counters }) b->release();
   e->h_out.release(); e->h_res.release();
   if (e->side) (void)hipStreamDestroy(e->side);
   if (e->low) (void)hipStreamDestroy(e->low);
   if (e->ev_fork) (void)hipEventDestroy(e->ev_fork);
   if (e->ev_join) (void)hipEventDestroy(e->ev_join);
   if (e->ev_low) (void)hipEventDestroy(e->ev_low);
+  if (e->other.ev_join) (void)hipEventDestroy(e->other.ev_join);
+  if (e->other.ev_low) (void)hipEventDestroy(e->other.ev_low);
+  if (e->ev_clear) (void)hipEventDestroy(e->ev_clear);
   e->timer.destroy();
   delete e->quality;
   delete e->rate;
@@ -85,6 +89,28 @@
 {
   if (!plan) return OJPHGPU_E_INVALID;
   return no_throw([&] { return encoder_create(plan, device, stream, 0, (uint32_t)plan->plan.tiles.size(), num_frames, out); });
+}
+
+#ifndef OJPHGPU_ENC_TOP_SHARE_RELEASED_DEFAULT
+#define OJPHGPU_ENC_TOP_SHARE_RELEASED_DEFAULT 50
+#endif
+static ojphgpu_encoder::EncoderCut encoder_cut(const ojphgpu_encoder* e, uint32_t n_top)
+{
+  const Plan& P = *e->P;
+  ojphgpu_encoder::EncoderCut c; c.n_top = n_top;
+  bool over32_top = false, over32_rest = false, over128_top = false, over128_rest = false;
+  for (size_t i = 0; i < e->block_ids.size(); ++i) {
+    const Block& k = P.blocks[e->block_ids[i]]; const Band& B = P.bands[k.band];
+    const bool wide = is_wide(P, B.comp), rev = P.style(B.comp).rev;
+    (i < n_top ? c.widths_top : c.widths_rest) |= wide ? 32 : ((k.r.w > 64 ? 2 : 1) | (rev ? 4 : 8));
+    if (!wide && k.r.w > 32 && k.r.w <= 64) (i < n_top ? over32_top : over32_rest) = true;
+    if (!wide && k.r.w > 128) (i < n_top ? over128_top : over128_rest) = true;
+  }
+  if (!over32_top) c.widths_top |= 16;
+  if (!over32_rest) c.widths_rest |= 16;
+  if (!over128_top) c.widths_top |= 64;
+  if (!over128_rest) c.widths_rest |= 64;
+  return c;
 }
 
 static void encoder_block_layout(ojphgpu_encoder* e, const uint32_t* band_kmax, std::vector<ojphgpu_cb_desc>& bd, uint64_t& scratch_total,
@@ -95,7 +121,6 @@
   const uint32_t nframes = e->nframes;
   bd.assign(e->block_ids.size(), ojphgpu_cb_desc());
   uint64_t scratch_bytes = 0, samples = 0;
-  bool over32_top = false, over32_rest = false, over128_top = false, over128_rest = false;
   for (size_t i = 0; i < bd.size(); ++i) {
     const Block& k = P.blocks[e->block_ids[i]]; const Band& B = P.bands[k.band];
     samples += (uint64_t)k.r.w * k.r.h;
@@ -106,14 +131,7 @@
     d.missing_msbs = (uint8_t)(B.K_max - 1); d.num_passes = 1; d.delta = B.delta;
     d.data_off = scratch_bytes; d.scratch_cap = block_scratch_bytes(k.r.w, k.r.h, band_kmax ? std::max(B.K_max, band_kmax[k.band]) : B.K_max);
     scratch_bytes += d.scratch_cap;
-    (i < e->n_top ? e->widths_top : e->widths_rest) |= wide ? 32 : ((k.r.w > 64 ? 2 : 1) | ((d.reversible & 1) ? 4 : 8));
-    if (!wide && k.r.w > 32 && k.r.w <= 64) (i < e->n_top ? over32_top : over32_rest) = true;
-    if (!wide && k.r.w > 128) (i < e->n_top ? over128_top : over128_rest) = true;
-  }
-  if (!over32_top) e->widths_top |= 16;
-  if (!over32_rest) e->widths_rest |= 16;
-  if (!over128_top) e->widths_top |= 64;
-  if (!over128_rest) e->widths_rest |= 64;
+  }
   if (nframes > 1) {
     const size_t nb = bd.size();
     bd.resize(nb * nframes);
@@ -137,7 +155,7 @@
     std::vector<uint64_t> rc(R ? R : 1, 0);
     if (R) for (size_t i = 0; i < bd.size(); ++i) {
       const uint64_t own = kmax_all > 20 ? bd[i].scratch_cap : std::min<uint64_t>(bd[i].scratch_cap, (uint64_t)bd[i].w * bd[i].h * 3 + 64);
-      rc[(i < e->n_top ? i : i - e->n_top) & (R - 1)] += own;
+      rc[i & (R - 1)] += own;
     }
     uint64_t total = 0;
     e->h_regions.assign(2 * (size_t)R, 0);
@@ -188,6 +206,7 @@
     replicate_converts(cd, nframes, P.arena_elems, P.frame_elems);
   }
   e->block_ids = blocks_of_tiles(P, tr);
+  uint32_t n_top_released = 0;
   if (nframes == 1 && max_recon_decomps(P) >= 2 && getenv("OJPHGPU_NO_OVERLAP") == nullptr) {
     auto top = [&](uint32_t id) { const Band& B = P.bands[P.blocks[id].band]; return B.res == P.style(B.comp).L; };
     auto mid = std::stable_partition(e->block_ids.begin(), e->block_ids.end(), top);
@@ -205,7 +224,12 @@
       const double move = (s_top + margin_us / us_per_ms - 1.6 * s_low - dwt_us / us_per_ms) / 2.0;
       int share = share_env;
       if (!share) { share = s_top > 0 && move > 0 ? (int)(100.0 * (1.0 - move / s_top)) : 100; share = share < 50 ? 50 : share > 100 ? 100 : share; }
-      e->n_top = (uint32_t)((uint64_t)e->n_top * (uint32_t)share / 100u);
+      const uint32_t n_res_top = e->n_top;
+      e->n_top = (uint32_t)((uint64_t)n_res_top * (uint32_t)share / 100u);
+      const char* rv = getenv("OJPHGPU_ENC_TOP_SHARE_RELEASED");
+      const int rshare = rv ? std::min(100, std::max(10, atoi(rv))) : OJPHGPU_ENC_TOP_SHARE_RELEASED_DEFAULT;
+      n_top_released = rshare ? (uint32_t)((uint64_t)n_res_top * (uint32_t)rshare / 100u) : e->n_top;
+      if (n_top_released == 0 || n_top_released == e->block_ids.size()) n_top_released = e->n_top;
     }
     if (e->n_top == 0 || e->n_top == e->block_ids.size()) e->n_top = 0;
     else {
@@ -222,8 +246,18 @@
       if (e->can_release &&
           (hipStreamCreateWithPriority(&e->low, hipStreamNonBlocking, own_prio) != hipSuccess ||
            hipEventCreateWithFlags(&e->ev_low, hipEventDisableTiming) != hipSuccess)) return bail(OJPHGPU_E_HIP);
-    }
-  }
+      const char* sets = getenv("OJPHGPU_ENC_SETS"); const char* sc = getenv("OJPHGPU_ENC_SIDE_CLEAR");
+      e->two_sets = e->can_release && !(sets && atoi(sets) == 1);
+      e->clear_on_side = e->can_release && !(sc && sc[0] == '0');
+      if (e->two_sets &&
+          (hipEventCreateWithFlags(&e->other.ev_join, hipEventDisableTiming) != hipSuccess ||
+           hipEventCreateWithFlags(&e->other.ev_low, hipEventDisableTiming) != hipSuccess)) return bail(OJPHGPU_E_HIP);
+      if (e->clear_on_side && hipEventCreateWithFlags(&e->ev_clear, hipEventDisableTiming) != hipSuccess) return bail(OJPHGPU_E_HIP);
+    }
+  }
+  e->cut_joined = encoder_cut(e, e->n_top);
+  e->cut_released = e->can_release ? encoder_cut(e, n_top_released) : e->cut_joined;
+  e->take_cut(e->cut_joined);
   std::vector<ojphgpu_cb_desc> bd;
   uint64_t scratch_bytes = 0;
   encoder_block_layout(e, nullptr, bd, scratch_bytes);
@@ -236,6 +270,12 @@
       e->results.alloc(bd.size() * sizeof(ojphgpu_cb_result)) || e->counters.alloc(e->counters_bytes) ||
       (e->nreg && e->regions.alloc(e->h_regions.size() * 4)))
     return bail(OJPHGPU_E_NOMEM);
+  if (e->two_sets) {
+    if (e->other.arena.alloc(P.arena_elems * 4) || e->other.out.alloc(cap) ||
+        e->other.results.alloc(bd.size() * sizeof(ojphgpu_cb_result)) || e->other.counters.alloc(e->counters_bytes))
+      return bail(OJPHGPU_E_NOMEM);
+    if (hipMemset(e->other.arena.p, 0, P.arena_elems * 4) != hipSuccess) return bail(OJPHGPU_E_HIP);
+  }
   if (e->nreg && hipMemcpy(e->regions.p, e->h_regions.data(), e->h_regions.size() * 4, hipMemcpyHostToDevice) != hipSuccess) return bail(OJPHGPU_E_HIP);
   if (!blocks_only && hipMemset(e->arena.p, 0, P.arena_elems * 4 * nframes) != hipSuccess) return bail(OJPHGPU_E_HIP);
   if (!dd.empty() && hipMemcpy(e->dwt_descs.p, dd.data(), dd.size() * sizeof(dd[0]), hipMemcpyHostToDevice) != hipSuccess) return bail(OJPHGPU_E_HIP);
@@ -258,16 +298,33 @@
 namespace {
 struct BlockCoderRun {
   ojphgpu_encoder* e; uint8_t* out; ojphgpu_cb_result* res; uint32_t* cnt; uint32_t nblocks; Spans* T;
-  bool forked = false;
+  bool forked = false, cleared_on_side = false;
   int launch(hipStream_t st, uint32_t first, uint32_t n, int widths) {
     const int sh = T ? T->begin(SP_HT_ENC, st) : -1;
     int rc = ojphgpu::ht_encode_launch(st, (const ojphgpu_cb_desc*)e->cb_descs.p + first, n, e->arena.p, (uint8_t*)e->scratch.p, out,
-                                       e->out_cap, res + first, cnt, cnt + 1, widths, (const uint32_t*)e->regions.p, e->nreg);
+                                       e->out_cap, res + first, cnt, cnt + 1, widths, (const uint32_t*)e->regions.p, e->nreg, first);
     if (rc) return rc;
     if (T) T->end(sh, st);
     return OJPHGPU_OK;
   }
-  int clear() { int rc = encoder_settle(e); if (rc) return rc; HIPCHK(hipMemsetAsync(cnt, 0, e->counters_bytes, e->stream)); return OJPHGPU_OK; }
+  int clear() {
+    int rc = encoder_settle(e);
+    if (rc) return rc;
+    e->stream_wrote = true;
+    HIPCHK(hipMemsetAsync(cnt, 0, e->counters_bytes, e->stream));
+    return OJPHGPU_OK;
+  }
+  int clear_released() {
+    int rc = encoder_settle_last(e);
+    if (rc) return rc;
+    cleared_on_side = e->clear_on_side && !e->stream_wrote;
+    e->stream_wrote = false;
+    if (!cleared_on_side) { HIPCHK(hipMemsetAsync(cnt, 0, e->counters_bytes, e->stream)); return OJPHGPU_OK; }
+    HIPCHK(hipStreamWaitEvent(e->side, e->ev_low, 0));
+    HIPCHK(hipMemsetAsync(cnt, 0, e->counters_bytes, e->side));
+    HIPCHK(hipEventRecord(e->ev_clear, e->side));
+    return OJPHGPU_OK;
+  }
   int fork_top(bool release = false) {
     forked = true;
     HIPCHK(hipEventRecord(e->ev_fork, e->stream));
@@ -275,7 +332,11 @@
     int rc = launch(e->side, 0, e->n_top, e->widths_top);
     if (rc) return rc;
     HIPCHK(hipEventRecord(e->ev_join, e->side));
-    if (release) { e->pending = true; HIPCHK(hipStreamWaitEvent(e->low, e->ev_fork, 0)); }
+    if (release) {
+      e->pending = true;
+      HIPCHK(hipStreamWaitEvent(e->low, e->ev_fork, 0));
+      if (cleared_on_side) HIPCHK(hipStreamWaitEvent(e->low, e->ev_clear, 0));
+    }
     return OJPHGPU_OK;
   }
   int rest_released() { return launch(e->low, e->n_top, nblocks - e->n_top, e->widths_rest); }
@@ -302,12 +363,14 @@
   if (container != 32) for (const CompGeo& g : P.comps) if (g.bit_depth > (uint32_t)container) return OJPHGPU_E_INVALID;
   hipStream_t s = e->stream;
   Spans& T = e->timer;
+  const bool release = encoder_releases(e);
+  if (release) encoder_next_set(e);
+  e->take_cut(release ? e->cut_released : e->cut_joined);
   BlockCoderRun coder{ e, (uint8_t*)(e->o_out ? e->o_out : e->out.p),
                        (ojphgpu_cb_result*)(e->o_results ? e->o_results : e->results.p),
                        (uint32_t*)(e->o_counters ? e->o_counters : e->counters.p), (uint32_t)e->block_ids.size() * e->nframes, &T };
-  int rc = coder.clear();
-  if (rc) return rc;
-  const bool release = encoder_releases(e);
+  int rc = release ? coder.clear_released() : coder.clear();
+  if (rc) return rc;
   ReleasedBranch branch{ e };
   T.start(s);
   if (e->need_convert) {
@@ -422,7 +485,7 @@
     if (rbytes) memcpy(e->h_results.data(), e->h_res.p, rbytes);
     if (e->nreg)
       for (size_t i = 0; i < e->h_results.size(); ++i) {
-        const uint32_t r = (uint32_t)(i < e->n_top ? i : i - e->n_top) & (e->nreg - 1);
+        const uint32_t r = (uint32_t)i & (e->nreg - 1);
         if (e->h_results[i].length) e->h_results[i].offset = (uint32_t)(e->h_results[i].offset - e->h_regions[2 * r] + hpos[r]);
       }
     e->fetched = true;
@@ -565,6 +628,7 @@
   if (!encoder_may_search(e) || e->quality_on) return OJPHGPU_E_INVALID;
   return no_throw([&]() -> int {
     if (!e->rate) { const int rc = encoder_rate_setup(e); if (rc) return rc; }
+    { const int rc = encoder_settle(e); if (rc) return rc; }
     e->budgets.assign(max_bytes, max_bytes + n);
     e->ran = false;
     return OJPHGPU_OK;
@@ -613,6 +677,10 @@
     HIPCHK(hipStreamSynchronize(e->stream));
     if (e->side) HIPCHK(hipStreamSynchronize(e->side));
     e->scratch.release(); e->out.release(); e->regions.release(); e->counters.release();
+    if (e->two_sets) {
+      e->other.out.release(); e->other.counters.release();
+      if (e->other.out.alloc(e->out_cap) || e->other.counters.alloc(e->counters_bytes)) return OJPHGPU_E_NOMEM;
+    }
     if (e->scratch.alloc(scratch_bytes) || e->out.alloc(e->out_cap) || e->counters.alloc(e->counters_bytes) ||
         (e->nreg && e->regions.alloc(e->h_regions.size() * 4)) ||
         R->stats_descs.alloc(sd.size() * sizeof(sd[0])) || R->hist.alloc(P.bands.size() * OJPHGPU_STATS_BINS * 4 * nframes) ||
@@ -779,7 +847,11 @@
   if (e->nframes > 1 || !encoder_may_search(e) || !e->budgets.empty()) return OJPHGPU_E_INVALID;
   const Plan& P = *e->P;
   for (const CompGeo& g : P.comps) if (g.bit_depth > 16) return OJPHGPU_E_INVALID;
-  if (e->quality) { e->max_sse = max_sse; e->cap_bytes = 0; e->quality_on = true; e->ran = false; return OJPHGPU_OK; }
+  if (e->quality) {
+    if (encoder_settle(e)) return OJPHGPU_E_HIP;
+    e->max_sse = max_sse; e->cap_bytes = 0; e->quality_on = true; e->ran = false;
+    return OJPHGPU_OK;
+  }
   return no_throw([&]() -> int {
     HIPCHK(hipSetDevice(e->device));
     {
diff --git a/openjph_amd/csrc/ojphgpu_objects.h b/openjph_amd/csrc/ojphgpu_objects.h
--- a/openjph_amd/csrc/ojphgpu_objects.h
+++ b/openjph_amd/csrc/ojphgpu_objects.h
@@ -7,6 +7,7 @@
 #include <cstdlib>
 #include <cstring>
 #include <map>
+#include <utility>
 #include <vector>
 
 #include "dwt_region.h"
@@ -467,11 +468,22 @@
   bool ran = false;
   uint32_t n_top = 0;
   int widths_top = 0, widths_rest = 0;
+  struct EncoderCut { uint32_t n_top = 0; int widths_top = 0, widths_rest = 0; } cut_joined, cut_released;
+  void take_cut(const EncoderCut& c) { n_top = c.n_top; widths_top = c.widths_top; widths_rest = c.widths_rest; }
   hipStream_t side = nullptr;
   hipEvent_t ev_fork = nullptr, ev_join = nullptr;
   hipStream_t low = nullptr;
   hipEvent_t ev_low = nullptr;
   bool pending = false, can_release = false;
+  bool stream_wrote = false;
+  struct OtherSet {
+    DeviceBuf arena, out, results, counters;
+    hipEvent_t ev_join = nullptr, ev_low = nullptr;
+    bool pending = false, stream_wrote = false;
+  } other;
+  bool two_sets = false;
+  hipEvent_t ev_clear = nullptr;
+  bool clear_on_side = false;
   void* o_out = nullptr; void* o_results = nullptr; void* o_counters = nullptr;
   uint32_t nreg = 0;
   std::vector<uint32_t> h_regions, h_cursors;
@@ -486,15 +498,32 @@
 };
 inline bool encoder_releases(const ojphgpu_encoder* e)
 {
-  return e->can_release && e->n_top && !e->o_out && !e->o_results && !e->o_counters && !e->searches() && !e->timer.detail;
-}
-inline int encoder_settle(ojphgpu_encoder* e)
+  return e->can_release && e->cut_released.n_top && !e->o_out && !e->o_results && !e->o_counters && !e->searches() && !e->timer.detail;
+}
+inline int encoder_settle_last(ojphgpu_encoder* e)
 {
   if (!e->pending) return OJPHGPU_OK;
   HIPCHK(hipStreamWaitEvent(e->stream, e->ev_join, 0));
   HIPCHK(hipStreamWaitEvent(e->stream, e->ev_low, 0));
   e->pending = false;
   return OJPHGPU_OK;
+}
+inline int encoder_settle(ojphgpu_encoder* e)
+{
+  if (e->other.pending) {
+    HIPCHK(hipStreamWaitEvent(e->stream, e->other.ev_join, 0));
+    HIPCHK(hipStreamWaitEvent(e->stream, e->other.ev_low, 0));
+    e->other.pending = false;
+  }
+  return encoder_settle_last(e);
+}
+inline void encoder_next_set(ojphgpu_encoder* e)
+{
+  if (!e->two_sets) return;
+  std::swap(e->arena, e->other.arena); std::swap(e->out, e->other.out);
+  std::swap(e->results, e->other.results); std::swap(e->counters, e->other.counters);
+  std::swap(e->ev_join, e->other.ev_join); std::swap(e->ev_low, e->other.ev_low);
+  std::swap(e->pending, e->other.pending); std::swap(e->stream_wrote, e->other.stream_wrote);
 }
 struct RateTrialOut {
   void* out; ojphgpu_cb_result* d_results; uint32_t* d_counters;
```

After: 116,800 Msamples/s, median of 6. +7.8%, better.
